# rll/rllab

Hardware: AMD Instinct MI355X
Metric: env steps/sec over full TRPO iterations (sample + process + update), 4096 envs per MI355X (higher is better)
Workload: dtype f32

## Files before the change

### include/rllab_amd.h

```cpp
#ifndef RLLAB_AMD_H
#define RLLAB_AMD_H

#include <stddef.h>
#include <stdint.h>

#ifdef __cplusplus
extern "C" {
#endif

enum rl_env_kind {
    RL_ENV_CARTPOLE = 0,
    RL_ENV_DOUBLE_PENDULUM = 1,
    RL_ENV_SWIMMER = 2,
    RL_ENV_HALF_CHEETAH = 3,
    RL_ENV_CARTPOLE_SWINGUP = 4,
    RL_ENV_WALKER2D = 5,
    RL_ENV_HOPPER = 6,
    RL_ENV_INVERTED_DOUBLE_PENDULUM = 7
};

enum rl_status {
    RL_OK = 0,
    RL_ERR_ARG = -1,
    RL_ERR_UNSUPPORTED = -2,
// ... 288 lines not shown
    float* actions;
    float* means;
    float* rewards;
    uint8_t* dones;
    float* first_path;
    const rl_env_cfg* cfg;
    const rl_launch_opts* opts;
} rl_population_gru_args;

int rl_rollout_population_gru(const rl_population_gru_args* args, void* stream);

int rl_gae(int T, int n, const float* rewards, const double* values, const uint8_t* dones,
           double gamma, double lambda, float* adv, float* ret, float* undiscounted, void* stream);

int rl_discount_cumsum(int T, int n, const float* x, const uint8_t* dones, double discount,
                       float* y, void* stream);


int rl_path_scan(int T, int n, int obs_dim, const uint8_t* dones, const float* obs, const double* coeffs,
                 int whole_paths, int32_t* tin, uint8_t* valid, double* values, void* stream);

size_t rl_process_workspace_bytes(int obs_dim);

int rl_sample_stats_cols(void);

int rl_sample_stats(size_t n_samples, const float* returns, const double* baselines,
                    const float* advantages, const float* undiscounted, const int32_t* tin,
                    const uint8_t* valid, double ret_shift, double und_shift, const float* progress,
                    int n_cols, void* workspace, size_t workspace_bytes, double* out, void* stream);

int rl_adv_finish(size_t n_samples, const float* adv_in, const uint8_t* valid, double mean, double denom,
                  double shift, float* adv_out, void* stream);

int rl_lfb_normal_eq(size_t n_samples, int obs_dim, const float* obs, const int32_t* tin,
                     const float* returns, const uint8_t* valid, void* workspace, size_t workspace_bytes,
                     double* out, int variant, void* stream);


size_t rl_reps_workspace_bytes(int T, int n);

int rl_reps_dual(int T, int n, int obs_dim, const float* obs, const float* rewards, const int32_t* tin,
                 const uint8_t* dones, const uint8_t* valid, double eta, const double* v_host, void* workspace,
                 size_t workspace_bytes, double* out, void* stream);

int rl_reps_weights(int T, int n, int obs_dim, const float* obs, const float* rewards, const int32_t* tin,
                    const uint8_t* dones, const uint8_t* valid, double eta, const double* v_host,
                    const double* dual_out, float* weights, void* stream);

typedef struct rl_policy_batch {
    int32_t n_samples;
    int32_t obs_dim, act_dim;
    int32_t hidden0, hidden1;
    int32_t hidden2;
    float inv_count;
    float log_min_std;
    const float* theta;
    const float* obs;
    const float* actions;
    const float* advantages;
    const float* old_means;
    const float* old_log_std;
    const float* weights;
    float* activations;
    float kl_penalty;
    int32_t activation;
    const rl_launch_opts* opts;
    int32_t layer_activations;
    int32_t reserved_pad;
    const int32_t* gate;
    float* obs_absmax;
} rl_policy_batch;

enum rl_activation { RL_ACT_TANH = 0, RL_ACT_RECTIFY = 1, RL_ACT_IDENTITY = 2 };

size_t rl_policy_workspace_bytes(int obs_dim, int act_dim, int hidden0, int hidden1, int hidden2);

size_t rl_policy_activation_bytes(int n_samples, int hidden0, int hidden1, int hidden2);

int rl_policy_loss_kl(const rl_policy_batch* batch, void* workspace, size_t workspace_bytes,
                      double* out4, void* stream);

int rl_policy_grad(const rl_policy_batch* batch, int vpg, void* workspace, size_t workspace_bytes,
                   double* grad_out, void* stream);

int rl_policy_grad_loss(const rl_policy_batch* batch, int vpg, void* workspace, size_t workspace_bytes,
                        double* grad_out, double* out4, void* stream);

int rl_policy_fvp(const rl_policy_batch* batch, const float* vec, void* workspace,
                  size_t workspace_bytes, double* fvp_out, void* stream);

int rl_policy_fvp_variant(const rl_policy_batch* batch);


int rl_mlp_forward(const rl_policy_batch* batch, const float* vec, float* out, float* dout, void* stream);
int rl_mlp_forward_ws(const rl_policy_batch* batch, const float* vec, void* workspace, size_t workspace_bytes, float* out,
                      float* dout, void* stream);

int rl_mlp_backward(const rl_policy_batch* batch, const float* cotangent, void* workspace, size_t workspace_bytes,
                    double* grad_out, void* stream);

size_t rl_gaussian_head_workspace_bytes(void);
int rl_gaussian_head(size_t n_samples, int act_dim, const float* mean, const float* log_std, const float* actions,
                     const float* advantages, const float* old_means, const float* old_log_stds,
// ... 45 lines not shown

int rl_categorical_softmax(size_t n_samples, int n_act, const float* logits, float* prob, void* stream);

size_t rl_categorical_head_workspace_bytes(void);
int rl_categorical_head(size_t n_samples, int n_act, const float* logits, const float* actions, const float* advantages,
                        const float* old_prob, const float* weights, float inv_count, int vpg, float kl_penalty,
                        float* g_logits, void* workspace, size_t workspace_bytes, double* out4, void* stream);

int rl_categorical_fisher(size_t n_samples, int n_act, const float* dlogits, const float* logits, const float* weights,
                          float inv_count, float* g_logits, void* stream);

int rl_cmaes_cov_update(int N, int ld, int mu, int mu_neg, double* C, double* Yneg, double* dC, const double* Ypos,
                        const double* wpos, const double* Vneg, const double* wneg, const double* pc, const double* scal,
                        void* stream);

int rl_cg_init(int n, const double* b, double* x, double* r, double* p, float* p32, double* scal,
               void* stream);
int rl_cg_step(int n, const double* fvp, double reg_coeff, double residual_tol, double* x, double* r,
               double* p, float* p32, double* scal, void* stream);

int rl_policy_fvp_cg_step(const rl_policy_batch* batch, void* workspace, size_t workspace_bytes, double reg_coeff,
                          double residual_tol, double* x, double* r, double* p, float* p32, double* scal,
                          double* fvp_scratch, unsigned int* ticket, void* stream);

int rl_trpo_step(int n, const double* x, const double* a, const double* b, double reg_coeff,
                 double max_constraint, double* step, double* out, void* stream);

int rl_line_search_point(int n, const float* prev, const double* step, double ratio, float* theta,
                         void* stream);

int rl_line_search_decide(int rows, const double* sums, const double* before, double inv_count, double max_constraint,
                          int candidate, double* state, int32_t* gate, int n, const float* prev, const double* step,
                          double next_ratio, float* theta, void* stream);

int rl_adam_step(int n, float* theta, const double* grad, double* m, double* v, double a_t, double beta1,
                 double beta2, double epsilon, void* stream);

size_t rl_peer_mailbox_bytes(int world, int max_n);
int rl_peer_alloc(size_t bytes, void** dev_ptr_out);
int rl_peer_free(void* dev_ptr);
int rl_peer_export(void* dev_ptr, void* handle_out64_host);
int rl_peer_open(const void* handle64_host, void** dev_ptr_out);
int rl_peer_close(void* dev_ptr);
int rl_peer_allreduce_sum(int n, double* data, int rank, int world, void* const* mailboxes_host, int max_n,
                          uint64_t seq, int* err_dev, int64_t spin_limit, void* stream);

int rl_debug_philox(uint32_t c0, uint32_t c1, uint32_t c2, uint32_t c3, uint32_t k0, uint32_t k1,
                    int count, uint32_t* out, void* stream);

#ifdef __cplusplus
}
#endif
#endif
```

### profiles/make_index.py

```python
#!/usr/bin/env python3
import fnmatch
import os
import subprocess

ROOT = os.path.dirname(os.path.dirname(os.path.abspath(__file__)))

RECIPES = [
    ("pmc_traffic.json", "HBM bytes + vector-instruction counters of the rollout kernels per workload, stamped with sha256(csrc/*); bench.py reads it",
     "profiles/run_profile.sh <tag> (traffic step: profiles/summarize.py traffic ...)"),
    ("gru_bptt_time.json", "loss + KL, gradient and Fisher-vector product of a GaussianGRUPolicy per call, and one whole TRPO update: the recurrent update kernels next to the float32 autograd closures, the sampler's batch for 4096 Cartpole envs, max_path_length 100 (105 rows x 4096 columns), 32 units",
     "python tools/exp/gru_bptt_time.py --out profiles/gru_bptt_time.json"),
    ("categorical_gru_bptt_time.json", "loss + KL, gradient and Fisher-vector product of a CategoricalGRUPolicy per call, and one whole TRPO update: the recurrent categorical update kernels next to the float32 autograd closures, the sampler's batch for 4096 GridWorld 4x4 envs, max_path_length 100, 32 units",
     "python tools/exp/categorical_gru_bptt_time.py --out profiles/categorical_gru_bptt_time.json"),
    ("*_bench_line.json", "the default bench line of that tree", "python bench.py"),
    ("*_bench_under_rocprof.log", "bench stdout under the kernel-trace pass", "profiles/run_profile.sh <tag>"),
    ("*_c5_kernel_stats.csv", "kernel stats of C5's per-GPU shard", "profiles/run_profile.sh <tag> cheetah1024_trpo_gae"),
    ("*_c5_pmc_*.csv", "PMC passes of C5's per-GPU shard (one counter group per pass)", "profiles/run_profile.sh <tag> cheetah1024_trpo_gae"),
    ("*_c2_*.csv", "kernel stats / PMC passes of C2 (Cartpole 4096 envs, VPG)", "profiles/run_profile.sh <tag> cartpole4096_vpg"),
    ("r06_csplit_*.csv", "SQ counter passes / kernel stats of csplit_fvp_kernel on (100, 50, 25) and (128, 128) at 2.048 M samples", "tools/exp/r06_call8.sh"),
    ("r06_c7_csplit_ab.txt", "cooperative product per library: round start / one instruction stream per wavefront (off) / compile-time shapes + k-slices", "tools/exp/r06_call7.sh"),
    ("r06_c9_csplit_ab.txt", "cooperative product per library: k-slices + compile-time shapes / round start / + late fetch", "tools/exp/r06_call9.sh"),
    ("r06_c10_csplit_ab.txt", "cooperative product: the library of the round's start, timed in the call that ran the parity tests and the wide bench lines on the final one", "tools/exp/r06_call10.sh"),
    ("r06_f16_split.txt", "device facts of the two-way f16 split: subnormal inputs honoured, accuracy of five product forms against float64 over ten magnitude regimes, the five-instruction split bit for bit, instruction rates", "tools/ubench/f16_split.hip (tools/exp/r06_call15.sh)"),
    ("r06_c14_half*.txt", "what a two-part / three-term product would buy: RL_ABL_HALF timing ablation of the bf16 split kernels (wrong results)", "tools/exp/r06_call14.sh"),
    ("r06_c16_splith_ab*.txt", "fvp() per library: bf16 three-way / f16 two-way / ablations and variants of policy_splith_kernels.hip", "tools/exp/r06_call16.sh"),
    ("r06_c18_splith_check.txt", "two-way f16 / three-way bf16 / f32 products against float64 over shapes, direction and observation scales, with timings", "tools/exp/fvp_splith_check.py (tools/exp/r06_call18.sh)"),
    ("r06_c17_bench_*.json", "headline and C5 bench lines, f16 two-way (default) and bf16 three-way (RLLAB_FVP_SPLIT=5) interleaved in one call", "tools/exp/r06_call17.sh"),
    ("r06_c20_splith_ab_wide.txt", "fvp() of (20, 6) on (32, 32), 512 k samples: bf16 three-way against f16 two-way at one wavefront per SIMD", "tools/exp/r06_call20.sh"),
    ("r06_splith_*.csv", "SQ counter passes / FETCH_SIZE / kernel stats of the bf16 and the f16 split products, (32, 32) at 2.048 M and (64, 64) at 512 k samples", "tools/exp/r06_call19.sh"),
    ("curves/r06_splith_*", "learning under the f16 two-way and the bf16 three-way split products, same seeds; 1500-iteration soak", "tools/exp/r06_splith_curves.sh"),
    ("fvp_lds_tr_ab_product.txt", "fvp() of the parent and the new library swapped in alternately, (13, 2) on (32, 32) at 2.048 M samples: the unit operands transposed through LDS, and two variants not kept",
     "tools/exp/fvp_split_ab.py's loop with FVP_AB_WARM=400 FVP_AB_N=300 FVP_AB_READINGS=9, the parent as build/exp/lib_parent.so"),
    ("fvp_lds_tr_ab_bench.txt", "headline bench lines of the parent and the new library, interleaved, and their --dump-outputs compared", "tools/exp/lib_ab.py 'python bench.py --gpus 1 --steps 20 --warmup 3'"),
    ("fvp_lds_tr_*_pmc_product.csv", "one SQ counter pass over ten f16 split products at 2.048 M samples, parent / new library", "rocprofv3 --kernel-trace --pmc SQ_VALU_MFMA_BUSY_CYCLES SQ_INSTS_VALU SQ_ACTIVE_INST_VALU SQ_INSTS_LDS SQ_LDS_BANK_CONFLICT SQ_WAIT_INST_ANY SQ_WAVES GRBM_GUI_ACTIVE -- python tools/exp/fvp_splith_pmc.py 32"),
    ("r06_c11_policy_time.txt", "wide loss / gradient / product passes with (.orig) and without (lib_before_wpf) the one-tile-ahead prefetch", "tools/exp/r06_call11.sh"),
    ("r06_wide_kernel_bench.txt", "loss / gradient / product passes of the wide nets at the final sources", "python tools/kernel_bench.py --configs ..."),
    ("*_split_kernel_stats.csv", "kernel stats of the three Fisher-vector-product kernels back to back", "tools/prof_split.sh"),
    ("*_split_pmc_*.csv", "PMC passes of the product kernels", "tools/prof_split.sh"),
    ("*_split64_*.csv", "kernel stats / PMC passes of the 64-unit split product", "tools/prof_split.sh 64"),
    ("*_wide*_pmc_*.csv", "PMC passes of the wide / deep kernels", "tools/prof_wide.sh"),
    ("*_wide*_stats.csv", "kernel stats of the wide / deep kernels", "tools/prof_wide.sh"),
    ("*_fvp_fixed_cost_stats.csv", "50 cached products back to back per batch size", "python tools/exp/fvp_fixed_cost.py under rocprofv3 --kernel-trace --stats"),
    ("*_step_kernel_roofline.jsonl", "rl_vecenv_step at 4 M envs, HIP-event timing", "python tools/step_kernel_roofline.py"),
    ("*_step_kernel_stats.csv", "the same under rocprofv3 --kernel-trace --stats", "profiles/run_profile.sh <tag>"),
    ("*_timeline.csv", "one iteration's dispatch timeline (start, duration, idle gap)", "profiles/run_profile.sh <tag> (summarize.py timeline)"),
    ("*_kernel_stats.csv", "rocprofv3 --kernel-trace --stats summary of `bench.py --steps 5 --warmup 2`", "profiles/run_profile.sh <tag>"),
    ("*_cheetah_pmc_*.csv", "PMC passes of the HalfCheetah shard", "profiles/run_profile.sh <tag> (cheetah leg)"),
    ("*_pmc_fetch_size.csv", "FETCH_SIZE pass (own run)", "profiles/run_profile.sh <tag>"),
    ("*_pmc_write_size.csv", "WRITE_SIZE pass (own run)", "profiles/run_profile.sh <tag>"),
    ("*_pmc_sq*.csv", "SQ_* counter passes (own runs)", "profiles/run_profile.sh <tag>"),
    ("*_bench_*.json", "side bench line: workload / size / switch in the file name", "python bench.py --workload ... | --n-envs ... | --hidden ... (tools/exp/r0N_final_bench.sh)"),
    ("*_resource_usage.txt", "-Rpass-analysis=kernel-resource-usage lines (registers, spills, LDS) of the named kernels", "tools/resource_usage.sh"),
    ("*_preflight*.json", "multi-GPU pre-flight record", "python tools/preflight_multigpu.py"),
    ("*_notes.md", "the round's measurements, experiments and dead ends in prose", "(written by hand from the files of that round)"),
    ("*_fallback_probe_*.txt", "which constructor options stay on the fused path, and the cost of an iteration (512 envs x 100 steps)",
     "python tools/exp/fallback_probe.py / tools/exp/fallback_probe_envs.py"),
    ("curves/r05_*", "tabular training logs of round 5's learning-curve runs", "tools/exp/r05_curves.sh, tools/exp/r05_call13.sh"),
    ("curves/*", "tabular training logs of the learning-curve runs", "tools/learning_curves.sh, tools/exp/r03_*curves*.sh"),
    ("run_profile.sh", "the profile recipe", "-"),
    ("summarize.py", "condenses rocprofv3 output directories into the CSVs kept here", "-"),
    ("make_index.py", "writes this index", "-"),
    ("INDEX.md", "this file", "python profiles/make_index.py"),
]
# ... 39 lines not shown
```

### rllab_amd/_lib.py

```python
import ctypes
import os

import torch

_HERE = os.path.dirname(os.path.abspath(__file__))
LIB_PATH = os.path.join(_HERE, "librllab_amd.so")

ENV_CARTPOLE = 0
ENV_DOUBLE_PENDULUM = 1
ENV_SWIMMER = 2
ENV_HALF_CHEETAH = 3
ENV_CARTPOLE_SWINGUP = 4
ENV_WALKER2D = 5
ENV_HOPPER = 6
ENV_INVERTED_DOUBLE_PENDULUM = 7

SYMBOLS = [
    "rl_last_error", "rl_abi_version", "rl_env_query", "rl_env_terminates", "rl_env_action_bounds", "rl_env_default_cfg", "rl_vecenv_com",
    "rl_vecenv_reset", "rl_vecenv_step", "rl_vecenv_step_graph", "rl_counter_add", "rl_vecenv_observe", "rl_rollout_gaussian_mlp", "rl_rollout_plan_query", "rl_rollout_lds_bytes", "rl_rollout_population", "rl_rollout_gaussian_gru",
    "rl_gru_workspace_bytes", "rl_gru_gaussian_eval", "rl_gru_gaussian_grad", "rl_gru_gaussian_fvp",
    "rl_gru_categorical_workspace_bytes", "rl_gru_categorical_eval", "rl_gru_categorical_grad", "rl_gru_categorical_fvp",
    "rl_rollout_population_gru", "rl_gae",
    "rl_discount_cumsum", "rl_debug_philox", "rl_policy_workspace_bytes", "rl_policy_activation_bytes", "rl_policy_loss_kl",
    "rl_policy_grad", "rl_policy_grad_loss", "rl_policy_fvp", "rl_policy_fvp_variant", "rl_policy_fvp_cg_step", "rl_cg_init", "rl_cg_step", "rl_trpo_step", "rl_line_search_point", "rl_line_search_decide", "rl_adam_step",
    "rl_path_scan", "rl_process_workspace_bytes", "rl_sample_stats_cols", "rl_sample_stats", "rl_adv_finish",
    "rl_lfb_normal_eq", "rl_reps_workspace_bytes", "rl_reps_dual", "rl_reps_weights",
    "rl_peer_mailbox_bytes", "rl_peer_alloc", "rl_peer_free", "rl_peer_export", "rl_peer_open", "rl_peer_close",
    "rl_peer_allreduce_sum",
    "rl_mlp_forward", "rl_mlp_forward_ws", "rl_mlp_backward", "rl_gaussian_head_workspace_bytes", "rl_gaussian_head", "rl_gaussian_fisher",
    "rl_rollout_gridworld", "rl_rollout_gridworld_gru", "rl_categorical_softmax", "rl_categorical_head_workspace_bytes", "rl_categorical_head",
    "rl_categorical_fisher", "rl_cmaes_cov_update",
]


class EnvCfg(ctypes.Structure):
    _fields_ = [
        ("ctrl_cost_coeff", ctypes.c_float), ("alive_coeff", ctypes.c_float), ("action_noise", ctypes.c_float),
        ("obs_noise", ctypes.c_float), ("frame_skip", ctypes.c_int32), ("flags", ctypes.c_int32),
        ("link_len", ctypes.c_float), ("reserved", ctypes.c_float), ("action_noise_z", ctypes.c_void_p), ("obs_noise_z", ctypes.c_void_p),
    ]


CFG_POLE_FOLLOWS_CART, CFG_FIXED_START, CFG_LIMIT_MUJOCO, CFG_CONTACT_MUJOCO = 1, 2, 4, 8


class RolloutArgs(ctypes.Structure):
    _fields_ = [
        ("kind", ctypes.c_int32), ("n_envs", ctypes.c_int32), ("horizon", ctypes.c_int32),
        ("max_path_length", ctypes.c_int32), ("normalize", ctypes.c_int32),
        ("reset_at_start", ctypes.c_int32), ("hidden0", ctypes.c_int32), ("hidden1", ctypes.c_int32),
        ("hidden2", ctypes.c_int32), ("env_offset", ctypes.c_int32), ("scale_reward", ctypes.c_float),
        ("log_min_std", ctypes.c_float), ("seed", ctypes.c_uint64), ("step_counter", ctypes.c_uint64),
        ("state", ctypes.c_void_p), ("ts", ctypes.c_void_p), ("theta", ctypes.c_void_p),
        ("eps", ctypes.c_void_p), ("reset_draws", ctypes.c_void_p), ("obs", ctypes.c_void_p),
        ("actions", ctypes.c_void_p), ("means", ctypes.c_void_p), ("rewards", ctypes.c_void_p),
        ("dones", ctypes.c_void_p), ("last_obs", ctypes.c_void_p), ("cfg", ctypes.POINTER(EnvCfg)),
        ("theta_std", ctypes.c_void_p), ("log_stds", ctypes.c_void_p), ("std_hidden0", ctypes.c_int32),
        ("std_hidden1", ctypes.c_int32), ("std_hidden2", ctypes.c_int32), ("layer_activations", ctypes.c_int32),
# ... 64 lines not shown
        ("reset_at_start", ctypes.c_int32), ("n_row", ctypes.c_int32), ("n_col", ctypes.c_int32),
        ("n_act", ctypes.c_int32), ("start_state", ctypes.c_int32), ("env_offset", ctypes.c_int32),
        ("reserved", ctypes.c_int32), ("seed", ctypes.c_uint64), ("step_counter", ctypes.c_uint64),
        ("cell", ctypes.c_void_p), ("prob", ctypes.c_void_p), ("u", ctypes.c_void_p), ("state", ctypes.c_void_p),
        ("ts", ctypes.c_void_p), ("obs", ctypes.c_void_p), ("actions", ctypes.c_void_p), ("prob_out", ctypes.c_void_p),
        ("rewards", ctypes.c_void_p), ("dones", ctypes.c_void_p),
    ]


class GridWorldGruArgs(ctypes.Structure):
    _fields_ = [
        ("n_envs", ctypes.c_int32), ("horizon", ctypes.c_int32), ("max_path_length", ctypes.c_int32),
        ("reset_at_start", ctypes.c_int32), ("n_row", ctypes.c_int32), ("n_col", ctypes.c_int32),
        ("n_act", ctypes.c_int32), ("start_state", ctypes.c_int32), ("env_offset", ctypes.c_int32),
        ("hidden", ctypes.c_int32), ("include_action", ctypes.c_int32), ("reserved", ctypes.c_int32),
        ("seed", ctypes.c_uint64), ("step_counter", ctypes.c_uint64),
        ("cell", ctypes.c_void_p), ("theta", ctypes.c_void_p), ("u", ctypes.c_void_p), ("state", ctypes.c_void_p),
        ("ts", ctypes.c_void_p), ("hidden_state", ctypes.c_void_p), ("prev_action", ctypes.c_void_p),
        ("obs", ctypes.c_void_p), ("actions", ctypes.c_void_p), ("prob_out", ctypes.c_void_p),
        ("rewards", ctypes.c_void_p), ("dones", ctypes.c_void_p),
    ]


class PolicyBatch(ctypes.Structure):
    _fields_ = [
        ("n_samples", ctypes.c_int32), ("obs_dim", ctypes.c_int32), ("act_dim", ctypes.c_int32),
        ("hidden0", ctypes.c_int32), ("hidden1", ctypes.c_int32), ("hidden2", ctypes.c_int32),
        ("inv_count", ctypes.c_float),
        ("log_min_std", ctypes.c_float), ("theta", ctypes.c_void_p), ("obs", ctypes.c_void_p),
        ("actions", ctypes.c_void_p), ("advantages", ctypes.c_void_p), ("old_means", ctypes.c_void_p),
        ("old_log_std", ctypes.c_void_p), ("weights", ctypes.c_void_p), ("activations", ctypes.c_void_p),
        ("kl_penalty", ctypes.c_float), ("activation", ctypes.c_int32), ("opts", ctypes.c_void_p),
        ("layer_activations", ctypes.c_int32), ("reserved_pad", ctypes.c_int32), ("gate", ctypes.c_void_p),
        ("obs_absmax", ctypes.c_void_p),
    ]


ACT_TANH, ACT_RECTIFY, ACT_IDENTITY = 0, 1, 2


def layer_activation_bits(codes):
    if all(c == ACT_TANH for c in codes):
        return 0
    return sum((int(c) + 1) << (2 * l) for l, c in enumerate(codes))


class LaunchOpts(ctypes.Structure):
    _fields_ = [
        ("rollout_epw", ctypes.c_int32), ("rollout_wpb", ctypes.c_int32), ("swimmer_lane_kernel", ctypes.c_int32),
        ("swimmer_coop", ctypes.c_int32), ("two_leg_lane_kernel", ctypes.c_int32), ("two_leg_wave_kernel", ctypes.c_int32),
        ("fvp_split", ctypes.c_int32), ("fvp_split_wps", ctypes.c_int32), ("lfb_valu", ctypes.c_int32),
        ("reserved", ctypes.c_int32 * 7),
    ]


class RunningNorm(ctypes.Structure):
    _fields_ = [
        ("obs_mean", ctypes.c_void_p), ("obs_var", ctypes.c_void_p), ("reward_mean", ctypes.c_void_p),
        ("reward_var", ctypes.c_void_p), ("obs_alpha", ctypes.c_double), ("reward_alpha", ctypes.c_double),
        ("normalize_obs", ctypes.c_int32), ("normalize_reward", ctypes.c_int32),
    ]


class RolloutPlan(ctypes.Structure):
    _fields_ = [
        ("kernel", ctypes.c_int32), ("envs_per_wavefront", ctypes.c_int32), ("wavefronts", ctypes.c_int32),
        ("wavefronts_per_workgroup", ctypes.c_int32), ("workgroups", ctypes.c_int32), ("lds_bytes", ctypes.c_int32),
# ... 73 lines not shown
                                         ctypes.POINTER(ctypes.c_size_t)]
    lib.rl_rollout_population.argtypes = [ctypes.POINTER(PopulationArgs), vp]
    lib.rl_rollout_gaussian_gru.argtypes = [ctypes.POINTER(GruRolloutArgs), vp]
    lib.rl_rollout_population_gru.argtypes = [ctypes.POINTER(PopulationGruArgs), vp]
    lib.rl_gru_workspace_bytes.restype = ctypes.c_size_t
    lib.rl_gru_workspace_bytes.argtypes = [i32, i32, i32, i32, i32, i32]
    lib.rl_gru_gaussian_eval.argtypes = [ctypes.POINTER(GruBatch), vp, vp]
    lib.rl_gru_gaussian_grad.argtypes = [ctypes.POINTER(GruBatch), vp, vp, vp]
    lib.rl_gru_gaussian_fvp.argtypes = [ctypes.POINTER(GruBatch), vp, vp, vp]
    lib.rl_gru_categorical_workspace_bytes.restype = ctypes.c_size_t
    lib.rl_gru_categorical_workspace_bytes.argtypes = [i32, i32, i32, i32, i32]
    lib.rl_gru_categorical_eval.argtypes = [ctypes.POINTER(GruCategoricalBatch), vp, vp]
    lib.rl_gru_categorical_grad.argtypes = [ctypes.POINTER(GruCategoricalBatch), vp, vp, vp]
    lib.rl_gru_categorical_fvp.argtypes = [ctypes.POINTER(GruCategoricalBatch), vp, vp, vp]
    lib.rl_gae.argtypes = [i32, i32, vp, vp, vp, f64, f64, vp, vp, vp, vp]
    lib.rl_discount_cumsum.argtypes = [i32, i32, vp, vp, f64, vp, vp]
    lib.rl_debug_philox.argtypes = [u32, u32, u32, u32, u32, u32, i32, vp, vp]
    pb = ctypes.POINTER(PolicyBatch)
    lib.rl_policy_workspace_bytes.restype = ctypes.c_size_t
    lib.rl_policy_workspace_bytes.argtypes = [i32, i32, i32, i32, i32]
    lib.rl_policy_activation_bytes.restype = ctypes.c_size_t
    lib.rl_policy_activation_bytes.argtypes = [i32, i32, i32, i32]
    lib.rl_policy_loss_kl.argtypes = [pb, vp, ctypes.c_size_t, vp, vp]
    lib.rl_policy_grad.argtypes = [pb, i32, vp, ctypes.c_size_t, vp, vp]
    lib.rl_policy_grad_loss.argtypes = [pb, i32, vp, ctypes.c_size_t, vp, vp, vp]
    lib.rl_policy_fvp.argtypes = [pb, vp, vp, ctypes.c_size_t, vp, vp]
    lib.rl_policy_fvp_variant.argtypes = [pb]
    lib.rl_policy_fvp_cg_step.argtypes = [pb, vp, ctypes.c_size_t, f64, f64, vp, vp, vp, vp, vp, vp, vp, vp]
    lib.rl_cg_init.argtypes = [i32, vp, vp, vp, vp, vp, vp, vp]
    lib.rl_cg_step.argtypes = [i32, vp, f64, f64, vp, vp, vp, vp, vp, vp]
    lib.rl_trpo_step.argtypes = [i32, vp, vp, vp, f64, f64, vp, vp, vp]
    lib.rl_line_search_point.argtypes = [i32, vp, vp, f64, vp, vp]
    lib.rl_line_search_decide.argtypes = [i32, vp, vp, f64, f64, i32, vp, vp, i32, vp, vp, f64, vp, vp]
    lib.rl_adam_step.argtypes = [i32, vp, vp, vp, vp, f64, f64, f64, f64, vp]
    sz = ctypes.c_size_t
    lib.rl_path_scan.argtypes = [i32, i32, i32, vp, vp, vp, i32, vp, vp, vp, vp]
    lib.rl_process_workspace_bytes.restype = sz
    lib.rl_process_workspace_bytes.argtypes = [i32]
    lib.rl_sample_stats_cols.restype = i32
    lib.rl_sample_stats.argtypes = [sz, vp, vp, vp, vp, vp, vp, f64, f64, vp, i32, vp, sz, vp, vp]
    lib.rl_adv_finish.argtypes = [sz, vp, vp, f64, f64, f64, vp, vp]
    lib.rl_lfb_normal_eq.argtypes = [sz, i32, vp, vp, vp, vp, vp, sz, vp, i32, vp]
    lib.rl_reps_workspace_bytes.restype = sz
    lib.rl_reps_workspace_bytes.argtypes = [i32, i32]
    lib.rl_reps_dual.argtypes = [i32, i32, i32, vp, vp, vp, vp, vp, f64, vp, vp, sz, vp, vp]
    lib.rl_reps_weights.argtypes = [i32, i32, i32, vp, vp, vp, vp, vp, f64, vp, vp, vp, vp]
    lib.rl_mlp_forward.argtypes = [pb, vp, vp, vp, vp]
    lib.rl_mlp_forward_ws.argtypes = [pb, vp, vp, sz, vp, vp, vp]
    lib.rl_mlp_backward.argtypes = [pb, vp, vp, sz, vp, vp]
    lib.rl_gaussian_head_workspace_bytes.restype = sz
    lib.rl_gaussian_head_workspace_bytes.argtypes = []
    lib.rl_gaussian_head.argtypes = [sz, i32, vp, vp, vp, vp, vp, vp, vp, f32, f32, i32, f32, vp, vp, vp, sz, vp, vp]
    lib.rl_gaussian_fisher.argtypes = [sz, i32, vp, vp, vp, vp, f32, f32, vp, vp, vp]
    lib.rl_rollout_gridworld.argtypes = [ctypes.POINTER(GridWorldArgs), vp]
    lib.rl_rollout_gridworld_gru.argtypes = [ctypes.POINTER(GridWorldGruArgs), vp]
    lib.rl_categorical_softmax.argtypes = [sz, i32, vp, vp, vp]
    lib.rl_categorical_head_workspace_bytes.restype = sz
    lib.rl_categorical_head_workspace_bytes.argtypes = []
    lib.rl_categorical_head.argtypes = [sz, i32, vp, vp, vp, vp, vp, f32, i32, f32, vp, vp, sz, vp, vp]
    lib.rl_categorical_fisher.argtypes = [sz, i32, vp, vp, vp, f32, vp, vp]
    lib.rl_cmaes_cov_update.argtypes = [i32, i32, i32, i32, vp, vp, vp, vp, vp, vp, vp, vp, vp, vp]
    vpp = ctypes.POINTER(ctypes.c_void_p)
    lib.rl_peer_mailbox_bytes.restype = sz
    lib.rl_peer_mailbox_bytes.argtypes = [i32, i32]
    lib.rl_peer_alloc.argtypes = [sz, vpp]
    lib.rl_peer_free.argtypes = [vp]
    lib.rl_peer_export.argtypes = [vp, vp]
    lib.rl_peer_open.argtypes = [vp, vpp]
    lib.rl_peer_close.argtypes = [vp]
    lib.rl_peer_allreduce_sum.argtypes = [i32, vp, i32, i32, vpp, i32, u64, vp, ctypes.c_int64, vp]
    for name in SYMBOLS:
        getattr(lib, name)
    return lib


# ... 81 lines not shown
```

### rllab_amd/algos/npo.py

```python
import os

import torch

import rllab_amd.misc.logger as logger
from rllab_amd.algos.batch_polopt import BatchPolopt
from rllab_amd.sampler import dist as D


def npo_inputs(policy, samples_data):
    traj = samples_data["_traj"]
    B = traj.B
    w = traj.valid.reshape(B).to(torch.float32)
    if getattr(traj, "count", None) is not None:
        cnt = torch.tensor(float(traj.count), dtype=torch.float64)
    else:
        cnt = D.all_reduce_sum_(w.to(torch.float64).sum())
    if getattr(traj, "categorical", False) and getattr(policy, "recurrent", False):
        return (traj.obs, traj.actions, traj.advantages, traj.means, (traj.tin == 0), traj.valid.to(torch.float32),
                (1.0 / cnt))
    if getattr(traj, "categorical", False):
        return (traj.obs.reshape(traj.obs_dim, B), traj.actions.reshape(traj.act_dim, B), traj.advantages.reshape(B),
                traj.means.reshape(traj.act_dim, B), w, (1.0 / cnt))
    if getattr(policy, "recurrent", False):
        if traj.log_std_planes is not None:
            raise NotImplementedError("a recurrent batch with per-sample log_std planes")
        return (traj.obs, traj.actions, traj.advantages, traj.means, traj.log_std.reshape(-1, 1, 1),
                (traj.tin == 0), traj.valid.to(torch.float32), (1.0 / cnt))
    old_ls = traj.log_std.reshape(-1, 1) if traj.log_std_planes is None \
        else traj.log_std_planes.reshape(traj.act_dim, B)
    return (traj.obs.reshape(traj.obs_dim, B), traj.actions.reshape(traj.act_dim, B),
            traj.advantages.reshape(B), traj.means.reshape(traj.act_dim, B), old_ls, w, (1.0 / cnt))


def log_update_path(policy, fused, why=None):
    if fused is not None:
        logger.log("update path: HIP kernels (%s)" % type(fused).__name__)
        return
    if why is None and hasattr(policy, "why_no_kernel_layout"):
        why = policy.why_no_kernel_layout()
    if why is None and getattr(policy, "recurrent", False) and getattr(policy, "bptt_kernels", False):
        why = "the recurrent kernels serve ConjugateGradientOptimizer (TRPO, TNPG)"
    logger.log("update path: torch autograd%s" % ("" if why is None else " -- " + why))


# ... 156 lines not shown
```

### rllab_amd/baselines/linear_feature_baseline.py

```python
import os

import numpy as np
import torch

from rllab_amd.baselines.base import Baseline


class LinearFeatureBaseline(Baseline):
    def __init__(self, env_spec, reg_coeff=1e-5):
        self._coeffs_value = None
        self._pending = None
        self._reg_coeff = reg_coeff

    @property
    def _coeffs(self):
        if self._pending is not None:
            read, F = self._pending
            self._pending = None
            host = read.get()
            self._coeffs_value = self._solve(host[:F * F].reshape(F, F), host[F * F:])
        return self._coeffs_value

    @_coeffs.setter
    def _coeffs(self, value):
        self._pending = None
        self._coeffs_value = value

    def __getstate__(self):
        d = dict(self.__dict__)
        d["_coeffs_value"] = self._coeffs
        d["_pending"] = None
        return d

    def __setstate__(self, d):
        d = dict(d)
        if "_coeffs" in d:
            d["_coeffs_value"] = d.pop("_coeffs")
        d.setdefault("_pending", None)
        self.__dict__.update(d)

    def get_param_values(self, **tags):
        return self._coeffs

    def set_param_values(self, val, **tags):
        self._coeffs = val

    def _features(self, path):
        o = np.clip(path["observations"], -10, 10)
        l = len(path["rewards"])
        al = np.arange(l).reshape(-1, 1) / 100.0
        return np.concatenate([o, o ** 2, al, al ** 2, al ** 3, np.ones((l, 1))], axis=1)

    def _solve(self, gram, rhs):
        reg_coeff = self._reg_coeff
        coeffs = None
        for _ in range(5):
            coeffs = np.linalg.lstsq(gram + reg_coeff * np.identity(gram.shape[0]), rhs, rcond=None)[0]
            if not np.any(np.isnan(coeffs)):
                break
            reg_coeff *= 10
        return coeffs

    def fit(self, paths):
        if hasattr(paths, "traj"):
            return self.fit_dense(paths.traj)
        featmat = np.concatenate([self._features(path) for path in paths])
        returns = np.concatenate([path["returns"] for path in paths])
        self._coeffs = self._solve(featmat.T.dot(featmat), featmat.T.dot(returns))

    def predict(self, path):
        if self._coeffs is None:
            return np.zeros(len(path["rewards"]))
        return self._features(path).dot(self._coeffs)

    def dense_coeffs(self):
        return self._coeffs

    @staticmethod
    def _features_dense(traj):
        o = traj.obs.reshape(traj.obs_dim, -1).to(torch.float64).clamp(-10, 10)
        al = (traj.time_in_path().reshape(1, -1).to(torch.float64)) / 100.0
        return torch.cat([o, o ** 2, al, al ** 2, al ** 3, torch.ones_like(al)], dim=0)

    def predict_dense(self, traj):
        if self._coeffs is None:
            return None
        if traj.obs_dim <= 21 and traj.device.type == "cuda":
            from rllab_amd.sampler.base import path_scan
            return path_scan(traj, True, self._coeffs)[2]
        w = torch.as_tensor(self._coeffs, dtype=torch.float64, device=traj.device)
        return (w @ self._features_dense(traj)).reshape(traj.T, traj.N)

    def fit_dense(self, traj, all_reduce=None):
        packed = self.normal_eq_dense(traj)
        if all_reduce is not None:
            all_reduce(packed)
        self.fit_from_packed(packed, 2 * traj.obs_dim + 4)

    def fit_from_packed(self, packed, F):
        from rllab_amd.misc.device_io import read_async
        self._coeffs_value = None
        self._pending = (read_async(packed), F)

    def normal_eq_dense(self, traj):
        F = 2 * traj.obs_dim + 4
        if traj.obs_dim <= 21 and traj.device.type == "cuda":
            from rllab_amd import _lib
            from rllab_amd.sampler.base import _workspace, path_scan
            tin = getattr(traj, "tin", None)
            if tin is None:
                tin = path_scan(traj, True, None, want_values=False)[0]
            valid = traj.valid if traj.valid is not None else torch.ones((traj.T, traj.N), dtype=torch.bool,
                                                                         device=traj.device)
            valid_u8 = valid.contiguous().view(torch.uint8) if valid.dtype == torch.bool else valid.to(torch.uint8).contiguous()
            ws = _workspace(traj.device, traj.obs_dim)
            packed = torch.empty((F + 1) * F, dtype=torch.float64, device=traj.device)
            _lib.check(_lib.lib.rl_lfb_normal_eq(traj.B, traj.obs_dim, _lib.ptr(traj.obs), _lib.ptr(tin),
                                                 _lib.ptr(traj.returns), _lib.ptr(valid_u8), _lib.ptr(ws),
                                                 ws.numel(), _lib.ptr(packed),
                                                 1 if os.environ.get("RLLAB_LFB_VALU") is not None else 0,
                                                 _lib.stream_ptr()),
                       "rl_lfb_normal_eq")
        else:
            phi = self._features_dense(traj)
            w = traj.valid.reshape(1, -1).to(torch.float64) if traj.valid is not None else None
            y = traj.returns.reshape(-1).to(torch.float64)
            phi_w = phi * w if w is not None else phi
            packed = torch.cat([(phi_w @ phi.t()).reshape(-1), phi_w @ y])
        return packed
```

### rllab_amd/csrc/cg_kernels.hip

```cpp
#include <hip/hip_runtime.h>
#include "../../include/rllab_amd.h"
#include "capi_util.h"
#include "cg_device.h"

namespace rl {

__global__ void __launch_bounds__(CG_THREADS) cg_init_kernel(int n, const double* __restrict__ b,
                                                             double* __restrict__ x, double* __restrict__ r,
                                                             double* __restrict__ p, float* __restrict__ p32,
                                                             double* __restrict__ scal) {
    __shared__ double scratch[CG_THREADS / 64];
    double acc = 0.0;
    for (int i = threadIdx.x; i < n; i += CG_THREADS) {
        const double bi = b[i];
        x[i] = 0.0; r[i] = bi; p[i] = bi; p32[i] = (float)bi;
        acc += bi * bi;
    }
    const double rdotr = block_sum(acc, scratch);
    if (threadIdx.x == 0) { scal[0] = rdotr; scal[1] = 1.0; scal[2] = 0.0; scal[3] = 0.0; }
}

__global__ void __launch_bounds__(CG_THREADS) cg_step_kernel(int n, const double* __restrict__ fp, double reg,
                                                             double tol, double* __restrict__ x,
                                                             double* __restrict__ r, double* __restrict__ p,
// ... 36 lines not shown
                                                               double delta, double* __restrict__ step,
                                                               double* __restrict__ out) {
    __shared__ double scratch[CG_THREADS / 64];
    double xv[CG_MAX_PER_THREAD];
    double acc = 0.0;
#pragma unroll
    for (int k = 0; k < CG_MAX_PER_THREAD; ++k) {
        const int i = threadIdx.x + k * CG_THREADS;
        if (i < n) {
            xv[k] = x[i];
            const double hx = (b ? a[i] - b[i] : a[i]) + reg * xv[k];
            acc += xv[k] * hx;
        }
    }
    const double xHx = block_sum(acc, scratch);
    double beta = sqrt(2.0 * delta * (1.0 / (xHx + 1e-8)));
    if (beta != beta) beta = 1.0;
#pragma unroll
    for (int k = 0; k < CG_MAX_PER_THREAD; ++k) {
        const int i = threadIdx.x + k * CG_THREADS;
        if (i < n) step[i] = beta * xv[k];
    }
    if (threadIdx.x == 0) { out[0] = xHx; out[1] = beta; }
}

__global__ void __launch_bounds__(256) line_search_point_kernel(int n, const float* __restrict__ prev,
                                                                const double* __restrict__ step, double ratio,
                                                                float* __restrict__ theta) {
    const int i = blockIdx.x * 256 + threadIdx.x;
    if (i < n) theta[i] = (float)((double)prev[i] - ratio * step[i]);
}

__global__ void __launch_bounds__(CG_THREADS) line_search_decide_kernel(
        int rows, const double* __restrict__ sums, const double* __restrict__ before, double inv_count, double delta,
        int candidate, double* __restrict__ state, int32_t* __restrict__ gate, int n, const float* __restrict__ prev,
        const double* __restrict__ step, double next_ratio, float* __restrict__ theta) {
    __shared__ int go_on;
    if (threadIdx.x == 0) {
        bool accepted = state[0] != 0.0;
        if (!accepted) {
            double s0 = 0.0, s1 = 0.0, s2 = 0.0, mx = -INFINITY, b0 = 0.0;
            for (int r = 0; r < rows; ++r) {
                s0 += sums[4 * r]; s1 += sums[4 * r + 1]; s2 += sums[4 * r + 2];
                mx = fmax(mx, sums[4 * r + 3]);
                b0 += before[4 * r];
            }
            double* rec = state + 2 + 4 * candidate;
            rec[0] = s0; rec[1] = s1; rec[2] = s2; rec[3] = mx;
            const double loss = -(s0 * inv_count), loss_before = -(b0 * inv_count), kl = s1 * inv_count;
            if (loss < loss_before && kl <= delta) {
                accepted = true;
                state[0] = 1.0;
                state[1] = (double)candidate;
                *gate = 1;
            }
        }
        go_on = accepted ? 0 : 1;
    }
    __syncthreads();
    if (go_on && next_ratio > 0.0)
        for (int i = threadIdx.x; i < n; i += CG_THREADS) theta[i] = (float)((double)prev[i] - next_ratio * step[i]);
}

__global__ void __launch_bounds__(256) adam_step_kernel(int n, float* __restrict__ theta, const double* __restrict__ g,
                                                        double* __restrict__ m, double* __restrict__ v, double a_t,
                                                        double b1, double b2, double eps) {
    const int i = blockIdx.x * 256 + threadIdx.x;
    if (i >= n) return;
    const double gi = g[i];
    const double mi = b1 * m[i] + (1.0 - b1) * gi;
    const double vi = b2 * v[i] + (1.0 - b2) * gi * gi;
    m[i] = mi;
    v[i] = vi;
// ... 11 lines not shown
                       a_t, beta1, beta2, epsilon);
    return check_launch("adam_step_kernel");
}

extern "C" int rl_trpo_step(int n, const double* x, const double* a, const double* b, double reg_coeff,
                            double max_constraint, double* step, double* out, void* stream) {
    if (n <= 0 || n > CG_MAX_N || !x || !a || !step || !out)
        return set_error(RL_ERR_ARG, "rl_trpo_step: bad argument (n = %d, max %d)", n, CG_MAX_N);
    if (n <= CG_THREADS * CG_MAX_PER_THREAD)
        hipLaunchKernelGGL(trpo_step_kernel, dim3(1), dim3(CG_THREADS), 0, (hipStream_t)stream, n, x, a, b, reg_coeff,
                           max_constraint, step, out);
    else
        hipLaunchKernelGGL(trpo_step_large_kernel, dim3(1), dim3(CG_THREADS), 0, (hipStream_t)stream, n, x, a, b,
                           reg_coeff, max_constraint, step, out);
    return check_launch("trpo_step_kernel");
}

extern "C" int rl_line_search_point(int n, const float* prev, const double* step, double ratio, float* theta,
                                    void* stream) {
    if (n <= 0 || !prev || !step || !theta) return set_error(RL_ERR_ARG, "rl_line_search_point: bad argument");
    hipLaunchKernelGGL(line_search_point_kernel, dim3((n + 255) / 256), dim3(256), 0, (hipStream_t)stream, n, prev,
                       step, ratio, theta);
    return check_launch("line_search_point_kernel");
}

extern "C" int rl_line_search_decide(int rows, const double* sums, const double* before, double inv_count,
                                     double max_constraint, int candidate, double* state, int32_t* gate, int n,
                                     const float* prev, const double* step, double next_ratio, float* theta,
                                     void* stream) {
    if (rows <= 0 || !sums || !before || !state || !gate || candidate < 0 ||
        (next_ratio > 0.0 && (n <= 0 || !prev || !step || !theta)))
        return set_error(RL_ERR_ARG, "rl_line_search_decide: bad argument");
    hipLaunchKernelGGL(line_search_decide_kernel, dim3(1), dim3(CG_THREADS), 0, (hipStream_t)stream, rows, sums, before,
                       inv_count, max_constraint, candidate, state, gate, n, prev, step, next_ratio, theta);
    return check_launch("line_search_decide_kernel");
}

extern "C" int rl_cg_init(int n, const double* b, double* x, double* r, double* p, float* p32, double* scal,
                          void* stream) {
    if (n <= 0 || n > CG_MAX_N || !b || !x || !r || !p || !p32 || !scal)
        return set_error(RL_ERR_ARG, "rl_cg_init: bad argument (n = %d, max %d)", n, CG_MAX_N);
    hipLaunchKernelGGL(cg_init_kernel, dim3(1), dim3(CG_THREADS), 0, (hipStream_t)stream, n, b, x, r, p, p32, scal);
    return check_launch("cg_init_kernel");
}

extern "C" int rl_cg_step(int n, const double* fvp, double reg_coeff, double residual_tol, double* x, double* r,
                          double* p, float* p32, double* scal, void* stream) {
    if (n <= 0 || n > CG_MAX_N || !fvp || !x || !r || !p || !p32 || !scal)
        return set_error(RL_ERR_ARG, "rl_cg_step: bad argument (n = %d, max %d)", n, CG_MAX_N);
    if (n <= CG_THREADS * CG_MAX_PER_THREAD)
        hipLaunchKernelGGL(cg_step_kernel, dim3(1), dim3(CG_THREADS), 0, (hipStream_t)stream, n, fvp, reg_coeff,
                           residual_tol, x, r, p, p32, scal);
    else
        hipLaunchKernelGGL(cg_step_large_kernel, dim3(1), dim3(CG_THREADS), 0, (hipStream_t)stream, n, fvp, reg_coeff,
                           residual_tol, x, r, p, p32, scal);
    return check_launch("cg_step_kernel");
}
```

### rllab_amd/csrc/policy_csplit_kernels.hip

```cpp
#include <hip/hip_runtime.h>
#include <cstdlib>
#include "../../include/rllab_amd.h"
#include "capi_util.h"
#include "policy_mfma.h"
#include "policy_wide.h"

namespace rl {

int launch_reduce_rows(const float* partial, int rows, int cols, double* out, hipStream_t st);
bool net_has_narrow_kernel(int obs_dim, int act_dim, int h0, int h1, int h2);

namespace cs {

typedef __attribute__((ext_vector_type(8))) __bf16 bf16x8;
typedef __attribute__((ext_vector_type(4))) __bf16 bf16x4;
typedef __attribute__((ext_vector_type(2))) __bf16 bf16x2;
typedef __attribute__((ext_vector_type(4))) short s16x4;
typedef __attribute__((ext_vector_type(2))) float f32x2;
typedef __attribute__((ext_vector_type(4))) float f32x4;
typedef __attribute__((address_space(3))) s16x4* lds_s16x4_ptr;

constexpr int CH = 1088;
constexpr int HSTR = 576;
constexpr int TILE_IMG = 6 * CH;
// ... 794 lines not shown
        if constexpr (L == 2) {
            CS_CASE(2, 0x44, 4) CS_CASE(2, 0x24, 2) CS_CASE(2, 0x14, 2) CS_CASE(2, 0x42, 2) CS_CASE(2, 0x41, 2)
        } else {
            CS_CASE(3, 0x244, 4) CS_CASE(3, 0x144, 4) CS_CASE(3, 0x224, 2) CS_CASE(3, 0x124, 2) CS_CASE(3, 0x114, 2)
        }
#undef CS_CASE
    }
    if (maxht == 2) return launch<L, 2, 2>(s, g, vec, ws, ws_bytes, out, st);
    return mt4 ? launch<L, 4, 4>(s, g, vec, ws, ws_bytes, out, st) : launch<L, 4, 2>(s, g, vec, ws, ws_bytes, out, st);
}

}

bool csplit_fvp_takes(const rl_policy_batch* g) {
    if (!g->activations || g->activation != RL_ACT_TANH || g->layer_activations != 0 || g->n_samples <= 0 ||
        g->n_samples % TS != 0)
        return false;
    const int req = g->opts ? g->opts->fvp_split : 0;
    if (req == 1) return false;
    cs::CsShape s;
    if (!cs::cs_shape(g, s)) return false;
    if (req == 2) return true;
    return s.HT[0] == 4 || s.HT[1] == 4 || s.HT[2] == 4;
}
size_t csplit_workspace_bytes_for(int obs_dim, int act_dim, int h0, int h1, int h2) {
    rl_policy_batch g = {};
    g.obs_dim = obs_dim; g.act_dim = act_dim; g.hidden0 = h0; g.hidden1 = h1; g.hidden2 = h2;
    cs::CsShape s;
    if (!cs::cs_shape(&g, s)) return 0;
    return cs::cs_workspace(s);
}
int csplit_fvp_dispatch(const rl_policy_batch* g, const float* vec, void* ws, size_t ws_bytes, double* out, hipStream_t st) {
    if (!csplit_fvp_takes(g)) return RL_SPLIT_NOT_TAKEN;
    cs::CsShape s;
    cs::cs_shape(g, s);
    return s.L == 2 ? cs::launch_class<2>(s, g, vec, ws, ws_bytes, out, st)
                    : cs::launch_class<3>(s, g, vec, ws, ws_bytes, out, st);
}

}
```

### rllab_amd/csrc/policy_kernels.hip

```cpp
#include <hip/hip_runtime.h>
#include "../../include/rllab_amd.h"
#include "capi_util.h"
#include "cg_device.h"
#include "policy_mfma.h"

namespace rl {


enum { MODE_LOSS = 0, MODE_GRAD = 1, MODE_FVP = 2, MODE_VPG = 3, MODE_OUT = 4, MODE_OUT_TAN = 5, MODE_BWD = 6 };
constexpr int LOSS_COLS = 4;

template <class N, int MODE, bool CACHE = false>
struct Smem {
    static constexpr bool GRADLIKE = (MODE == MODE_GRAD || MODE == MODE_FVP || MODE == MODE_VPG || MODE == MODE_BWD);
    static constexpr bool FVP = (MODE == MODE_FVP);
    static constexpr bool TAN = (MODE == MODE_FVP || MODE == MODE_OUT_TAN);
    static constexpr int ACT_FLOATS = 2 * N::H * TS;
    static constexpr int A0 = 0;
    static constexpr int A1 = A0 + N::FA0;
    static constexpr int A1T = A1 + N::FA1;
    static constexpr int DA0 = A1T + (GRADLIKE ? N::FA1 : 0);
    static constexpr int DA1 = DA0 + (TAN ? N::FA0 : 0);
    static constexpr int TAIL = DA1 + (TAN ? N::FA1 : 0);
    static constexpr int DTAIL = TAIL + N::TAILP;
    static constexpr int WAVE0 = DTAIL + (TAN ? N::TAILP : 0);
    static constexpr int WAVES = N::WAVES;
    static constexpr int ACTQ = WAVE0 + WAVES * N::WAVE_LDS;
    static constexpr int TOTAL = ACTQ + ((FVP && CACHE && N::ACT_LDS_PREFETCH) ? WAVES * ACT_FLOATS : 0);
    static constexpr int RED = 0;
    static_assert(TOTAL >= N::P, "LDS fold buffer must fit");
};

struct PolicyBatch {
    int B;
    const float* theta;
    const float* vec;
    float* acts;
    const float* obs;
    const float* act;
    const float* adv;
    const float* old_mean;
    const float* old_log_std;
    const float* weight;
    float inv_count;
    float log_min_std;
    float kl_penalty;
    const float* cot;
    float* out_mean;
    float* out_dmean;
    float* partial;
    double* partial_loss;
    const int* gate;
    unsigned* obs_absmax;
    int act0, act1;
};

template <bool RELU> __device__ __forceinline__ float act_fn(float z) { return RELU ? fmaxf(z, 0.0f) : ftanh(z); }
template <bool RELU> __device__ __forceinline__ float act_dz(float h) {
    return RELU ? (h > 0.0f ? 1.0f : 0.0f) : (1.0f - h * h);
}

#ifndef RL_POLICY_LOSS_WPS
#define RL_POLICY_LOSS_WPS 4
#endif
template <class N, int MODE>
constexpr int pass_wps() { return (MODE == MODE_LOSS && N::WPS < RL_POLICY_LOSS_WPS) ? RL_POLICY_LOSS_WPS : N::WPS; }

template <class N, int MODE, bool CACHE, bool RELU = false, bool ACTS = false>
__global__ void __launch_bounds__(N::WAVES * WV, (pass_wps<N, MODE>())) policy_pass_kernel(PolicyBatch a) {
    constexpr int WAVES = N::WAVES;
    static_assert(!CACHE || MODE == MODE_GRAD || MODE == MODE_FVP, "activation cache: grad writes, FVP reads");
    static_assert(!RELU || MODE == MODE_LOSS || MODE == MODE_VPG, "rectify nets: loss and log-likelihood gradient");
    using S = Smem<N, MODE, CACHE>;
    constexpr int DO = N::DO, DA = N::DA, H = N::H, HT = N::HT, KS0 = N::KS0, KS1 = N::KS1, P = N::P;
    constexpr bool GRADLIKE = S::GRADLIKE, FVP = S::FVP, TAN = S::TAN;
    constexpr bool OUTMODE = (MODE == MODE_OUT || MODE == MODE_OUT_TAN), BWD = (MODE == MODE_BWD);
    constexpr bool HEAD = (MODE == MODE_LOSS || MODE == MODE_GRAD || MODE == MODE_VPG);
    constexpr bool LOAD_ACTS = CACHE && FVP, STORE_ACTS = CACHE && !FVP;
    constexpr int TSTR = N::TSTR, XS = N::XS, GS = N::GS;
    constexpr int ACT_ROWS = 2 * HT * 4;

    extern __shared__ __attribute__((aligned(16))) float smem[];
    if (MODE == MODE_LOSS) {
        if (a.gate != nullptr && *a.gate != 0) return;
    }
    const int wave = threadIdx.x / WV, lane = threadIdx.x % WV;
    const int lj = lane & 31, lh = lane >> 5;
    const int c0 = RELU ? 1 : (ACTS ? a.act0 : 0), c1 = RELU ? 1 : (ACTS ? a.act1 : 0);
    float* const fa0 = smem + S::A0;
    float* const fa1 = smem + S::A1;
    float* const fa1t = smem + S::A1T;
    float* const fda0 = smem + S::DA0;
    float* const fda1 = smem + S::DA1;
    float* const tail = smem + S::TAIL;
    float* const dtail = smem + S::DTAIL;
    float* const tb = smem + S::WAVE0 + wave * N::WAVE_LDS;
    float* const tbx = tb + TS * TSTR;
    float* const tbg = tbx + TS * XS;

    stage_fragments<N, WAVES * WV>(a.theta, fa0, fa1, GRADLIKE ? fa1t : nullptr);
    if (TAN) stage_fragments<N, WAVES * WV>(a.vec, fda0, fda1, nullptr);
    for (int k = threadIdx.x; k < N::TAIL; k += WAVES * WV) {
        tail[k] = a.theta[N::B1 + k];
        if (TAN) dtail[k] = a.vec[N::B1 + k];
    }
    for (int k = lane; k < N::WAVE_LDS; k += WV) tb[k] = 0.0f;
    __syncthreads();
    constexpr int T_B1 = 0, T_W2 = N::W2 - N::B1, T_B2 = N::B2 - N::B1, T_LS = N::LSTD - N::B1;

    float lstd[DA], inv_std[DA], var_[DA];
    bool floored[DA];
#pragma unroll
    for (int k = 0; k < DA; ++k) {
        const float raw = tail[T_LS + k];
        floored[k] = raw < a.log_min_std;
// ... 167 lines not shown
            const float advb = a.adv[bi];
            float zz_new = 0.0f, zz_old = 0.0f, sls_new = 0.0f, sls_old = 0.0f, kl = 0.0f;
            float znew[DA], dmv[DA], numv[DA];
#pragma unroll
            for (int k = 0; k < DA; ++k) {
                const float ak = a.act[(size_t)k * B + bi];
                const float mo = a.old_mean[(size_t)k * B + bi];
                const float lo = a.old_log_std[k];
                const float so = __expf(lo);
                znew[k] = (ak - mean[k]) * inv_std[k];
                const float zo = (ak - mo) / so;
                zz_new = __builtin_fmaf(znew[k], znew[k], zz_new);
                zz_old = __builtin_fmaf(zo, zo, zz_old);
                sls_new += lstd[k];
                sls_old += lo;
                const float dm = mo - mean[k];
                const float num = dm * dm + so * so - var_[k];
                const float den = 2.0f * var_[k] + 1e-8f;
                kl += num / den + lstd[k] - lo;
                dmv[k] = dm;
                numv[k] = num;
            }
            const float logp_new = -sls_new - 0.5f * zz_new;
            const float dlog = logp_new - (-sls_old - 0.5f * zz_old);
            const float lr = __expf(dlog);
            const float w1 = (lh == 0) ? wgt : 0.0f;
            if (MODE == MODE_LOSS || ((MODE == MODE_GRAD || MODE == MODE_VPG) && a.partial_loss != nullptr)) {
                acc_loss += (double)(w1 * lr * advb);
                acc_kl += (double)(w1 * kl);
                acc_vpg += (double)(w1 * (logp_new - 0.5f * (float)DA * 1.8378770664093453f) * advb);
                if (w1 > 0.0f) max_kl = fmaxf(max_kl, kl);
            }
            if (MODE != MODE_LOSS) {
                const float c = -wgt * advb * (MODE == MODE_GRAD ? lr : 1.0f) * a.inv_count;
                const float c1 = (lh == 0) ? c : 0.0f;
#pragma unroll
                for (int k = 0; k < DA; ++k) {
                    gmu[k] = c * znew[k] * inv_std[k];
                    if (!floored[k]) gls[k] += c1 * (znew[k] * znew[k] - 1.0f);
                }
                if (a.kl_penalty != 0.0f) {
                    const float p = a.kl_penalty * wgt * a.inv_count;
                    const float p1 = (lh == 0) ? p : 0.0f;
#pragma unroll
                    for (int k = 0; k < DA; ++k) {
                        const float den = 2.0f * var_[k] + 1e-8f;
                        const float dkl_mu = -2.0f * dmv[k] / den;
                        const float dkl_ls = 1.0f - (2.0f * var_[k] * den + 4.0f * var_[k] * numv[k]) / (den * den);
                        gmu[k] = __builtin_fmaf(p, dkl_mu, gmu[k]);
                        if (!floored[k]) gls[k] += p1 * dkl_ls;
                    }
                }
            }
        }
        float dmu_[DA];
        if constexpr (TAN) {
            f32x16 dh0[HT], dh1[HT];
#pragma unroll
            for (int t = 0; t < HT; ++t) {
                f32x16 acc;
#pragma unroll
                for (int r = 0; r < 16; ++r) acc[r] = 0.0f;
#pragma unroll
                for (int m = 0; m < KS0; ++m) acc = mfma(fda0[(t * KS0 + m) * WV + lane], xb[m], acc);
                act_bwd_frag(dh0[t], acc, h0[t], c0);
            }
#pragma unroll
            for (int t = 0; t < HT; ++t) {
                f32x16 acc;
#pragma unroll
                for (int r = 0; r < 16; ++r) acc[r] = dtail[T_B1 + 32 * t + frag_unit(r, 0) + 4 * lh];
#pragma unroll
                for (int m = 0; m < KS1; ++m) {
                    acc = mfma(fda1[(t * KS1 + m) * WV + lane], h0[m / 16][m % 16], acc);
                    acc = mfma(fa1[(t * KS1 + m) * WV + lane], dh0[m / 16][m % 16], acc);
                }
                act_bwd_frag(dh1[t], acc, h1[t], c1);
            }
            const float c = wgt * a.inv_count;
#pragma unroll
            for (int k = 0; k < DA; ++k) {
                float pd = 0.0f;
#pragma unroll
                for (int t = 0; t < HT; ++t)
#pragma unroll
                    for (int r = 0; r < 16; ++r) {
                        const int u = (32 * t + frag_unit(r, 0) + 4 * lh) * DA + k;
                        pd = __builtin_fmaf(h1[t][r], dtail[T_W2 + u], pd);
                        pd = __builtin_fmaf(dh1[t][r], tail[T_W2 + u], pd);
                    }
                const float dmu = dtail[T_B2 + k] + half_sum(pd);
                dmu_[k] = dmu;
                if constexpr (FVP) gmu[k] = c * dmu * (2.0f / (2.0f * var_[k] + 1e-8f));
            }
            if (FVP && lh == 0) wsum += c;
        }
        if constexpr (OUTMODE) {
            if (live && lh == 0) {
#pragma unroll
                for (int k = 0; k < DA; ++k) {
                    a.out_mean[(size_t)k * B + b] = mean[k];
                    if constexpr (MODE == MODE_OUT_TAN) a.out_dmean[(size_t)k * B + b] = dmu_[k];
                }
            }
        }
        if constexpr (BWD) {
#pragma unroll
            for (int k = 0; k < DA; ++k) gmu[k] = live ? a.cot[(size_t)k * B + bi] : 0.0f;
        }

        if (GRADLIKE) {
            f32x16 gz1[HT], gz0[HT];
// ... 319 lines not shown
int launch_reduce_loss(const double* partial, int rows, double* out, hipStream_t st) {
    hipLaunchKernelGGL(reduce_loss_kernel, dim3(1), dim3(LOSS_COLS * WV), 0, st, partial, rows, out);
    return check_launch("reduce_loss_kernel");
}
int wide_dispatch(int mode, const rl_policy_batch* g, const float* vec, void* ws, size_t ws_bytes, double* out,
                  hipStream_t st, double* loss_out, const float* cot = nullptr, float* out_mean = nullptr,
                  float* out_dmean = nullptr);
struct WideShape;
int split_fvp_dispatch(const rl_policy_batch* g, const float* vec, void* ws, size_t ws_bytes, double* out, hipStream_t st);
int splith_fvp_dispatch(const rl_policy_batch* g, const float* vec, void* ws, size_t ws_bytes, double* out, hipStream_t st);
int csplit_fvp_dispatch(const rl_policy_batch* g, const float* vec, void* ws, size_t ws_bytes, double* out, hipStream_t st);
size_t csplit_workspace_bytes_for(int obs_dim, int act_dim, int h0, int h1, int h2);
size_t wide_workspace_bytes_for(int obs_dim, int act_dim, int h0, int h1, int h2);

struct PlaneArgs {
    const float* cot = nullptr;
    float* out_mean = nullptr;
    float* out_dmean = nullptr;
};

template <class N, int MODE, bool CACHE = false, bool RELU = false, bool ACTS = false>
static int launch_pass(const rl_policy_batch* g, const float* vec, void* workspace, size_t workspace_bytes,
                       double* out, hipStream_t st, double* loss_out = nullptr, const CgArgs* cg = nullptr,
                       const PlaneArgs* planes = nullptr) {
    using S = Smem<N, MODE, CACHE>;
    PolicyBatch a;
    a.cot = planes ? planes->cot : nullptr;
    a.out_mean = planes ? planes->out_mean : nullptr;
    a.out_dmean = planes ? planes->out_dmean : nullptr;
    a.acts = g->activations;
    a.kl_penalty = g->kl_penalty;
    a.B = g->n_samples; a.theta = g->theta; a.vec = vec; a.obs = g->obs; a.act = g->actions; a.adv = g->advantages;
    a.old_mean = g->old_means; a.old_log_std = g->old_log_std; a.weight = g->weights;
    a.inv_count = g->inv_count; a.log_min_std = g->log_min_std;
    a.gate = (MODE == MODE_LOSS) ? g->gate : nullptr;
    a.obs_absmax = nullptr;
    if (MODE == MODE_GRAD && CACHE && g->activations && g->obs_absmax) {
        a.obs_absmax = reinterpret_cast<unsigned*>(g->obs_absmax);
        hipError_t e = hipMemsetAsync(g->obs_absmax, 0, sizeof(float), st);
        if (e != hipSuccess) return set_error(RL_ERR_HIP, "hipMemsetAsync(obs_absmax): %s", hipGetErrorString(e));
    }
    a.act0 = layer_act(g->activation, g->layer_activations, 0);
    a.act1 = layer_act(g->activation, g->layer_activations, 1);
    const int n_tiles = (a.B + TS - 1) / TS;
    const size_t lds = (size_t)S::TOTAL * sizeof(float);
    if (lds > 160 * 1024) return set_error(RL_ERR_UNSUPPORTED, "policy pass needs %zu B of LDS", lds);
    constexpr int WAVES = N::WAVES;
    int blocks_per_cu = (int)((160 * 1024) / lds);
    if (blocks_per_cu > pass_wps<N, MODE>() * 4 / WAVES) blocks_per_cu = pass_wps<N, MODE>() * 4 / WAVES;
    int grid = 256 * blocks_per_cu;
    const int need = (n_tiles + WAVES - 1) / WAVES;
    if (grid > need) grid = need;
    if (grid > MAX_GRID) grid = MAX_GRID;
    const bool with_loss = (MODE == MODE_GRAD || MODE == MODE_VPG) && loss_out != nullptr;
    const size_t row_bytes = (((size_t)grid * N::P * sizeof(float)) + 15) & ~(size_t)15;
    constexpr bool OUTMODE = (MODE == MODE_OUT || MODE == MODE_OUT_TAN);
    const size_t need_bytes = OUTMODE ? 0 : (MODE == MODE_LOSS)
        ? (size_t)grid * LOSS_COLS * sizeof(double)
        : row_bytes + (with_loss ? (size_t)grid * LOSS_COLS * sizeof(double) : 0);
    if (workspace_bytes < need_bytes)
        return set_error(RL_ERR_ARG, "policy pass workspace too small: %zu < %zu bytes", workspace_bytes,
                         need_bytes);
    a.partial = (float*)workspace;
    a.partial_loss = (MODE == MODE_LOSS) ? (double*)workspace
                                         : (with_loss ? (double*)((char*)workspace + row_bytes) : nullptr);
    auto kern = policy_pass_kernel<N, MODE, CACHE, RELU, ACTS>;
    static bool attr_set = false;
// ... 69 lines not shown
#define NARROWCASE(DO, DA, H) if (d == DO && k == DA && h0 == H && h1 == H) return true;
    RL_NARROW_NETS(NARROWCASE)
#undef NARROWCASE
    return false;
}

static int dispatch_net(int mode, const rl_policy_batch* g, const float* vec, void* ws, size_t ws_bytes,
                        double* out, hipStream_t st, double* loss_out = nullptr, const CgArgs* cg = nullptr,
                        const PlaneArgs* pl = nullptr) {
    const int d = g->obs_dim, k = g->act_dim, h0 = g->hidden0, h1 = g->hidden1;
    const int a0 = layer_act(g->activation, g->layer_activations, 0), a1 = layer_act(g->activation, g->layer_activations, 1),
              a2 = g->hidden2 > 0 ? layer_act(g->activation, g->layer_activations, 2) : RL_ACT_TANH;
    if (a0 < 0 || a0 > RL_ACT_IDENTITY || a1 < 0 || a1 > RL_ACT_IDENTITY || a2 < 0 || a2 > RL_ACT_IDENTITY)
        return set_error(RL_ERR_ARG, "unknown activation (%d, layers 0x%x)", g->activation, g->layer_activations);
    const bool all_tanh = a0 == RL_ACT_TANH && a1 == RL_ACT_TANH && a2 == RL_ACT_TANH;
    if (mode >= MODE_OUT) {
        if (a0 == RL_ACT_RECTIFY || a1 == RL_ACT_RECTIFY || a2 == RL_ACT_RECTIFY)
            return set_error(RL_ERR_UNSUPPORTED, "rl_mlp_forward / rl_mlp_backward: tanh (and identity) layers");
#define PLANECASE(DO, DA, H) \
        if (all_tanh && g->hidden2 == 0 && d == DO && k == DA && h0 == H && h1 == H) \
            return dispatch_planes<Net<DO, DA, H>>(mode, g, vec, ws, ws_bytes, out, st, pl);
        PLANECASE(4, 1, 32) PLANECASE(6, 1, 32) PLANECASE(11, 1, 32) PLANECASE(13, 2, 32) PLANECASE(20, 3, 32)
        PLANECASE(20, 6, 32) PLANECASE(21, 6, 32)
        PLANECASE(4, 1, 64) PLANECASE(6, 1, 64) PLANECASE(11, 1, 64) PLANECASE(13, 2, 64) PLANECASE(20, 3, 64)
        PLANECASE(20, 6, 64) PLANECASE(21, 6, 64)
#undef PLANECASE
        if (ws == nullptr)
            return set_error(RL_ERR_ARG, "rl_mlp_forward: obs_dim=%d act_dim=%d hidden=(%d,%d,%d) runs on the cooperative "
                             "kernels, which need a workspace: call rl_mlp_forward_ws", d, k, h0, h1, g->hidden2);
        return wide_dispatch(mode, g, vec, ws, ws_bytes, out, st, nullptr, pl ? pl->cot : nullptr,
                             pl ? pl->out_mean : nullptr, pl ? pl->out_dmean : nullptr);
    }
    if (g->hidden2 < 0) return set_error(RL_ERR_ARG, "rl_policy_batch.hidden2 = %d", g->hidden2);
    if (g->hidden2 > 0) {
        if (cg) return set_error(RL_ERR_UNSUPPORTED, "rl_policy_fvp_cg_step: two-layer 32 / 64-unit nets only");
        if (!all_tanh)
            return set_error(RL_ERR_UNSUPPORTED, "three hidden layers: tanh layers only (the cooperative kernels)");
        if (mode == MODE_FVP) {
            const int rc = csplit_fvp_dispatch(g, vec, ws, ws_bytes, out, st);
            if (rc != RL_SPLIT_NOT_TAKEN) return rc;
        }
        return wide_dispatch(mode, g, vec, ws, ws_bytes, out, st, loss_out);
    }
    if (g->activation == RL_ACT_RECTIFY && g->layer_activations == 0 && k == 1 && h0 == 32 && h1 == 32 &&
        (mode == MODE_LOSS || mode == MODE_VPG)) {
#define RELUCASE(DO) \
        if (d == DO && k == 1 && h0 == 32 && h1 == 32) return dispatch_relu<Net<DO, 1, 32>>(mode, g, ws, ws_bytes, out, st, loss_out);
        RELUCASE(4) RELUCASE(6) RELUCASE(11) RELUCASE(13) RELUCASE(20) RELUCASE(21)
#undef RELUCASE
    }
    if (g->kl_penalty != 0.0f && mode != MODE_VPG && mode != MODE_GRAD)
        return set_error(RL_ERR_ARG, "rl_policy_batch.kl_penalty applies to the gradient passes only");
    if (mode == MODE_FVP && cg == nullptr && all_tanh) {
        int rc = splith_fvp_dispatch(g, vec, ws, ws_bytes, out, st);
        if (rc != RL_SPLIT_NOT_TAKEN) return rc;
        rc = split_fvp_dispatch(g, vec, ws, ws_bytes, out, st);
        if (rc != RL_SPLIT_NOT_TAKEN) return rc;
        rc = csplit_fvp_dispatch(g, vec, ws, ws_bytes, out, st);
        if (rc != RL_SPLIT_NOT_TAKEN) return rc;
    }
#define NETCASE(DO, DA, H) \
    if (d == DO && k == DA && h0 == H && h1 == H) \
        return all_tanh ? dispatch_mode<Net<DO, DA, H>, false>(mode, g, vec, ws, ws_bytes, out, st, loss_out, cg) \
                        : dispatch_mode<Net<DO, DA, H>, true>(mode, g, vec, ws, ws_bytes, out, st, loss_out, cg);
    RL_NARROW_NETS(NETCASE)
#undef NETCASE
// ... 128 lines not shown
```

### rllab_amd/csrc/policy_mfma.h

```cpp
#pragma once
#include <hip/hip_runtime.h>

namespace rl {

constexpr int WV = 64;
constexpr int RL_SPLIT_NOT_TAKEN = 1 << 20;
constexpr int TS = 32;

using f32x16 = __attribute__((ext_vector_type(16))) float;

__device__ __forceinline__ float ftanh(float x) {
    const float e = __builtin_amdgcn_exp2f(x * 2.8853900817779268f);
    return __builtin_fmaf(-2.0f, __builtin_amdgcn_rcpf(e + 1.0f), 1.0f);
}

__device__ __forceinline__ void act_frag(f32x16& h, const f32x16& z, int code) {
    if (code == 0) {
#pragma unroll
        for (int r = 0; r < 16; ++r) h[r] = ftanh(z[r]);
    } else if (code == 1) {
#pragma unroll
        for (int r = 0; r < 16; ++r) h[r] = fmaxf(z[r], 0.0f);
    } else {
        h = z;
    }
}
__device__ __forceinline__ void act_bwd_frag(f32x16& out, const f32x16& v, const f32x16& h, int code) {
    if (code == 0) {
#pragma unroll
        for (int r = 0; r < 16; ++r) out[r] = v[r] * (1.0f - h[r] * h[r]);
    } else if (code == 1) {
#pragma unroll
        for (int r = 0; r < 16; ++r) out[r] = h[r] > 0.0f ? v[r] : 0.0f;
    } else {
        out = v;
    }
}
__device__ __forceinline__ float act_one(float z, int code) { return code == 0 ? ftanh(z) : code == 1 ? fmaxf(z, 0.0f) : z; }
__host__ __device__ inline int layer_act(int activation, int layer_activations, int l) {
    const int f = (layer_activations >> (2 * l)) & 3;
    return (layer_activations == 0 || f == 0) ? activation : f - 1;
}

__device__ __forceinline__ f32x16 mfma(float a, float b, f32x16 c) {
    return __builtin_amdgcn_mfma_f32_32x32x2f32(a, b, c, 0, 0, 0);
}
// ... 83 lines not shown
```

### rllab_amd/csrc/policy_split16_kernels.hip

```cpp
#include <hip/hip_runtime.h>
#include <cstdlib>
#include "../../include/rllab_amd.h"
#include "capi_util.h"
#include "policy_mfma.h"

namespace rl {

int launch_reduce_rows(const float* partial, int rows, int cols, double* out, hipStream_t st);

namespace split16 {

typedef __attribute__((ext_vector_type(8))) __bf16 bf16x8;
typedef __attribute__((ext_vector_type(2))) __bf16 bf16x2;
typedef __attribute__((ext_vector_type(2))) float f32x2;
typedef __attribute__((ext_vector_type(4))) float f32x4;
typedef __attribute__((ext_vector_type(4))) unsigned u32x4;
typedef __attribute__((address_space(3))) void* lptr_t;

constexpr int H = 32;
constexpr int T16 = 16;

#ifndef RL_SPLIT16_DOT2
#define RL_SPLIT16_DOT2 0
#endif
// ... 527 lines not shown
    int grid = (n_tiles + WAVES - 1) / WAVES;
    if (grid > 256) grid = 256;
    const size_t need = (size_t)grid * N::P * sizeof(float);
    if (ws_bytes < need) return set_error(RL_ERR_ARG, "policy pass workspace too small: %zu < %zu bytes", ws_bytes, need);
    a.partial = (float*)ws;
    auto kern = fvp_split16_kernel<DO, DA, WPS>;
    static bool attr_set = false;
    if (!attr_set) {
        hipError_t e = hipFuncSetAttribute(reinterpret_cast<const void*>(kern), hipFuncAttributeMaxDynamicSharedMemorySize,
                                           S::LDS_TOTAL);
        if (e != hipSuccess) return set_error(RL_ERR_HIP, "hipFuncSetAttribute: %s", hipGetErrorString(e));
        attr_set = true;
    }
    hipLaunchKernelGGL(kern, dim3(grid), dim3(WAVES * WV), S::LDS_TOTAL, st, a);
    int rc = check_launch("fvp_split16_kernel");
    if (rc) return rc;
    return launch_reduce_rows(a.partial, grid, N::P, out, st);
}

}

#define SPLIT16_SHAPES(X) X(4, 1) X(6, 1) X(11, 1) X(13, 2) X(13, 1)
bool split16_fvp_takes(const rl_policy_batch* g) {
    if (!g->activations || g->hidden2 != 0 || g->hidden0 != 32 || g->hidden1 != 32 || g->activation != RL_ACT_TANH ||
        g->layer_activations != 0 || g->n_samples <= 0 || g->n_samples % TS != 0)
        return false;
#define SPLITCASE(DO, DA) if (g->obs_dim == DO && g->act_dim == DA) return true;
    SPLIT16_SHAPES(SPLITCASE)
#undef SPLITCASE
    return false;
}
int split16_fvp_dispatch(const rl_policy_batch* g, const float* vec, void* ws, size_t ws_bytes, double* out, hipStream_t st) {
    if (!split16_fvp_takes(g)) return RL_SPLIT_NOT_TAKEN;
    const bool three = !(g->opts && g->opts->fvp_split_wps == 4);
#define SPLITCASE(DO, DA) if (g->obs_dim == DO && g->act_dim == DA) \
        return three ? split16::launch<DO, DA, 3>(g, vec, ws, ws_bytes, out, st) : split16::launch<DO, DA, 4>(g, vec, ws, ws_bytes, out, st);
    SPLIT16_SHAPES(SPLITCASE)
#undef SPLITCASE
    return RL_SPLIT_NOT_TAKEN;
}

}
```

### rllab_amd/csrc/policy_split_kernels.hip

```cpp
#include <hip/hip_runtime.h>
#include <cstdlib>
#include "../../include/rllab_amd.h"
#include "capi_util.h"
#include "policy_mfma.h"

namespace rl {

int launch_reduce_rows(const float* partial, int rows, int cols, double* out, hipStream_t st);

namespace split {

typedef __attribute__((ext_vector_type(8))) __bf16 bf16x8;
typedef __attribute__((ext_vector_type(2))) __bf16 bf16x2;
typedef __attribute__((ext_vector_type(2))) float f32x2;
typedef __attribute__((ext_vector_type(4))) float f32x4;
typedef __attribute__((address_space(1))) const void* gptr_t;
typedef __attribute__((address_space(3))) void* lptr_t;

constexpr int H = 32;
constexpr int LAND_BYTES = 2 * H * TS * 4;
constexpr int ops_count(int kb0) { return kb0 + 6; }
constexpr int ops_bytes(int kb0) { return ops_count(kb0) * 3 * WV * 16; }

struct Args {
    int B;
    const float* theta;
    const float* vec;
    const float* acts;
    const float* obs;
    const float* weight;
    float inv_count;
    float log_min_std;
    float* partial;
};

struct Parts { bf16x8 p[3]; };

#ifndef RL_ABL_MFMA
#define RL_ABL_MFMA 0
#endif
#ifndef RL_ABL_SPLIT
#define RL_ABL_SPLIT 0
#endif
#ifndef RL_ABL_FETCH
#define RL_ABL_FETCH 0
#endif
#ifndef RL_ABL_OPS
#define RL_ABL_OPS 0
#endif
#ifndef RL_ABL_HALF
#define RL_ABL_HALF 0
#endif
__device__ __forceinline__ f32x16 mfma16(bf16x8 a, bf16x8 b, f32x16 c) {
#if RL_ABL_MFMA
    asm volatile("" : "+v"(c) : "v"(a), "v"(b));
    return c;
#else
    return __builtin_amdgcn_mfma_f32_32x32x16_bf16(a, b, c, 0, 0, 0);
#endif
}
__device__ __forceinline__ f32x16 mm6(const Parts& A, const Parts& B, f32x16 c) {
#if !RL_ABL_HALF
    c = mfma16(A.p[1], B.p[1], c);
    c = mfma16(A.p[0], B.p[2], c);
// ... 139 lines not shown
__device__ __forceinline__ void set_pair(f32x16& v, int j, f32x2 p) { v[2 * j] = p[0]; v[2 * j + 1] = p[1]; }
__device__ __forceinline__ void times_dtanh(const f32x16& acc, const f32x16& h, f32x16& out) {
#if RL_SPLIT_PK
#pragma unroll
    for (int j = 0; j < 8; ++j) {
        const f32x2 hh = pair_of(h, j);
        const f32x2 d = __builtin_elementwise_fma(-hh, hh, f32x2{1.0f, 1.0f});
        set_pair(out, j, pair_of(acc, j) * d);
    }
#else
#pragma unroll
    for (int r = 0; r < 16; ++r) out[r] = acc[r] * (1.0f - h[r] * h[r]);
#endif
}

template <int DO, int DA, int WPS>
__global__ void __launch_bounds__(4 * WPS * WV, 1) fvp_split_kernel(Args a) {
    using N = Net<DO, DA, H>;
    constexpr int P = N::P;
    constexpr int WAVES = 4 * WPS;
    constexpr int KB0 = (DO + 1 + 15) / 16;
    constexpr int N_OPS = ops_count(KB0), OPS_BYTES = ops_bytes(KB0);
    constexpr bool INV_LDS = (WPS == 2);
    constexpr bool TAIL_LDS = INV_LDS || DA > 2;
    constexpr int TAILV = 16 * DA * 2 + 16;
    constexpr int SPILL_BYTES = INV_LDS ? 2 * 3 * WV * 16 : 0;
    constexpr int XPIECES = (DO + 1 + 7) / 8;
    constexpr int XLAND_BYTES = RL_SPLIT_ASM_DMA ? XPIECES * WV * 16 : 0;
    constexpr int WAVE_BYTES = LAND_BYTES + SPILL_BYTES + XLAND_BYTES;
    constexpr int LDS_TOTAL = WAVES * WAVE_BYTES + (INV_LDS ? OPS_BYTES : 0) + (TAIL_LDS ? 2 * TAILV * 4 : 0);
    static_assert(DO + 1 <= 32, "two k-blocks of inputs + the bias slot");
    static_assert(LDS_TOTAL >= WAVES * P * 4 && LDS_TOTAL <= 160 * 1024, "LDS budget; the fold rows alias the landing zones");
    extern __shared__ __attribute__((aligned(16))) char smem[];
    const int wave = threadIdx.x / WV, lane = threadIdx.x % WV;
    const int lj = lane & 31, lh = lane >> 5;
    char* const land = smem + wave * WAVE_BYTES;
    char* const spill = land + LAND_BYTES;
    char* const xland = spill + SPILL_BYTES;
    char* const ops = smem + WAVES * WAVE_BYTES;
    float* const tailv = reinterpret_cast<float*>(ops + (INV_LDS ? OPS_BYTES : 0));

    const int B = a.B;
    const int n_tiles = B / TS;
    const int wave_global = blockIdx.x * WAVES + wave;
    const int waves_total = gridDim.x * WAVES;

#if RL_SPLIT_ASM_DMA
    const unsigned xland_lds = __builtin_amdgcn_readfirstlane((unsigned)(size_t)(lptr_t)xland);
    auto fetch = [&](int tile, float (&)[KB0][8], float&) {
#pragma unroll
        for (int p = 0; p < XPIECES; ++p) {
            const int d = 8 * p + (lane >> 3);
            const float* g = (d < DO ? a.obs + (size_t)d * B : a.weight) + tile * TS + 4 * (lane & 7);
            asm volatile("s_mov_b32 m0, %1\n\tglobal_load_lds_dwordx4 %0, off" :: "v"(g), "s"(xland_lds + p * (WV * 16)) : "memory");
        }
    };
    auto take_x = [&](float (&xq)[KB0][8], float& wq) {
        const float* xl = reinterpret_cast<const float*>(xland) + lj;
#pragma unroll
        for (int kb = 0; kb < KB0; ++kb)
#pragma unroll
            for (int j = 0; j < 8; ++j) {
                const int d = 16 * kb + 8 * lh + j;
                const float v = xl[32 * (d < DO ? d : DO)];
                xq[kb][j] = d < DO ? v : (d == DO ? 1.0f : 0.0f);
            }
// ... 239 lines not shown
                }
                opcur = nxtp;
                __builtin_amdgcn_sched_barrier(0);
            }
        } else
#elif RL_SPLIT_OPS_AHEAD
        if constexpr (INV_LDS) acc = chain_ahead(KB0, 2, H0s, acc, opcur, KB0 + 2);
        else
#endif
#pragma unroll
        for (int kb = 0; kb < 2; ++kb) acc = mm6(op(KB0 + kb), H0s[kb], acc);
        if constexpr (INV_LDS) {
#pragma unroll
            for (int kb = 0; kb < 2; ++kb)
#pragma unroll
                for (int p = 0; p < 3; ++p) *reinterpret_cast<bf16x8*>(spill + ((kb * 3 + p) * WV + lane) * 16) = H0s[kb].p[p];
        }
        stage();
        {
            Parts D0s[2];
#if RL_SPLIT_OPS_AHEAD && RL_SPLIT_FILL
            if constexpr (INV_LDS) { D0s[0] = D0s_f[0]; D0s[1] = D0s_f[1]; }
            else
#endif
            split_frag(dh0, D0s);
#if RL_SPLIT_OPS_AHEAD
            if constexpr (INV_LDS) acc = chain_ahead(KB0 + 2, 2, D0s, acc, opcur, -1);
            else
#endif
#pragma unroll
            for (int kb = 0; kb < 2; ++kb) acc = mm6(op(KB0 + 2 + kb), D0s[kb], acc);
        }
        stage();
        const float c = wgt * a.inv_count;
        f32x16 dz1;
        float gmu[DA];
        f32x16 gz1;
#if RL_SPLIT_PK
#pragma unroll
        for (int j = 0; j < 8; ++j) {
            const f32x2 hh = pair_of(h1, j);
            const f32x2 d = __builtin_elementwise_fma(-hh, hh, f32x2{1.0f, 1.0f});
            set_pair(dz1, j, d);
            set_pair(acc, j, pair_of(acc, j) * d);
        }
#if RL_SPLIT_BULK_ROWS
        auto rows_of = [&](int which, int k, f32x4 (&out_)[4]) {
#pragma unroll
            for (int q = 0; q < 4; ++q) {
                if constexpr (TAIL_LDS) out_[q] = *reinterpret_cast<const f32x4*>(tv + (which * DA + k) * 16 + 4 * q);
                else
#pragma unroll
                    for (int e = 0; e < 4; ++e) out_[q][e] = which ? R_dW2[4 * q + e][k] : R_W2[4 * q + e][k];
            }
        };
#pragma unroll
        for (int k = 0; k < DA; ++k) {
            f32x4 wq[4], dq[4];
            rows_of(0, k, wq);
            rows_of(1, k, dq);
            f32x2 pa[2], pb[2];
            pa[0] = pa[1] = pb[0] = pb[1] = f32x2{0.0f, 0.0f};
#pragma unroll
            for (int j = 0; j < 8; ++j) {
                const int q = j >> 1, e = 2 * (j & 1);
                pa[j & 1] = __builtin_elementwise_fma(pair_of(h1, j), f32x2{dq[q][e], dq[q][e + 1]}, pa[j & 1]);
                pb[j & 1] = __builtin_elementwise_fma(pair_of(acc, j), f32x2{wq[q][e], wq[q][e + 1]}, pb[j & 1]);
// ... 191 lines not shown
            const float cc = floored[k] ? 0.0f : 4.0f * vv * (2.0f * vv - e) / ((2.0f * vv + e) * (2.0f * vv + e));
            myrow[N::LSTD + k] = cc * vc[N::LSTD + k] * ws;
        }
    }
    __syncthreads();
    float* row = a.partial + (size_t)blockIdx.x * P;
    for (int k = threadIdx.x; k < P; k += WAVES * WV) {
        float t = 0.0f;
#pragma unroll
        for (int w = 0; w < WAVES; ++w) t += reinterpret_cast<const float*>(smem)[w * P + k];
        row[k] = t;
    }
}

template <int DO, int DA>
__global__ void __launch_bounds__(4 * WV, 1) fvp_split64_kernel(Args a) {
    constexpr int HT = 2, HH = 64;
    using N = Net<DO, DA, HH>;
    constexpr int P = N::P;
    constexpr int WAVES = 4;
    constexpr int KB0 = (DO + 1 + 15) / 16;
    constexpr int KBH = 2 * HT;
    constexpr int O_DW0 = 0, O_DW1 = O_DW0 + HT * KB0, O_W1T = O_DW1 + HT * KBH, O_W1 = O_W1T + HT * KBH,
                  N_OPS = O_W1 + HT * KBH;
    constexpr int OPS_BYTES = N_OPS * 3 * WV * 16;
    constexpr int TAILV = HT * 16 * DA * 2 + HT * 16;
    constexpr int LAND64 = 2 * HH * TS * 4;
    constexpr int GMU_BYTES = TS * 8 * 4;
    constexpr int WAVE_BYTES = LAND64 + GMU_BYTES;
    constexpr int LDS_TOTAL = WAVES * WAVE_BYTES + OPS_BYTES + 2 * TAILV * 4;
    static_assert(DO + 1 <= 32 && DA <= 8, "two k-blocks of inputs + the bias slot; at most eight actions");
    static_assert(LDS_TOTAL >= WAVES * P * 4 && LDS_TOTAL <= 160 * 1024, "LDS budget; the fold rows alias everything");
    extern __shared__ __attribute__((aligned(16))) char smem[];
    const int wave = threadIdx.x / WV, lane = threadIdx.x % WV;
    const int lj = lane & 31, lh = lane >> 5;
    char* const land = smem + wave * WAVE_BYTES;
    float* const gmub = reinterpret_cast<float*>(land + LAND64);
    char* const ops = smem + WAVES * WAVE_BYTES;
    float* const tailv = reinterpret_cast<float*>(ops + OPS_BYTES);

    const int B = a.B;
    const int n_tiles = B / TS;
    const int wave_global = blockIdx.x * WAVES + wave;
    const int waves_total = gridDim.x * WAVES;

    auto fetch = [&](int tile, float (&xq)[KB0][8], float& wq) {
        const int b = tile * TS + lj;
        wq = a.weight[b];
#pragma unroll
        for (int kb = 0; kb < KB0; ++kb)
#pragma unroll
            for (int j = 0; j < 8; ++j) {
                const int d = 16 * kb + 8 * lh + j;
                const float v = a.obs[(size_t)(d < DO ? d : DO - 1) * B + b];
                xq[kb][j] = d < DO ? v : (d == DO ? 1.0f : 0.0f);
            }
    };
    auto fetch_acts = [&](int tile) {
        const float* src = a.acts + ((size_t)tile * (4 * 2 * HT) * WV + lane) * 4;
#pragma unroll
        for (int q = 0; q < 4 * 2 * HT; ++q)
            __builtin_amdgcn_global_load_lds((gptr_t)(src + q * WV * 4), (lptr_t)(land + q * WV * 16), 16, 0, 0);
    };
    float xb[KB0][8], xb_next[KB0][8];
    float wgt = 0.0f, wgt_next = 0.0f;
    if (wave_global < n_tiles) {
// ... 130 lines not shown
        f32x16 acc[HT], dh0[HT];
#pragma unroll
        for (int t = 0; t < HT; ++t)
#pragma unroll
            for (int r = 0; r < 16; ++r) acc[t][r] = 0.0f;
        chains(O_DW0, Xs, acc);
#pragma unroll
        for (int t = 0; t < HT; ++t) times_dtanh(acc[t], h0[t], dh0[t]);
        stage();
        {
            f32x4 bq[HT][4];
#pragma unroll
            for (int t = 0; t < HT; ++t)
#pragma unroll
                for (int q = 0; q < 4; ++q) bq[t][q] = *reinterpret_cast<const f32x4*>(tv + 2 * DA * HT * 16 + t * 16 + 4 * q);
#pragma unroll
            for (int t = 0; t < HT; ++t)
#pragma unroll
                for (int r = 0; r < 16; ++r) acc[t][r] = bq[t][r >> 2][r & 3];
        }
        chains(O_DW1, H0s, acc);
        stage();
        {
            Parts D0s[KBH];
#pragma unroll
            for (int t = 0; t < HT; ++t) {
                Parts tmp[2];
                split_frag(dh0[t], tmp);
                D0s[2 * t] = tmp[0]; D0s[2 * t + 1] = tmp[1];
            }
            chains(O_W1T, D0s, acc);
        }
        stage();
        const float c = wgt * a.inv_count;
        f32x16 dz1[HT], gz1[HT];
        float gmu[DA];
#pragma unroll
        for (int t = 0; t < HT; ++t)
#pragma unroll
            for (int j = 0; j < 8; ++j) {
                const f32x2 hh = pair_of(h1[t], j);
                const f32x2 d = __builtin_elementwise_fma(-hh, hh, f32x2{1.0f, 1.0f});
                set_pair(dz1[t], j, d);
                set_pair(acc[t], j, pair_of(acc[t], j) * d);
            }
#ifndef RL_ABL_THIN
#define RL_ABL_THIN 0
#endif
#if RL_ABL_THIN
#pragma unroll
        for (int k = 0; k < DA; ++k) gmu[k] = c * db2[k];
#pragma unroll
        for (int t = 0; t < HT; ++t) gz1[t] = acc[t];
        asm volatile("s_waitcnt lgkmcnt(0)" ::: "memory");
        fetch_acts(nxt);
#else
        auto rows_of = [&](int which, int k, f32x4 (&out_)[HT][4]) {
#pragma unroll
            for (int t = 0; t < HT; ++t)
#pragma unroll
                for (int q = 0; q < 4; ++q)
                    out_[t][q] = *reinterpret_cast<const f32x4*>(tv + ((which * DA + k) * HT + t) * 16 + 4 * q);
        };
#pragma unroll
        for (int k = 0; k < DA; ++k) {
            f32x4 wq[HT][4], dq[HT][4];
            rows_of(0, k, wq);
// ... 149 lines not shown
#pragma unroll
            for (int r = 0; r < 16; ++r) myrow[N::B1 + 32 * t + frag_unit(r, lh)] = b1s[t][r];
    }
#pragma unroll
    for (int k = 0; k < DA; ++k) myrow[N::W2 + lane * DA + k] = gW2u[k];
    if (lane == 0) {
#pragma unroll
        for (int k = 0; k < DA; ++k) {
            myrow[N::B2 + k] = b2s[k];
            const float vv = var_[k], e = 1e-8f;
            const float cc = floored[k] ? 0.0f : 4.0f * vv * (2.0f * vv - e) / ((2.0f * vv + e) * (2.0f * vv + e));
            myrow[N::LSTD + k] = cc * vc[N::LSTD + k] * ws;
        }
    }
    __syncthreads();
    float* row = a.partial + (size_t)blockIdx.x * P;
    for (int k = threadIdx.x; k < P; k += WAVES * WV) {
        float t = 0.0f;
#pragma unroll
        for (int w = 0; w < WAVES; ++w) t += reinterpret_cast<const float*>(smem)[w * P + k];
        row[k] = t;
    }
}

template <int DO, int DA>
static int launch64(const rl_policy_batch* g, const float* vec, void* ws, size_t ws_bytes, double* out, hipStream_t st) {
    using N = Net<DO, DA, 64>;
    constexpr int HT = 2, WAVES = 4;
    constexpr int KB0 = (DO + 1 + 15) / 16;
    constexpr int N_OPS = HT * KB0 + 3 * HT * 2 * HT;
    constexpr int LDS_BYTES = WAVES * (2 * 64 * TS * 4 + TS * 8 * 4) + N_OPS * 3 * WV * 16 + 2 * (HT * 16 * DA * 2 + HT * 16) * 4;
    Args a;
    a.B = g->n_samples; a.theta = g->theta; a.vec = vec; a.acts = g->activations; a.obs = g->obs; a.weight = g->weights;
    a.inv_count = g->inv_count; a.log_min_std = g->log_min_std;
    const int n_tiles = a.B / TS;
    int grid = (n_tiles + WAVES - 1) / WAVES;
    if (grid > 256) grid = 256;
    const size_t need = (size_t)grid * N::P * sizeof(float);
    if (ws_bytes < need) return set_error(RL_ERR_ARG, "policy pass workspace too small: %zu < %zu bytes", ws_bytes, need);
    a.partial = (float*)ws;
    auto kern = fvp_split64_kernel<DO, DA>;
    static bool attr_set = false;
    if (!attr_set) {
        hipError_t e = hipFuncSetAttribute(reinterpret_cast<const void*>(kern), hipFuncAttributeMaxDynamicSharedMemorySize,
                                           LDS_BYTES);
        if (e != hipSuccess) return set_error(RL_ERR_HIP, "hipFuncSetAttribute: %s", hipGetErrorString(e));
        attr_set = true;
    }
    hipLaunchKernelGGL(kern, dim3(grid), dim3(WAVES * WV), LDS_BYTES, st, a);
    int rc = check_launch("fvp_split64_kernel");
    if (rc) return rc;
    return launch_reduce_rows(a.partial, grid, N::P, out, st);
}

template <int DO, int DA, int WPS>
static int launch(const rl_policy_batch* g, const float* vec, void* ws, size_t ws_bytes, double* out, hipStream_t st) {
    using N = Net<DO, DA, H>;
    constexpr int WAVES = 4 * WPS;
    constexpr int KB0 = (DO + 1 + 15) / 16;
    constexpr int LDS_BYTES = WAVES * (LAND_BYTES + (WPS == 2 ? 2 * 3 * WV * 16 : 0) + (RL_SPLIT_ASM_DMA ? ((DO + 1 + 7) / 8) * WV * 16 : 0)) +
                              (WPS == 2 ? ops_bytes(KB0) : 0) +
                              ((WPS == 2 || DA > 2) ? 2 * (16 * DA * 2 + 16) * 4 : 0);
    Args a;
    a.B = g->n_samples; a.theta = g->theta; a.vec = vec; a.acts = g->activations; a.obs = g->obs; a.weight = g->weights;
    a.inv_count = g->inv_count; a.log_min_std = g->log_min_std;
    const int n_tiles = a.B / TS;
    int grid = (n_tiles + WAVES - 1) / WAVES;
    if (grid > 256) grid = 256;
    const size_t need = (size_t)grid * N::P * sizeof(float);
    if (ws_bytes < need) return set_error(RL_ERR_ARG, "policy pass workspace too small: %zu < %zu bytes", ws_bytes, need);
    a.partial = (float*)ws;
    auto kern = fvp_split_kernel<DO, DA, WPS>;
    static bool attr_set = false;
    if (!attr_set) {
        hipError_t e = hipFuncSetAttribute(reinterpret_cast<const void*>(kern), hipFuncAttributeMaxDynamicSharedMemorySize,
                                           LDS_BYTES);
        if (e != hipSuccess) return set_error(RL_ERR_HIP, "hipFuncSetAttribute: %s", hipGetErrorString(e));
        attr_set = true;
    }
    hipLaunchKernelGGL(kern, dim3(grid), dim3(WAVES * WV), LDS_BYTES, st, a);
    int rc = check_launch("fvp_split_kernel");
    if (rc) return rc;
    return launch_reduce_rows(a.partial, grid, N::P, out, st);
}

}

#define SPLIT_SHAPES(X) X(4, 1) X(6, 1) X(11, 1) X(13, 2) X(13, 1) X(20, 3) X(20, 6) X(21, 6)
#define SPLIT64_SHAPES(X) X(4, 1) X(6, 1) X(11, 1) X(13, 2) X(20, 3) X(20, 6) X(21, 6)
bool split_fvp_takes(const rl_policy_batch* g) {
    if (!g->activations || g->hidden2 != 0 || g->hidden0 != g->hidden1 || (g->hidden0 != 32 && g->hidden0 != 64) ||
        g->activation != RL_ACT_TANH || g->layer_activations != 0 || g->n_samples <= 0 || g->n_samples % TS != 0)
        return false;
    const int req = g->opts ? g->opts->fvp_split : 0;
    if (req == 1) return false;
    if (g->hidden0 == 64) {
        if (req == 2) return false;
#define SPLITCASE(DO, DA) if (g->obs_dim == DO && g->act_dim == DA) return true;
// ... 43 lines not shown
```

### rllab_amd/csrc/policy_splith_kernels.hip

```cpp
#include <hip/hip_runtime.h>
#include <cstdlib>
#include "../../include/rllab_amd.h"
#include "capi_util.h"
#include "policy_mfma.h"
#include "lds_tr_image.h"

namespace rl {

int launch_reduce_rows(const float* partial, int rows, int cols, double* out, hipStream_t st);

namespace splith {

typedef _Float16 f16;
typedef __attribute__((ext_vector_type(8))) _Float16 f16x8;
typedef __attribute__((ext_vector_type(4))) _Float16 f16x4;
typedef __attribute__((ext_vector_type(2))) _Float16 f16x2;
typedef __attribute__((ext_vector_type(2))) float f32x2;
typedef __attribute__((ext_vector_type(4))) float f32x4;
typedef __attribute__((address_space(1))) const void* gptr_t;
typedef __attribute__((address_space(3))) void* lptr_t;

struct Args {
    int B;
    const float* theta;
    const float* vec;
    const float* acts;
    const float* obs;
    const float* weight;
    const float* xmax;
    float inv_count;
    float log_min_std;
    float* partial;
};

struct PB { f16x8 hi, lo; };
struct PA { f16x8 hi, lo, hs; };

#ifndef RL_ABL_FETCH
#define RL_ABL_FETCH 0
#endif
#ifndef RL_ABL_MFMA
#define RL_ABL_MFMA 0
#endif
#ifndef RL_ABL_SPLIT
#define RL_ABL_SPLIT 0
#endif
#ifndef RL_ABL_TRANSPOSE
#define RL_ABL_TRANSPOSE 0
#endif

__device__ __forceinline__ f32x16 mf(f16x8 a, f16x8 b, f32x16 c) {
#if RL_ABL_MFMA
    asm volatile("" : "+v"(c) : "v"(a), "v"(b));
    return c;
#else
    return __builtin_amdgcn_mfma_f32_32x32x16_f16(a, b, c, 0, 0, 0);
#endif
}
__device__ __forceinline__ f32x16 mm_ab(const PA& A, const PB& b, f32x16 c) {
    c = mf(A.hs, b.lo, c);
    c = mf(A.lo, b.hi, c);
    c = mf(A.hi, b.hi, c);
    return c;
// ... 254 lines not shown
        m[i] = v;
    }
}
__host__ __device__ constexpr int ceil_log2(int n) { return n <= 1 ? 0 : n <= 2 ? 1 : n <= 4 ? 2 : 3; }

constexpr int H = 32;
constexpr int LAND_BYTES = 2 * H * TS * 4;
constexpr int ops_count(int kb0) { return kb0 + 6; }
constexpr int ops_bytes(int kb0) { return ops_count(kb0) * 3 * WV * 16; }
#ifndef RL_SPLITH_TWO_ACC
#define RL_SPLITH_TWO_ACC 0
#endif
#ifndef RL_SPLITH_TWO_ACC_W0
#define RL_SPLITH_TWO_ACC_W0 0
#endif
constexpr float XT_SCALE = 256.0f;

template <int DO, int DA, int WPS>
__global__ void __launch_bounds__(4 * WPS * WV, 1) fvp_splith_kernel(Args a) {
    using N = Net<DO, DA, H>;
    constexpr int P = N::P;
    constexpr int WAVES = 4 * WPS;
    constexpr int KB0 = (DO + 1 + 15) / 16;
    constexpr int N_OPS = ops_count(KB0), OPS_BYTES = ops_bytes(KB0);
    constexpr int TAILV = 16 * DA * 2 + 16;
    constexpr int SPILL_BYTES = 2 * lds_tr::TR_PART_BYTES;
    constexpr int XPIECES = (DO + 1 + 7) / 8;
    constexpr int XLAND_BYTES = XPIECES * WV * 16;
    constexpr int WAVE_BYTES = LAND_BYTES + SPILL_BYTES + XLAND_BYTES;
    constexpr int LDS_TOTAL = WAVES * WAVE_BYTES + OPS_BYTES + 2 * TAILV * 4 + WAVES * 5 * 4;
    static_assert(DO + 1 <= 32 && (DA <= 2 || WPS == 1), "two k-blocks of inputs + the bias slot; thin heads at two per SIMD");
    static_assert(LDS_TOTAL >= WAVES * P * 4 && LDS_TOTAL <= 160 * 1024, "LDS budget; the fold rows alias the landing zones");
    extern __shared__ __attribute__((aligned(16))) char smem[];
    const int wave = threadIdx.x / WV, lane = threadIdx.x % WV;
    const int lj = lane & 31, lh = lane >> 5;
    char* const land = smem + wave * WAVE_BYTES;
    char* const spill = land + LAND_BYTES;
    char* const xland = spill + SPILL_BYTES;
    char* const tr_w = spill + lds_tr::tr_store_lane(lane);
    const char* const tr_r = spill + lds_tr::tr_read_lane(lane);
    char* const ops = smem + WAVES * WAVE_BYTES;
    float* const tailv = reinterpret_cast<float*>(ops + OPS_BYTES);
    float* const red = tailv + 2 * TAILV;

    const int B = a.B;
    const int n_tiles = B / TS;
    const int wave_global = blockIdx.x * WAVES + wave;
    const int waves_total = gridDim.x * WAVES;

    const unsigned xland_lds = __builtin_amdgcn_readfirstlane((unsigned)(size_t)(lptr_t)xland);
    auto fetch = [&](int tile) {
#pragma unroll
        for (int p = 0; p < XPIECES; ++p) {
            const int d = 8 * p + (lane >> 3);
            const float* g = (d < DO ? a.obs + (size_t)d * B : a.weight) + tile * TS + 4 * (lane & 7);
            asm volatile("s_mov_b32 m0, %1\n\tglobal_load_lds_dwordx4 %0, off" :: "v"(g), "s"(xland_lds + p * (WV * 16)) : "memory");
        }
    };
    const unsigned land_lds = __builtin_amdgcn_readfirstlane((unsigned)(size_t)(lptr_t)land);
    auto fetch_acts = [&](int tile) {
        const float* src = a.acts + ((size_t)tile * 8 * WV + lane) * 4;
        asm volatile("s_mov_b32 m0, %2\n\t"
                     "global_load_lds_dwordx4 %0, off\n\t"
                     "global_load_lds_dwordx4 %0, off offset:1024\n\t"
                     "global_load_lds_dwordx4 %0, off offset:2048\n\t"
                     "global_load_lds_dwordx4 %0, off offset:3072\n\t"
                     "s_mov_b32 m0, %3\n\t"
                     "global_load_lds_dwordx4 %1, off\n\t"
                     "global_load_lds_dwordx4 %1, off offset:1024\n\t"
                     "global_load_lds_dwordx4 %1, off offset:2048\n\t"
                     "global_load_lds_dwordx4 %1, off offset:3072"
                     :: "v"(src), "v"(src + 4 * WV * 4), "s"(land_lds), "s"(land_lds + 4096u) : "memory");
    };
    if (wave_global < n_tiles) {
        fetch(wave_global);
        fetch_acts(wave_global);
    }
    asm volatile("" ::: "memory");

    const float* __restrict__ th = a.theta;
    const float* __restrict__ vc = a.vec;
    float db2[DA], fkS[DA], var_[DA];
    bool floored[DA];
    float fkmax = 0.0f;
#pragma unroll
    for (int k = 0; k < DA; ++k) {
        const float raw = th[N::LSTD + k];
        floored[k] = raw < a.log_min_std;
        const float ls = fmaxf(raw, a.log_min_std);
        var_[k] = __expf(2.0f * ls);
        fkS[k] = 2.0f / (2.0f * var_[k] + 1e-8f) * a.inv_count;
        fkmax = fmaxf(fkmax, fkS[k]);
    }
    float mx[5];
    block_maxima<N, WAVES * WV>(th, vc, red, mx);
    const Scales S = make_scales<5, ceil_log2(DA)>(*a.xmax, mx[0], mx[1], mx[2], mx[3], mx[4], fkmax);
#pragma unroll
    for (int k = 0; k < DA; ++k) {
        fkS[k] *= S.eg2;
        db2[k] = vc[N::B2 + k] * S.s1;
    }

    for (int o = wave; o < N_OPS; o += WAVES) {
        float t[8];
#pragma unroll
        for (int j = 0; j < 8; ++j) {
            if (o < KB0) {
                const int d = 16 * o + 8 * lh + j;
                t[j] = d < DO ? vc[N::W0 + d * H + lj] * S.sv0 : (d == DO ? vc[N::B0 + lj] * S.sv0b : 0.0f);
            } else {
                const int q = o - KB0, kb = q & 1, u = frag_unit(8 * kb + j, lh);
                t[j] = q < 2 ? vc[N::W1 + u * H + lj] * S.s1
                     : q < 4 ? th[N::W1 + u * H + lj] * S.sw1
                             : th[N::W1 + lj * H + u] * S.sw1;
            }
        }
        const PA im = image8(t);
        *reinterpret_cast<f16x8*>(ops + ((o * 3 + 0) * WV + lane) * 16) = im.hi;
        *reinterpret_cast<f16x8*>(ops + ((o * 3 + 1) * WV + lane) * 16) = im.lo;
        *reinterpret_cast<f16x8*>(ops + ((o * 3 + 2) * WV + lane) * 16) = im.hs;
    }
    for (int e = threadIdx.x; e < 2 * 16; e += WAVES * WV) {
        const int hh = e / 16, r = e % 16, u = frag_unit(r, hh);
        float* tv = tailv + hh * TAILV;
// ... 106 lines not shown
        }
        stage();
        f32x16 dz1, gz1;
        float gmu[DA];
#pragma unroll
        for (int j = 0; j < 8; ++j) {
            const f32x2 hh = pair_of(h1, j);
            const f32x2 d = __builtin_elementwise_fma(-hh, hh, f32x2{1.0f, 1.0f});
            set_pair(dz1, j, d);
            set_pair(acc, j, pair_of(acc, j) * d);
        }
        auto rows_of = [&](int which, int k, f32x4 (&out_)[4]) {
#pragma unroll
            for (int q = 0; q < 4; ++q) out_[q] = *reinterpret_cast<const f32x4*>(tv + (which * DA + k) * 16 + 4 * q);
        };
#pragma unroll
        for (int k = 0; k < DA; ++k) {
            f32x4 wq[4], dq[4];
            rows_of(0, k, wq);
            rows_of(1, k, dq);
            f32x2 pa[2], pb[2];
            pa[0] = pa[1] = pb[0] = pb[1] = f32x2{0.0f, 0.0f};
#pragma unroll
            for (int j = 0; j < 8; ++j) {
                const int q = j >> 1, e = 2 * (j & 1);
                pa[j & 1] = __builtin_elementwise_fma(pair_of(h1, j), f32x2{dq[q][e], dq[q][e + 1]}, pa[j & 1]);
                pb[j & 1] = __builtin_elementwise_fma(pair_of(acc, j), f32x2{wq[q][e], wq[q][e + 1]}, pb[j & 1]);
            }
            const f32x2 pd = (pa[0] + pb[0]) + (pa[1] + pb[1]);
            const float dmu = db2[k] + half_sum_swap(pd[0] + pd[1]);
            gmu[k] = wgt * (dmu * fkS[k]);
        }
        if (lh == 0) {
            wsum += wgt * a.inv_count;
#pragma unroll
            for (int k = 0; k < DA; ++k) gb2[k] += gmu[k];
        }
        stage();
        {
            f32x2 g[8];
#pragma unroll
            for (int j = 0; j < 8; ++j) g[j] = f32x2{0.0f, 0.0f};
#pragma unroll
            for (int k = 0; k < DA; ++k) {
                f32x4 wq[4];
                rows_of(0, k, wq);
                const f32x2 gk = {gmu[k], gmu[k]};
#pragma unroll
                for (int j = 0; j < 8; ++j) {
                    const int q = j >> 1, e = 2 * (j & 1);
                    g[j] = __builtin_elementwise_fma(f32x2{wq[q][e], wq[q][e + 1]}, gk, g[j]);
                    const f32x2 w2 = __builtin_elementwise_fma(pair_of(h1, j), gk, f32x2{gW2l[2 * j][k], gW2l[2 * j + 1][k]});
                    gW2l[2 * j][k] = w2[0]; gW2l[2 * j + 1][k] = w2[1];
                }
            }
#pragma unroll
            for (int j = 0; j < 8; ++j) {
                const f32x2 gz = g[j] * pair_of(dz1, j);
                set_pair(gz1, j, gz);
                const f32x2 b1n = f32x2{gb1l[2 * j], gb1l[2 * j + 1]} + gz;
                gb1l[2 * j] = b1n[0]; gb1l[2 * j + 1] = b1n[1];
            }
        }
        stage();
        opcur = op(KB0 + 4);
        __builtin_amdgcn_sched_barrier(0);
        PB G1s[2], H0t[2], G1t[2];
// ... 87 lines not shown
            const float cc = floored[k] ? 0.0f : 4.0f * vv * (2.0f * vv - e) / ((2.0f * vv + e) * (2.0f * vv + e));
            myrow[N::LSTD + k] = cc * vc[N::LSTD + k] * ws;
        }
    }
    __syncthreads();
    float* row = a.partial + (size_t)blockIdx.x * P;
    for (int k = threadIdx.x; k < P; k += WAVES * WV) {
        float t = 0.0f;
#pragma unroll
        for (int w = 0; w < WAVES; ++w) t += reinterpret_cast<const float*>(smem)[w * P + k];
        row[k] = t;
    }
}

template <int DO, int DA>
__global__ void __launch_bounds__(4 * WV, 1) fvp_splith64_kernel(Args a) {
    constexpr int HT = 2, HH = 64;
    using N = Net<DO, DA, HH>;
    constexpr int P = N::P;
    constexpr int WAVES = 4;
    constexpr int KB0 = (DO + 1 + 15) / 16;
    constexpr int KBH = 2 * HT;
    constexpr int O_DW0 = 0, O_DW1 = O_DW0 + HT * KB0, O_W1T = O_DW1 + HT * KBH, O_W1 = O_W1T + HT * KBH,
                  N_OPS = O_W1 + HT * KBH;
    constexpr int OPS_BYTES = N_OPS * 3 * WV * 16;
    constexpr int TAILV = HT * 16 * DA * 2 + HT * 16;
    constexpr int LAND64 = 2 * HH * TS * 4;
    constexpr int GMU_BYTES = TS * 8 * 4;
    constexpr int WAVE_BYTES = LAND64 + GMU_BYTES;
    constexpr int LDS_TOTAL = WAVES * WAVE_BYTES + OPS_BYTES + 2 * TAILV * 4 + WAVES * 5 * 4;
    static_assert(DO + 1 <= 32 && DA <= 8, "two k-blocks of inputs + the bias slot; at most eight actions");
    static_assert(LDS_TOTAL >= WAVES * P * 4 && LDS_TOTAL <= 160 * 1024, "LDS budget; the fold rows alias everything");
    extern __shared__ __attribute__((aligned(16))) char smem[];
    const int wave = threadIdx.x / WV, lane = threadIdx.x % WV;
    const int lj = lane & 31, lh = lane >> 5;
    char* const land = smem + wave * WAVE_BYTES;
    float* const gmub = reinterpret_cast<float*>(land + LAND64);
    char* const ops = smem + WAVES * WAVE_BYTES;
    float* const tailv = reinterpret_cast<float*>(ops + OPS_BYTES);
    float* const red = tailv + 2 * TAILV;

    const int B = a.B;
    const int n_tiles = B / TS;
    const int wave_global = blockIdx.x * WAVES + wave;
    const int waves_total = gridDim.x * WAVES;

    auto fetch = [&](int tile, float (&xq)[KB0][8], float& wq) {
        const int b = tile * TS + lj;
        wq = a.weight[b];
#pragma unroll
        for (int kb = 0; kb < KB0; ++kb)
#pragma unroll
            for (int j = 0; j < 8; ++j) {
                const int d = 16 * kb + 8 * lh + j;
                xq[kb][j] = a.obs[(size_t)(d < DO ? d : DO - 1) * B + b];
            }
    };
    auto fetch_acts = [&](int tile) {
        const float* src = a.acts + ((size_t)tile * (4 * 2 * HT) * WV + lane) * 4;
#pragma unroll
        for (int q = 0; q < 4 * 2 * HT; ++q)
            __builtin_amdgcn_global_load_lds((gptr_t)(src + q * WV * 4), (lptr_t)(land + q * WV * 16), 16, 0, 0);
    };
    float xb[KB0][8], xb_next[KB0][8];
    float wgt = 0.0f, wgt_next = 0.0f;
    if (wave_global < n_tiles) {
        fetch(wave_global, xb_next, wgt_next);
        fetch_acts(wave_global);
    }
    asm volatile("" ::: "memory");

    const float* __restrict__ th = a.theta;
    const float* __restrict__ vc = a.vec;
    float db2[DA], fkS[DA], var_[DA];
    bool floored[DA];
    float fkmax = 0.0f;
#pragma unroll
    for (int k = 0; k < DA; ++k) {
        const float raw = th[N::LSTD + k];
        floored[k] = raw < a.log_min_std;
        const float ls = fmaxf(raw, a.log_min_std);
        var_[k] = __expf(2.0f * ls);
        fkS[k] = 2.0f / (2.0f * var_[k] + 1e-8f) * a.inv_count;
        fkmax = fmaxf(fkmax, fkS[k]);
    }
    float mx[5];
    block_maxima<N, WAVES * WV>(th, vc, red, mx);
    const Scales S = make_scales<6, ceil_log2(DA)>(*a.xmax, mx[0], mx[1], mx[2], mx[3], mx[4], fkmax);
#pragma unroll
    for (int k = 0; k < DA; ++k) {
        fkS[k] *= S.eg2;
        db2[k] = vc[N::B2 + k] * S.s1;
    }

    for (int o = wave; o < N_OPS; o += WAVES) {
        float tv8[8];
#pragma unroll
        for (int j = 0; j < 8; ++j) {
            if (o < O_DW1) {
                const int t = o / KB0, kb0 = o % KB0, i = 32 * t + lj, d = 16 * kb0 + 8 * lh + j;
                tv8[j] = d < DO ? vc[N::W0 + d * HH + i] * S.sv0 : (d == DO ? vc[N::B0 + i] * S.sv0b : 0.0f);
            } else {
                const int q = o - O_DW1, fam = q / (HT * KBH), r_ = q % (HT * KBH), t = r_ / KBH, kbg = r_ % KBH;
                const int i = 32 * t + lj, u = 32 * (kbg >> 1) + frag_unit(8 * (kbg & 1) + j, lh);
                tv8[j] = fam == 0 ? vc[N::W1 + u * HH + i] * S.s1
                       : fam == 1 ? th[N::W1 + u * HH + i] * S.sw1
                                  : th[N::W1 + i * HH + u] * S.sw1;
            }
        }
        const PA im = image8(tv8);
        *reinterpret_cast<f16x8*>(ops + ((o * 3 + 0) * WV + lane) * 16) = im.hi;
        *reinterpret_cast<f16x8*>(ops + ((o * 3 + 1) * WV + lane) * 16) = im.lo;
        *reinterpret_cast<f16x8*>(ops + ((o * 3 + 2) * WV + lane) * 16) = im.hs;
    }
    for (int e = threadIdx.x; e < 2 * HT * 16; e += WAVES * WV) {
        const int hh = e / (HT * 16), t = (e / 16) % HT, r = e % 16, u = 32 * t + frag_unit(r, hh);
// ... 126 lines not shown
                const f32x2 hh = pair_of(h1[t], j);
                const f32x2 d = __builtin_elementwise_fma(-hh, hh, f32x2{1.0f, 1.0f});
                set_pair(dz1[t], j, d);
                set_pair(acc[t], j, pair_of(acc[t], j) * d);
            }
        auto rows_of = [&](int which, int k, f32x4 (&out_)[HT][4]) {
#pragma unroll
            for (int t = 0; t < HT; ++t)
#pragma unroll
                for (int q = 0; q < 4; ++q)
                    out_[t][q] = *reinterpret_cast<const f32x4*>(tv + ((which * DA + k) * HT + t) * 16 + 4 * q);
        };
#pragma unroll
        for (int k = 0; k < DA; ++k) {
            f32x4 wq[HT][4], dq[HT][4];
            rows_of(0, k, wq);
            rows_of(1, k, dq);
            f32x2 pa[HT], pb[HT];
#pragma unroll
            for (int t = 0; t < HT; ++t) pa[t] = pb[t] = f32x2{0.0f, 0.0f};
#pragma unroll
            for (int j = 0; j < 8; ++j)
#pragma unroll
                for (int t = 0; t < HT; ++t) {
                    const int q = j >> 1, e = 2 * (j & 1);
                    pa[t] = __builtin_elementwise_fma(pair_of(h1[t], j), f32x2{dq[t][q][e], dq[t][q][e + 1]}, pa[t]);
                    pb[t] = __builtin_elementwise_fma(pair_of(acc[t], j), f32x2{wq[t][q][e], wq[t][q][e + 1]}, pb[t]);
                }
            const f32x2 pd = (pa[0] + pb[0]) + (pa[1] + pb[1]);
            const float dmu = db2[k] + half_sum_swap(pd[0] + pd[1]);
            gmu[k] = wgt * (dmu * fkS[k]);
        }
        if (lh == 0) {
            wsum += wgt * a.inv_count;
#pragma unroll
            for (int k = 0; k < DA; ++k) { gb2[k] += gmu[k]; gmub[lj * 8 + k] = gmu[k]; }
        }
        {
            f32x2 g[HT][8];
#pragma unroll
            for (int t = 0; t < HT; ++t)
#pragma unroll
                for (int j = 0; j < 8; ++j) g[t][j] = f32x2{0.0f, 0.0f};
#pragma unroll
            for (int k = 0; k < DA; ++k) {
                f32x4 wq[HT][4];
                rows_of(0, k, wq);
                const f32x2 gk = {gmu[k], gmu[k]};
#pragma unroll
                for (int t = 0; t < HT; ++t)
#pragma unroll
                    for (int j = 0; j < 8; ++j) {
                        const int q = j >> 1, e = 2 * (j & 1);
                        g[t][j] = __builtin_elementwise_fma(f32x2{wq[t][q][e], wq[t][q][e + 1]}, gk, g[t][j]);
                    }
            }
#pragma unroll
            for (int t = 0; t < HT; ++t)
#pragma unroll
                for (int j = 0; j < 8; ++j) {
                    const f32x2 gz = g[t][j] * pair_of(dz1[t], j);
                    set_pair(gz1[t], j, gz);
                    const f32x2 b1n = f32x2{gb1l[t][2 * j], gb1l[t][2 * j + 1]} + gz;
                    gb1l[t][2 * j] = b1n[0]; gb1l[t][2 * j + 1] = b1n[1];
                }
        }
        wave_sync();
// ... 95 lines not shown
            if (d < DO) myrow[N::W0 + d * HH + 32 * t + lj] = gW0[t][r] * S.u0;
            else if (d == DO) myrow[N::B0 + 32 * t + lj] = gW0[t][r] * S.u0b;
        }
    if (lj == 0) {
#pragma unroll
        for (int t = 0; t < HT; ++t)
#pragma unroll
            for (int r = 0; r < 16; ++r) myrow[N::B1 + 32 * t + frag_unit(r, lh)] = b1s[t][r] * S.u1;
    }
#pragma unroll
    for (int k = 0; k < DA; ++k) myrow[N::W2 + lane * DA + k] = gW2u[k] * S.u1;
    if (lane == 0) {
#pragma unroll
        for (int k = 0; k < DA; ++k) {
            myrow[N::B2 + k] = b2s[k] * S.u1;
            const float vv = var_[k], e = 1e-8f;
            const float cc = floored[k] ? 0.0f : 4.0f * vv * (2.0f * vv - e) / ((2.0f * vv + e) * (2.0f * vv + e));
            myrow[N::LSTD + k] = cc * vc[N::LSTD + k] * ws;
        }
    }
    __syncthreads();
    float* row = a.partial + (size_t)blockIdx.x * P;
    for (int k = threadIdx.x; k < P; k += WAVES * WV) {
        float t = 0.0f;
#pragma unroll
        for (int w = 0; w < WAVES; ++w) t += reinterpret_cast<const float*>(smem)[w * P + k];
        row[k] = t;
    }
}

static Args make_args(const rl_policy_batch* g, const float* vec) {
    Args a;
    a.B = g->n_samples; a.theta = g->theta; a.vec = vec; a.acts = g->activations; a.obs = g->obs; a.weight = g->weights;
    a.xmax = g->obs_absmax; a.inv_count = g->inv_count; a.log_min_std = g->log_min_std; a.partial = nullptr;
    return a;
}

template <int DO, int DA>
static int launch32(const rl_policy_batch* g, const float* vec, void* ws, size_t ws_bytes, double* out, hipStream_t st) {
    using N = Net<DO, DA, H>;
    constexpr int WPS = DA <= 2 ? 2 : 1;
    constexpr int WAVES = 4 * WPS;
    constexpr int KB0 = (DO + 1 + 15) / 16;
    constexpr int LDS_BYTES = WAVES * (LAND_BYTES + 2 * 2 * WV * 16 + ((DO + 1 + 7) / 8) * WV * 16) + ops_bytes(KB0) +
                              2 * (16 * DA * 2 + 16) * 4 + WAVES * 5 * 4;
    Args a = make_args(g, vec);
    const int n_tiles = a.B / TS;
    int grid = (n_tiles + WAVES - 1) / WAVES;
    if (grid > 256) grid = 256;
    const size_t need = (size_t)grid * N::P * sizeof(float);
    if (ws_bytes < need) return set_error(RL_ERR_ARG, "policy pass workspace too small: %zu < %zu bytes", ws_bytes, need);
    a.partial = (float*)ws;
    auto kern = fvp_splith_kernel<DO, DA, WPS>;
    static bool attr_set = false;
    if (!attr_set) {
        hipError_t e = hipFuncSetAttribute(reinterpret_cast<const void*>(kern), hipFuncAttributeMaxDynamicSharedMemorySize,
                                           LDS_BYTES);
        if (e != hipSuccess) return set_error(RL_ERR_HIP, "hipFuncSetAttribute: %s", hipGetErrorString(e));
        attr_set = true;
    }
    hipLaunchKernelGGL(kern, dim3(grid), dim3(WAVES * WV), LDS_BYTES, st, a);
    int rc = check_launch("fvp_splith_kernel");
    if (rc) return rc;
    return launch_reduce_rows(a.partial, grid, N::P, out, st);
}

template <int DO, int DA>
// ... 60 lines not shown
```

### rllab_amd/csrc/process_kernels.hip

```cpp
#include <hip/hip_runtime.h>
#include <stdlib.h>
#include "../../include/rllab_amd.h"
#include "capi_util.h"

namespace rl {

constexpr int PS_EW = 32;
constexpr int PS_KB = 32;
constexpr int MAX_DO = 21;

template <class F>
__device__ __forceinline__ void lfb_features(int Do, const float* __restrict__ obs, size_t plane, size_t off,
                                             int tin, F&& emit) {
    for (int d = 0; d < Do; ++d) {
        double o = (double)obs[(size_t)d * plane + off];
        o = fmin(fmax(o, -10.0), 10.0);
        emit(d, o);
        emit(Do + d, o * o);
    }
    const double al = (double)tin / 100.0;
    emit(2 * Do, al);
    emit(2 * Do + 1, al * al);
    emit(2 * Do + 2, al * al * al);
    emit(2 * Do + 3, 1.0);
// ... 221 lines not shown
    if (threadIdx.x < ST_NCOLS) {
        const int c = threadIdx.x;
        double v = sm[0][c];
        for (int w = 1; w < ST_BLOCK / 64; ++w)
            v = (c < ST_NSUM) ? v + sm[w][c] : (stat_is_max(c) ? fmax(v, sm[w][c]) : fmin(v, sm[w][c]));
        partial[(size_t)blockIdx.x * ST_NCOLS + c] = v;
    }
}

__global__ void __launch_bounds__(64) stats_reduce_kernel(const double* __restrict__ partial, int rows,
                                                          double* __restrict__ out) {
    const int c = blockIdx.x, lane = threadIdx.x;
    const bool is_sum = c < ST_NSUM, is_max = stat_is_max(c);
    double v = is_sum ? 0.0 : (is_max ? -INFINITY : INFINITY);
    for (int r = lane; r < rows; r += 64) {
        const double w = partial[(size_t)r * ST_NCOLS + c];
        v = is_sum ? v + w : (is_max ? fmax(v, w) : fmin(v, w));
    }
#pragma unroll
    for (int o = 32; o > 0; o >>= 1) {
        const double w = __shfl_xor(v, o, 64);
        v = is_sum ? v + w : (is_max ? fmax(v, w) : fmin(v, w));
    }
    if (lane == 0) out[c] = v;
}

__global__ void __launch_bounds__(256)
adv_finish_kernel(size_t B, const float* __restrict__ adv_in, const uint8_t* __restrict__ valid, double mean,
                  double denom, double shift, float* __restrict__ adv_out) {
    const size_t b = (size_t)blockIdx.x * 256 + threadIdx.x;
    if (b >= B) return;
    const double a = ((double)adv_in[b] - mean) / denom + shift;
    adv_out[b] = valid[b] ? (float)a : 0.0f;
}

constexpr int NE_TILE = 64;
constexpr int NE_WAVES = 4;

template <int FB>
__global__ void __launch_bounds__(NE_WAVES * 64)
lfb_normal_eq_kernel(size_t B, int Do, const float* __restrict__ obs, const int32_t* __restrict__ tin,
                     const float* __restrict__ ret, const uint8_t* __restrict__ valid,
                     double* __restrict__ partial) {
    constexpr int FE = 8 * FB;
    constexpr int STR = FE + 2;
    extern __shared__ __attribute__((aligned(16))) double sm[];
    const int wave = threadIdx.x >> 6, lane = threadIdx.x & 63;
    double* tile = sm + (size_t)wave * NE_TILE * STR;
    const int bi = lane >> 3, bj = lane & 7;
    const int F = 2 * Do + 4;
    double acc[FB][FB];
#pragma unroll
    for (int r = 0; r < FB; ++r)
#pragma unroll
        for (int c = 0; c < FB; ++c) acc[r][c] = 0.0;
    const size_t n_tiles = (B + NE_TILE - 1) / NE_TILE;
    for (size_t tl = (size_t)blockIdx.x * NE_WAVES + wave; tl < n_tiles; tl += (size_t)gridDim.x * NE_WAVES) {
        const size_t b = tl * NE_TILE + lane;
        const bool use = (b < B) && valid[b];
        double* row = tile + (size_t)lane * STR;
        if (use) {
            lfb_features(Do, obs, B, b, tin[b], [&](int f, double v) { row[f] = v; });
            row[F] = (double)ret[b];
            for (int f = F + 1; f < FE; ++f) row[f] = 0.0;
        } else {
            for (int f = 0; f < FE; ++f) row[f] = 0.0;
// ... 190 lines not shown
extern "C" size_t rl_process_workspace_bytes(int obs_dim) {
    const int FE = (2 * obs_dim + 5 <= 32) ? 32 : 64;
    const size_t a = (size_t)1024 * ST_NCOLS * sizeof(double);
    const size_t b = (size_t)512 * FE * FE * sizeof(double);
    return a > b ? a : b;
}

extern "C" int rl_sample_stats(size_t n_samples, const float* returns, const double* baselines,
                               const float* advantages, const float* undiscounted, const int32_t* tin,
                               const uint8_t* valid, double ret_shift, double und_shift, const float* progress,
                               int n_cols, void* workspace, size_t workspace_bytes, double* out, void* stream) {
    if (n_samples == 0 || !returns || !advantages || !undiscounted || !tin || !valid || !workspace || !out ||
        (progress && n_cols <= 0))
        return set_error(RL_ERR_ARG, "rl_sample_stats: bad argument");
    int grid = (int)((n_samples + ST_BLOCK * 8 - 1) / (ST_BLOCK * 8));
    if (grid > 1024) grid = 1024;
    if (grid < 1) grid = 1;
    if (workspace_bytes < (size_t)grid * ST_NCOLS * sizeof(double))
        return set_error(RL_ERR_ARG, "rl_sample_stats: workspace too small");
    hipLaunchKernelGGL(sample_stats_kernel, dim3(grid), dim3(ST_BLOCK), 0, (hipStream_t)stream, n_samples, returns,
                       baselines, advantages, undiscounted, tin, valid, ret_shift, und_shift, progress, n_cols,
                       (double*)workspace);
    hipLaunchKernelGGL(stats_reduce_kernel, dim3(ST_NCOLS), dim3(64), 0, (hipStream_t)stream,
                       (const double*)workspace, grid, out);
    return check_launch("sample_stats_kernel");
}

extern "C" int rl_adv_finish(size_t n_samples, const float* adv_in, const uint8_t* valid, double mean,
                             double denom, double shift, float* adv_out, void* stream) {
    if (n_samples == 0 || !adv_in || !valid || !adv_out) return set_error(RL_ERR_ARG, "rl_adv_finish: bad argument");
    hipLaunchKernelGGL(adv_finish_kernel, dim3((unsigned)((n_samples + 255) / 256)), dim3(256), 0,
                       (hipStream_t)stream, n_samples, adv_in, valid, mean, denom, shift, adv_out);
    return check_launch("adv_finish_kernel");
}

extern "C" int rl_lfb_normal_eq(size_t n_samples, int obs_dim, const float* obs, const int32_t* tin,
                                const float* returns, const uint8_t* valid, void* workspace,
                                size_t workspace_bytes, double* out, int variant, void* stream) {
    if (n_samples == 0 || obs_dim <= 0 || obs_dim > MAX_DO || !obs || !tin || !returns || !valid || !workspace || !out)
        return set_error(RL_ERR_ARG, "rl_lfb_normal_eq: bad argument (obs_dim <= %d)", MAX_DO);
    const int F = 2 * obs_dim + 4;
    const int FE = (F + 1 <= 32) ? 32 : 64;
    const size_t n_tiles = (n_samples + NE_TILE - 1) / NE_TILE;
    int grid = (int)((n_tiles + NE_WAVES - 1) / NE_WAVES);
    if (grid > 512) grid = 512;
    if (workspace_bytes < (size_t)grid * FE * FE * sizeof(double))
        return set_error(RL_ERR_ARG, "rl_lfb_normal_eq: workspace too small");
    const size_t lds = (size_t)NE_WAVES * NE_TILE * (FE + 2) * sizeof(double);
    hipError_t e = hipSuccess;
    const bool valu = variant == 1;
    if (FE == 32 && !valu) {
        static bool set = false;
        if (!set) { e = hipFuncSetAttribute(reinterpret_cast<const void*>(lfb_normal_eq_mfma_kernel<32>), hipFuncAttributeMaxDynamicSharedMemorySize, (int)lds); set = true; }
        hipLaunchKernelGGL(lfb_normal_eq_mfma_kernel<32>, dim3(grid), dim3(NE_WAVES * 64), lds, (hipStream_t)stream, n_samples,
                           obs_dim, obs, tin, returns, valid, (double*)workspace);
    } else if (!valu) {
        static bool set = false;
        if (!set) { e = hipFuncSetAttribute(reinterpret_cast<const void*>(lfb_normal_eq_mfma_kernel<64>), hipFuncAttributeMaxDynamicSharedMemorySize, (int)lds); set = true; }
        hipLaunchKernelGGL(lfb_normal_eq_mfma_kernel<64>, dim3(grid), dim3(NE_WAVES * 64), lds, (hipStream_t)stream, n_samples,
                           obs_dim, obs, tin, returns, valid, (double*)workspace);
    } else if (FE == 32) {
        static bool set32 = false;
        if (!set32) { e = hipFuncSetAttribute(reinterpret_cast<const void*>(lfb_normal_eq_kernel<4>), hipFuncAttributeMaxDynamicSharedMemorySize, (int)lds); set32 = true; }
        hipLaunchKernelGGL(lfb_normal_eq_kernel<4>, dim3(grid), dim3(NE_WAVES * 64), lds, (hipStream_t)stream, n_samples,
                           obs_dim, obs, tin, returns, valid, (double*)workspace);
    } else {
// ... 11 lines not shown
```

### rllab_amd/policies/fused_ops.py

```python
import ctypes
import math
import os

import torch

from rllab_amd import _lib
from rllab_amd.core.serializable import Serializable
from rllab_amd.misc.device_io import read_async
from rllab_amd.sampler import dist as D


class FusedGaussianMLPOps(object):
    device_line_search = True

    def __init__(self, policy):
        self.policy = policy
        self.layout = policy.kernel_layout()
        assert self.layout is not None
        self.dims = (policy.obs_dim, policy.action_dim) + self.layout.hidden3
        self.n_kernel = self.layout.P_pad
        self.wide_kernels = self.layout.wide or (policy.obs_dim, policy.action_dim) not in self.NARROW_PAIRS
        self._ws = None
        self._loss_cache = None
        self._bound = {}
# ... 7 lines not shown

    @_epoch.setter
    def _epoch(self, value):
        self.policy._raw_writes = value

    NARROW_PAIRS = ((4, 1), (6, 1), (11, 1), (13, 2), (20, 3), (20, 6), (21, 6))

    @staticmethod
    def supported(policy):
        layout = policy.kernel_layout() if hasattr(policy, "kernel_layout") else None
        return layout is not None

    def accepts(self, inputs):
        return inputs[4].numel() == self.dims[1] and inputs[0].is_cuda

    def _workspace(self, device):
        if self._ws is None or self._ws.device != device:
            n = _lib.lib.rl_policy_workspace_bytes(*self.dims)
            self._ws = torch.empty(n, dtype=torch.uint8, device=device)
        return self._ws

    def _batch(self, inputs):
        self.layout.theta()
        key = tuple(id(t) for t in inputs)
        hit = self._bound.get(key)
        if hit is not None:
            return hit
        obs, act, adv, old_mean, old_log_std, w, inv_count = inputs
        theta = self.layout.theta()
        keep = [t.contiguous() for t in (obs, act, adv, old_mean, old_log_std.reshape(-1).float(), w, theta)]
        obs, act, adv, old_mean, old_ls, w, theta = keep
        assert theta.data_ptr() == self.layout.theta().data_ptr()
        pol = self.policy
        inv = float(inv_count)
        b = _lib.PolicyBatch(
            n_samples=obs.shape[-1], obs_dim=self.dims[0], act_dim=self.dims[1], hidden0=self.dims[2],
            hidden1=self.dims[3], hidden2=self.dims[4], inv_count=inv,
            log_min_std=math.log(pol.min_std) if pol.min_std is not None else -1e30,
            theta=theta.data_ptr(), obs=obs.data_ptr(), actions=act.data_ptr(), advantages=adv.data_ptr(),
            old_means=old_mean.data_ptr(), old_log_std=old_ls.data_ptr(), weights=w.data_ptr(),
            layer_activations=self.layout.layer_activations,
            opts=_lib.launch_opts())
        if len(self._bound) >= 2:
            self._bound.clear()
        self._bound[key] = (b, keep + list(inputs), inv)
        return self._bound[key]

    def release(self):
        self._bound.clear()
        self._loss_cache = None
        self._acts = None
        self._acts_tag = None

    def _loss_record(self, tag, out, inv, rows=None):
        if rows is None:
            rows = D.all_gather_rows(out)
        c = dict(tag=tag, out=out, rows=rows, inv=inv, dev=None, read=read_async(rows), host=None)
        self._loss_cache = c
        return c

    def _loss_eval(self, inputs):
        tag = self._eval_point(inputs)
        c = self._loss_cache
        if c is not None and c["tag"] == tag:
            return c
        b, keep, inv = self._batch(inputs)
        ws = self._workspace(keep[0].device)
        out = torch.empty(4, dtype=torch.float64, device=keep[0].device)
        _lib.check(_lib.lib.rl_policy_loss_kl(ctypes.byref(b), _lib.ptr(ws), ws.numel(), _lib.ptr(out),
                                              _lib.stream_ptr()), "rl_policy_loss_kl")
        return self._loss_record(tag, out, inv)

    @staticmethod
    def _resolve(c):
        if c["host"] is None:
            h = c["read"].get().reshape(-1, 4)
            sums = h[:, :3].sum(axis=0) * c["inv"]
            c["host"] = (float(sums[0]), float(sums[1]), float(sums[2]), float(h[:, 3].max()))
        return c["host"]

    def loss_stats(self, inputs):
        c = self._loss_eval(inputs)
        if c["dev"] is None:
            c["dev"] = torch.as_tensor(self._resolve(c), dtype=torch.float64, device=c["out"].device)
        return c["dev"]

    def loss_stats_host(self, inputs):
        return self._resolve(self._loss_eval(inputs))

    def loss_and_kl(self, inputs):
        s = self.loss_stats_host(inputs)
        return -s[0], s[1]

    def loss_stats_deferred(self, inputs):
        c = self._loss_eval(inputs)
        return lambda: self._resolve(c)

    def loss_and_kl_deferred(self, inputs):
        c = self._loss_eval(inputs)

        def get():
            s = self._resolve(c)
            return -s[0], s[1]
        get.record = c
        return get

    def _eval_point(self, inputs):
        return (tuple(id(t) for t in inputs), self.policy.flat_params._version, self._epoch)

    def loss_grad(self, inputs, vpg=False, keep_activations=False, with_loss=False):
# ... 36 lines not shown
            b.activations = None
            b.obs_absmax = None
        return self._mask_frozen(self.layout.unpack(D.update_sum_(out)))

    @property
    def masks_frozen(self):
        return self._frozen_index() is not None

    def _frozen_index(self):
        if not hasattr(self, "_frozen_idx"):
            pol = self.policy
            tr = pol._flat_index(trainable=True)
            if tr is None:
                self._frozen_idx = None
            else:
                keep = torch.ones(pol.flat_params.numel(), dtype=torch.bool, device=pol.flat_params.device)
                keep[tr] = False
                self._frozen_idx = torch.nonzero(keep).reshape(-1)
        return self._frozen_idx

    def _mask_frozen(self, g):
        idx = self._frozen_index()
        if idx is not None:
            g.index_fill_(0, idx, 0.0)
        return g

    def value_and_grad(self, inputs, penalty=0.0, vpg=False):
        assert not (vpg and penalty), "the log-likelihood objective has no KL penalty"
        b, keep, inv = self._batch(inputs)
        dev = keep[0].device
        ws = self._workspace(dev)
        grad = torch.empty(self.n_kernel, dtype=torch.float64, device=dev)
        out4 = torch.empty(4, dtype=torch.float64, device=dev)
        self._acts_tag = None
        b.activations = None
        b.kl_penalty = float(penalty)
        try:
            _lib.check(_lib.lib.rl_policy_grad_loss(ctypes.byref(b), int(bool(vpg)), _lib.ptr(ws), ws.numel(),
                                                    _lib.ptr(grad), _lib.ptr(out4), _lib.stream_ptr()),
                       "rl_policy_grad_loss")
        finally:
            b.kl_penalty = 0.0
        packed = torch.cat([out4[:3], self.layout.unpack(grad)])
        D.all_reduce_sum_(packed)
        idx = self.policy._flat_index(trainable=True)
        host = packed.cpu().numpy()
        g = host[3:] if idx is None else host[3:][idx.cpu().numpy()]
        if vpg:
            return float(-host[2] * inv), g.copy()
        return float((-host[0] + penalty * host[1]) * inv), g.copy()

    def loglik_loss(self, inputs):
        return -self.loss_stats_host(inputs)[2]

    def _fvp_into(self, b, ws, vec32, out, inputs=None):
        cached = inputs is not None and self._acts_tag is not None and self._acts_tag == self._eval_point(inputs)
        b.activations = self._acts.data_ptr() if cached else None
        b.obs_absmax = self._absmax.data_ptr() if cached and self._absmax is not None else None
        b.opts = _lib.launch_opts()
        try:
            _lib.check(_lib.lib.rl_policy_fvp(ctypes.byref(b), _lib.ptr(vec32), _lib.ptr(ws), ws.numel(),
                                              _lib.ptr(out), _lib.stream_ptr()), "rl_policy_fvp")
        finally:
            b.activations = None
            b.obs_absmax = None
        out = D.update_sum_(out)
# ... 93 lines not shown
        theta = self.policy.flat_params
        assert prev32.dtype == torch.float32 and step.dtype == torch.float64 and theta.is_contiguous()
        _lib.check(_lib.lib.rl_line_search_point(theta.numel(), _lib.ptr(prev32), _lib.ptr(step), float(ratio),
                                                 _lib.ptr(theta.detach()), _lib.stream_ptr()),
                   "rl_line_search_point")
        self._epoch += 1

    def line_search_device(self, inputs, prev32, step, ratios, max_constraint, before_record):
        b, keep, inv = self._batch(inputs)
        dev = keep[0].device
        ws = self._workspace(dev)
        K = len(ratios)
        theta = self.policy.flat_params.detach()
        assert prev32.dtype == torch.float32 and step.dtype == torch.float64 and theta.is_contiguous() and K >= 1
        buf = getattr(self, "_ls_buf", None)
        if buf is None or buf.numel() != 3 + 4 * K or buf.device != dev:
            buf = self._ls_buf = torch.empty(3 + 4 * K, dtype=torch.float64, device=dev)
        buf.zero_()
        state, gate = buf[:2 + 4 * K], buf[2 + 4 * K:].view(torch.int32)
        outs = torch.empty((K, 4), dtype=torch.float64, device=dev)
        n, st = theta.numel(), _lib.stream_ptr()
        brows = before_record["rows"]
        _lib.check(_lib.lib.rl_line_search_point(n, _lib.ptr(prev32), _lib.ptr(step), float(ratios[0]), _lib.ptr(theta),
                                                 st), "rl_line_search_point")
        self._epoch += 1
        b.gate = gate.data_ptr()
        try:
            for k in range(K):
                self.layout.theta()
                _lib.check(_lib.lib.rl_policy_loss_kl(ctypes.byref(b), _lib.ptr(ws), ws.numel(), _lib.ptr(outs[k]),
                                                      st), "rl_policy_loss_kl")
                rows = D.all_gather_rows(outs[k])
                nxt = float(ratios[k + 1]) if k + 1 < K else 0.0
                _lib.check(_lib.lib.rl_line_search_decide(
                    rows.shape[0], _lib.ptr(rows), _lib.ptr(brows), inv, float(max_constraint), k, _lib.ptr(state),
                    _lib.ptr(gate), n, _lib.ptr(prev32), _lib.ptr(step), nxt, _lib.ptr(theta), st),
                    "rl_line_search_decide")
                self._epoch += 1
        finally:
            b.gate = None
        return dict(read=read_async(state), K=K, inv=inv, state=state, world=brows.shape[0])

    def line_search_resolve(self, rec, inputs):
        h = rec["read"].get()
        K, inv = rec["K"], rec["inv"]
        accepted = int(h[1]) if h[0] != 0.0 else None
        n_eval = K if accepted is None else accepted + 1
        sums = h[2:2 + 4 * K].reshape(K, 4)
        evals = [(-(sums[k, 0] * inv), sums[k, 1] * inv) for k in range(n_eval)]
        last = n_eval - 1
        host = (float(sums[last, 0] * inv), float(sums[last, 1] * inv), float(sums[last, 2] * inv), float(sums[last, 3]))
        rows = torch.zeros((rec["world"], 4), dtype=torch.float64, device=rec["state"].device)
        rows[0].copy_(rec["state"][2 + 4 * last:6 + 4 * last])
        self._loss_cache = dict(tag=self._eval_point(inputs), out=rows[0], rows=rows, inv=inv, dev=None, read=None,
                                host=host)
        return accepted, [(float(l), float(c)) for l, c in evals]

    def hvp_approach(self):
        return FusedFisherHvp(self)


class FusedFisherHvp(Serializable):

    def __init__(self, ops=None):
        self.ops = ops
        self.target = None
        self.reg_coeff = None

    def update_opt(self, f, target, inputs, reg_coeff):
        self.target, self.reg_coeff = target, reg_coeff

    def build_eval(self, inputs, trainable_index=None):
        ops, reg = self.ops, self.reg_coeff
        n = self.target.flat_params.numel()

        def eval(x):
            if trainable_index is None:
                full = x
# ... 9 lines not shown
```

### rllab_amd/sampler/base.py

```python
import numpy as np
import torch

import rllab_amd.misc.logger as logger
from rllab_amd import _lib
from rllab_amd.misc import special
from rllab_amd.misc.device_io import read_async, upload_async
from rllab_amd.sampler import dist as D
from rllab_amd.sampler.trajectories import PathList, Trajectories


class Sampler(object):
    def start_worker(self):
        raise NotImplementedError

    def obtain_samples(self, itr):
        raise NotImplementedError

    def process_samples(self, itr, paths):
        raise NotImplementedError

    def shutdown_worker(self):
        raise NotImplementedError


# ... 8 lines not shown

        def rows(planes):
            x = planes.reshape(planes.shape[0], -1).t()
            return x if sel is None else x[sel]

        def vec(plane):
            x = plane.reshape(-1)
            return x if sel is None else x[sel]
        if key == "observations":
            val = rows(tr.obs)
        elif key == "actions":
            val = rows(tr.actions)
        elif key == "rewards":
            val = vec(tr.rewards)
        elif key == "returns":
            val = vec(tr.returns)
        elif key == "advantages":
            val = vec(tr.advantages)
        elif key == "agent_infos" and getattr(tr, "categorical", False):
            val = dict(prob=rows(tr.means))
        elif key == "agent_infos":
            mean = rows(tr.means)
            val = dict(mean=mean, log_std=rows(tr.log_std_planes) if tr.log_std_planes is not None
                       else tr.log_std.unsqueeze(0).expand_as(mean))
        else:
            val = dict()
        self[key] = val
        return val


_WS = {}


def _workspace(device, obs_dim):
    key = (device, obs_dim)
    if key not in _WS:
        n = _lib.lib.rl_process_workspace_bytes(int(obs_dim))
        _WS[key] = torch.empty(n, dtype=torch.uint8, device=device)
    return _WS[key]


(_COUNT, _RET, _RET2, _BASE, _BASE2, _RES, _RES2, _ADV, _ADV2, _NPATH, _UND, _UND2, _DISC, _PROG, _PROG2,
 _ADVMIN, _UNDMAX, _UNDMIN, _PROGMAX, _PROGMIN) = range(20)
_N_SUM = 15


def path_scan(traj, whole_paths, coeffs=None, want_values=True):
    dev = traj.device
    T, N = traj.T, traj.N
    tin = torch.empty((T, N), dtype=torch.int32, device=dev)
    valid = torch.empty((T, N), dtype=torch.uint8, device=dev)
    values = torch.empty((T, N), dtype=torch.float64, device=dev) if (want_values and coeffs is not None) else None
    cf = None
    if coeffs is not None:
        if torch.is_tensor(coeffs) and coeffs.device == dev:
            cf = coeffs.to(torch.float64).contiguous()
        else:
            cf = upload_async(np.asarray(coeffs, dtype=np.float64), torch.float64, dev)
        assert cf.numel() == 2 * traj.obs_dim + 4
    obs_dim = traj.obs_dim if (cf is not None or traj.obs_dim <= 21) else 0
    _lib.check(_lib.lib.rl_path_scan(T, N, obs_dim, _lib.ptr(traj.dones), _lib.ptr(traj.obs) if obs_dim else None, _lib.ptr(cf),
                                     int(bool(whole_paths)), _lib.ptr(tin), _lib.ptr(valid), _lib.ptr(values),
                                     _lib.stream_ptr()), "rl_path_scan")
    return tin, valid.view(torch.bool), values


def merge_stats(st):
    if not D.is_distributed():
        return st
    return torch.as_tensor(fold_stats(D.all_gather_rows(st).cpu().numpy()), device=st.device)


def fold_stats(rows):
    rows = np.asarray(rows, dtype=np.float64).reshape(-1, 20)
    out = rows[:, :].sum(axis=0)
    for c in (_ADVMIN, _UNDMIN, _PROGMIN):
        out[c] = rows[:, c].min()
    for c in (_UNDMAX, _PROGMAX):
        out[c] = rows[:, c].max()
    return out


_SHIFT = dict(ret=0.0, und=0.0)


def process_dense(algo, itr, traj, log=True):
    dev = traj.device
    T, N = traj.T, traj.N
    B = T * N
    gamma, lam = float(algo.discount), float(algo.gae_lambda)
    baseline = algo.baseline
    dense_lfb = hasattr(baseline, "dense_coeffs") and traj.obs_dim <= 21
    preset_valid = traj.valid
    tin, valid, base = path_scan(traj, algo.whole_paths, baseline.dense_coeffs() if dense_lfb else None)
    if preset_valid is not None:
        valid = preset_valid
    traj.valid, traj.tin = valid, tin
    if not dense_lfb:
        if hasattr(baseline, "predict_dense"):
            base = baseline.predict_dense(traj)
        else:
            base = _predict_by_path(baseline, traj)
    adv = torch.empty((T, N), dtype=torch.float32, device=dev)
    ret = torch.empty((T, N), dtype=torch.float32, device=dev)
    und = torch.empty((T, N), dtype=torch.float32, device=dev)
    base_c = base.contiguous() if base is not None else None
    _lib.check(_lib.lib.rl_gae(T, N, _lib.ptr(traj.rewards), _lib.ptr(base_c), _lib.ptr(traj.dones),
                               gamma, lam, _lib.ptr(adv), _lib.ptr(ret), _lib.ptr(und), _lib.stream_ptr()), "rl_gae")
    traj.returns = ret
    traj.baselines = base

    valid_u8 = valid.contiguous().view(torch.uint8)
    ws = _workspace(dev, traj.obs_dim)
    st = torch.empty(20, dtype=torch.float64, device=dev)
    inner = getattr(algo, "env", None)
    while hasattr(inner, "wrapped_env"):
        inner = inner.wrapped_env
    prog_idx = getattr(inner, "progress_obs_index", None)
    prog = traj.obs[prog_idx % traj.obs_dim] if prog_idx is not None else None
    _lib.check(_lib.lib.rl_sample_stats(B, _lib.ptr(ret), _lib.ptr(base_c), _lib.ptr(adv), _lib.ptr(und),
                                        _lib.ptr(tin), _lib.ptr(valid_u8), _SHIFT["ret"], _SHIFT["und"],
                                        _lib.ptr(prog), N, _lib.ptr(ws), ws.numel(), _lib.ptr(st),
                                        _lib.stream_ptr()), "rl_sample_stats")
    dense_fit = hasattr(baseline, "fit_dense")
    pdist = algo.policy.distribution
    categorical = getattr(traj, "categorical", False)
    if categorical and D.is_distributed():
        raise NotImplementedError("a categorical batch is processed in one process on one GPU (not sharded over ranks)")
    if categorical and type(baseline).__name__ == "GaussianMLPBaseline":
        raise NotImplementedError("GaussianMLPBaseline on a categorical batch: its fused regressor is built for the "
                                  "continuous envs' observations; use LinearFeatureBaseline or ZeroBaseline")
    if dense_fit and log:
        logger.log("fitting baseline...")
    if dense_fit and D.is_distributed() and hasattr(baseline, "normal_eq_dense"):
        packed = baseline.normal_eq_dense(traj)
        rows = D.all_gather_rows(torch.cat([st, packed]))
        stats_read = read_async(rows[:, :st.numel()].contiguous())
        baseline.fit_from_packed(rows[:, st.numel():].sum(dim=0), 2 * traj.obs_dim + 4)
        dense_fit_done = True
    elif categorical:
        ent_sum = (pdist.entropy_sym(dict(prob=traj.means.to(torch.float64)), axis=0) * valid.to(torch.float64)).sum()
        stats_read = read_async(torch.cat([st, ent_sum.reshape(1)]).reshape(1, -1))
        dense_fit_done = False
    else:
        stats_read = read_async(D.all_gather_rows(st))
        dense_fit_done = False
    ls_read = read_async(traj.log_std) if (traj.log_std is not None and traj.log_std_planes is None) else None
    if dense_fit and not dense_fit_done:
        baseline.fit_dense(traj, all_reduce=D.all_reduce_sum_ if D.is_distributed() else None)
    if categorical:
        host = stats_read.get().reshape(-1)
        s, ent_sum_host = fold_stats(host[:20]), float(host[20])
    else:
        s = fold_stats(stats_read.get())
    traj.log_std_host = ls_read.get().astype(np.float64) if ls_read is not None else None
    cnt, n_paths = s[_COUNT], s[_NPATH]
    traj.count = float(cnt)

    def moments(i_sum, i_sq, n):
        m = s[i_sum] / n
        return m, max(s[i_sq] / n - m * m, 0.0)
    m_ret, var_y = moments(_RET, _RET2, cnt)
    _, var_pred = moments(_BASE, _BASE2, cnt)
    _, var_res = moments(_RES, _RES2, cnt)
    if np.isclose(var_y, 0):
        ev = 0 if var_pred > 0 else 1
    else:
        ev = 1 - var_res / (var_y + 1e-8)

    mean_a, denom, shift = 0.0, 1.0, 0.0
    if algo.center_adv:
        mean_a, var_a = moments(_ADV, _ADV2, cnt)
        denom = float(np.sqrt(var_a)) + 1e-8
    if algo.positive_adv:
        shift = -((s[_ADVMIN] - mean_a) / denom) + 1e-8
    adv_out = torch.empty((T, N), dtype=torch.float32, device=dev)
    _lib.check(_lib.lib.rl_adv_finish(B, _lib.ptr(adv), _lib.ptr(valid_u8), float(mean_a), float(denom),
                                      float(shift), _lib.ptr(adv_out), _lib.stream_ptr()), "rl_adv_finish")
    traj.advantages = adv_out
    paths = PathList(traj)
    samples_data = SamplesData(_traj=traj, paths=paths)
    if hasattr(algo, "prefetch_update") and traj.obs.is_cuda and getattr(algo, "_update_follows", False):
        algo.prefetch_update(samples_data)

    if prog is not None and n_paths > 0:
        m_prog, var_prog = moments(_PROG, _PROG2, n_paths)
        traj.progress_stats = (float(m_prog), float(s[_PROGMAX]), float(s[_PROGMIN]), float(np.sqrt(var_prog)))
    m_und_s, var_und = moments(_UND, _UND2, n_paths) if n_paths > 0 else (np.nan, np.nan)
    mean_und = m_und_s + _SHIFT["und"]
    _SHIFT["ret"], _SHIFT["und"] = float(m_ret + _SHIFT["ret"]), (float(mean_und) if n_paths > 0 else 0.0)

    if categorical:
        ent = ent_sum_host / cnt
    elif traj.log_std_planes is not None and hasattr(pdist, "entropy_sym"):
        e = pdist.entropy_sym(dict(log_std=traj.log_std_planes.to(torch.float64)), axis=0)
        (es,) = D.sums((e * valid.to(torch.float64)).sum())
        ent = float(es) / cnt
    elif traj.log_std_host is not None and hasattr(pdist, "entropy"):
        ent = float(np.asarray(pdist.entropy(dict(log_std=traj.log_std_host[None, :]))).reshape(-1)[0])
    elif traj.log_std is not None and hasattr(pdist, "entropy_sym"):
        ent = float(pdist.entropy_sym(dict(log_std=traj.log_std.to(torch.float64)), axis=0))
    else:
        ent = float("nan")

    if not dense_fit:
        if log:
            logger.log("fitting baseline...")
        if hasattr(baseline, 'fit_with_samples'):
            baseline.fit_with_samples(paths, samples_data)
        else:
            baseline.fit(paths)
    if log:
        logger.log("fitted")
        logger.record_tabular('Iteration', itr)
        logger.record_tabular('AverageDiscountedReturn', float(s[_DISC] / n_paths) if n_paths > 0 else np.nan)
        logger.record_tabular('AverageReturn', float(mean_und))
# ... 71 lines not shown
```

### rllab_amd/sampler/trajectories.py

```python
import numpy as np
import torch


class Trajectories(object):
    def __init__(self, obs, actions, means, log_std, rewards, dones, max_path_length, log_std_planes=None,
                 categorical=False, prev_action_info=False):
        self.obs, self.actions, self.means = obs, actions, means
        self.categorical = bool(categorical)
        self.prev_action_info = bool(prev_action_info)
        self.log_std, self.rewards, self.dones = log_std, rewards, dones
        self.log_std_planes = log_std_planes
        self.max_path_length = max_path_length
        self.T, self.N = rewards.shape
        self.obs_dim, self.act_dim = obs.shape[0], actions.shape[0]
        self._seg = None
        self.valid = None
        self.advantages = None
        self.returns = None
        self.baselines = None
        self.tin = None
        self.progress_stats = None
        self.count = None
        self.log_std_host = None

    @property
    def device(self):
        return self.rewards.device

    _PLANES = ("obs", "actions", "means", "log_std_planes")
    _ROWS = ("rewards", "dones")

    @classmethod
    def concat(cls, chunks):
        if len(chunks) == 1:
            return chunks[0]
        first = chunks[0]
        cat = lambda name, dim: (None if getattr(first, name) is None
                                 else torch.cat([getattr(c, name) for c in chunks], dim=dim))
        return cls(cat("obs", 1), cat("actions", 1), cat("means", 1), first.log_std, cat("rewards", 0), cat("dones", 0),
                   first.max_path_length, log_std_planes=cat("log_std_planes", 1), categorical=first.categorical,
                   prev_action_info=first.prev_action_info)

    def first_steps(self, steps):
        if steps >= self.T:
            return self
        cut3 = lambda x: None if x is None else x[:, :steps, :].contiguous()
        return Trajectories(cut3(self.obs), cut3(self.actions), cut3(self.means), self.log_std,
                            self.rewards[:steps].contiguous(), self.dones[:steps].contiguous(), self.max_path_length,
                            log_std_planes=cut3(self.log_std_planes), categorical=self.categorical,
                            prev_action_info=self.prev_action_info)

    @property
    def B(self):
        return self.T * self.N

    def segments(self):
# ... 92 lines not shown
```

### rllab_amd/sampler/vectorized_sampler.py

```python
import math
import os
import time

import torch

import rllab_amd.misc.logger as logger
from rllab_amd import _lib
from rllab_amd.sampler import dist as D
from rllab_amd.sampler.base import BaseSampler
from rllab_amd.sampler.trajectories import PathList, Trajectories


class VectorizedSampler(BaseSampler):
    def __init__(self, algo, n_envs=None, seed=None, use_graph=True):
        super(VectorizedSampler, self).__init__(algo)
        self.n_envs = n_envs
        self.seed = seed
        self.use_graph = use_graph
        self.vec_env = None
        self.last_sample_time = None
        self.last_num_samples = None

    def start_worker(self):
        algo = self.algo
# ... 23 lines not shown
        if not self._takes_fused_rollout(policy):
            raise NotImplementedError("recurrent policy without a sampling path: this executor has no recurrent rollout")

    def sampling_path(self, policy):
        ve = self.vec_env
        if self._takes_fused_rollout(policy):
            return "fused rollout kernel (one launch per batch of %d envs)" % ve.n, None
        if ve is None:
            return "none (no executor yet)", None
        if not getattr(ve, "graphable", True) and ve.position_ids is not None:
            why = "Box2DEnv(position_only=True) under NormalizedEnv(normalize_obs / normalize_reward): the running " \
                  "estimates are over the kept rows, the fused rollout's over the full observation"
        elif not getattr(ve, "graphable", True):
            why = "NormalizedEnv(normalize_obs / normalize_reward): the running estimates ride in the fused rollout of the " \
                  "(32, 32) / (64, 64) policies only (and not together with obs_noise)"
        else:
            layout = policy.kernel_layout() if hasattr(policy, "kernel_layout") else None
            dual = policy.rollout_networks() if hasattr(policy, "rollout_networks") else None
            if layout is not None or dual is not None:
                why = "the policy's weight fragments do not fit the 160 KB LDS of a CU next to this env's observation tile"
            elif getattr(policy, "state_dependent_std", False):
                why = "the policy's two networks have no rollout kernel (each: two or three tanh layers of at most 128 units)"
            elif hasattr(policy, "why_no_kernel_layout"):
                why = policy.why_no_kernel_layout()
            else:
                why = "%s is not a GaussianMLPPolicy" % type(policy).__name__
        graph = self.use_graph and getattr(ve, "graphable", True) and not os.environ.get("RLLAB_NO_GRAPH") \
            and hasattr(policy, "recorded_log_std")
        name = "per-transition loop (%s), one policy evaluation + one env-step launch per step" % (
            "hipGraph replay" if graph else "eager")
        return name, why

    def shutdown_worker(self):
        if self.vec_env is not None:
            self.vec_env.terminate()

    def __getstate__(self):
        d = dict(self.__dict__)
        d["vec_env"] = None
        d.pop("_step_graph", None)
        d.pop("_prefetched", None)
        d.pop("_carry_obs", None)
        d.pop("_launch_start", None)
        return d

    def _takes_fused_rollout(self, policy):
        ve = self.vec_env
        if ve is None:
            return False
        if hasattr(ve, "takes_rollout_of"):
            return ve.takes_rollout_of(policy)
        return (hasattr(policy, "kernel_layout") and policy.kernel_layout() is not None) or \
            (hasattr(policy, "rollout_networks") and policy.rollout_networks() is not None)

    def prefetch(self, itr):
        policy = self.algo.policy
        pre = getattr(self, "_prefetched", None)
        if pre is not None and pre[0] == itr and hasattr(policy, "param_version") and pre[1] == policy.param_version():
            return
        self._drop_prefetched()
        if not hasattr(policy, "param_version") or not self._takes_fused_rollout(policy):
            return
        if getattr(self.vec_env, "stateful_rollouts", False):
            return
        counter = self.vec_env.step_counter
        first = self._rollout_chunk(policy, self.algo.max_path_length, True)
        self._prefetched = (itr, policy.param_version(), first, counter)

    def _drop_prefetched(self):
        pre = getattr(self, "_prefetched", None)
        self._prefetched = None
        if pre is not None and self.vec_env is not None:
            self.vec_env.step_counter = pre[3]

    def obtain_samples(self, itr):
        algo = self.algo
        policy = algo.policy
        pre = getattr(self, "_prefetched", None)
        first = None
        if pre is not None:
            if pre[0] == itr and pre[1] is not None and pre[1] == policy.param_version():
                first = pre[2]
                self._prefetched = None
            else:
                self._drop_prefetched()
        t_start = time.time()
        if first is None:
            first = self._launch(policy, algo.max_path_length, True)
        traj = self._meet_batch_size(policy, first)
        self.last_num_samples = traj.B
        self.last_sample_time = time.time() - t_start
        return PathList(traj)

    def _rollout_chunk(self, policy, steps, first):
        graphable = getattr(self.vec_env, "graphable", True)
        if self._takes_fused_rollout(policy):
            return self.vec_env.rollout(policy, steps, reset_at_start=first)
        if self.use_graph and graphable and not os.environ.get("RLLAB_NO_GRAPH") and hasattr(policy, "recorded_log_std"):
            try:
                return self._stepwise_rollout_graph(policy, steps, first)
            except RuntimeError as err:
                logger.log("hipGraph capture of the per-transition loop failed (%s); using the eager loop"
                           % str(err).split("\n")[0])
                self.use_graph = False
                self._step_graph = None
                torch.cuda.synchronize()
        return self._stepwise_rollout(policy, steps, first)

    MAX_STALLED_CHUNKS = 8

    def _launch(self, policy, steps, first):
        v = self.vec_env
        self._launch_start = None
        if getattr(v, "stateful_rollouts", False):
            self._launch_start = (v.snapshot(), getattr(self, "_carry_obs", None), bool(first))
        return self._rollout_chunk(policy, steps, first)

    def _commit_first_steps(self, policy, chunk, steps):
        start = getattr(self, "_launch_start", None)
        if start is None:
            return
        v = self.vec_env
        snap, carry, first = start
        v.restore(snap)
        self._carry_obs = carry
# ... 202 lines not shown
```

Measured before the change: 274.4 million.

## Compute batch scalars on device and defer baseline fit to a side stream

Advantage normalisation scalars (mean, denom, shift, 1/count) are now computed by a device kernel and consumed through device pointers by the policy, line-search and advantage-finish kernels. This removes the host round-trip on the sample stats before the update can be prefetched. The linear feature baseline fit is deferred and launched on a side stream after the next rollout is enqueued, so it overlaps sampling. The cost is more code paths, extra synchronisation with events, and a fallback guard that excludes distributed, categorical, recurrent and some split-FVP configurations.

Measured after the change: 275.7 million, median of 6. About the same (+0.4%).

```diff
diff --git a/include/rllab_amd.h b/include/rllab_amd.h
--- a/include/rllab_amd.h
+++ b/include/rllab_amd.h
@@ -344,6 +344,18 @@
 int rl_adv_finish(size_t n_samples, const float* adv_in, const uint8_t* valid, double mean, double denom,
                   double shift, float* adv_out, void* stream);
 
+typedef struct rl_batch_scalars_t {
+    double mean, denom, shift;
+    double inv_count;
+    float inv_count_f32;
+    float reserved_pad;
+} rl_batch_scalars_t;
+
+int rl_batch_scalars(const double* stats20, int center_adv, int positive_adv, rl_batch_scalars_t* out, void* stream);
+
+int rl_adv_finish_dev(size_t n_samples, const float* adv_in, const uint8_t* valid, const rl_batch_scalars_t* scalars,
+                      float* adv_out, float* weight_out, void* stream);
+
 int rl_lfb_normal_eq(size_t n_samples, int obs_dim, const float* obs, const int32_t* tin,
                      const float* returns, const uint8_t* valid, void* workspace, size_t workspace_bytes,
                      double* out, int variant, void* stream);
@@ -381,6 +393,7 @@
     int32_t reserved_pad;
     const int32_t* gate;
     float* obs_absmax;
+    const float* inv_count_dev;
 } rl_policy_batch;
 
 enum rl_activation { RL_ACT_TANH = 0, RL_ACT_RECTIFY = 1, RL_ACT_IDENTITY = 2 };
@@ -492,6 +505,9 @@
 int rl_line_search_decide(int rows, const double* sums, const double* before, double inv_count, double max_constraint,
                           int candidate, double* state, int32_t* gate, int n, const float* prev, const double* step,
                           double next_ratio, float* theta, void* stream);
+int rl_line_search_decide_dev(int rows, const double* sums, const double* before, const double* inv_count_dev,
+                              double max_constraint, int candidate, double* state, int32_t* gate, int n, const float* prev,
+                              const double* step, double next_ratio, float* theta, void* stream);
 
 int rl_adam_step(int n, float* theta, const double* grad, double* m, double* v, double a_t, double beta1,
                  double beta2, double epsilon, void* stream);
diff --git a/profiles/make_index.py b/profiles/make_index.py
--- a/profiles/make_index.py
+++ b/profiles/make_index.py
@@ -29,6 +29,9 @@
     ("r06_c20_splith_ab_wide.txt", "fvp() of (20, 6) on (32, 32), 512 k samples: bf16 three-way against f16 two-way at one wavefront per SIMD", "tools/exp/r06_call20.sh"),
     ("r06_splith_*.csv", "SQ counter passes / FETCH_SIZE / kernel stats of the bf16 and the f16 split products, (32, 32) at 2.048 M and (64, 64) at 512 k samples", "tools/exp/r06_call19.sh"),
     ("curves/r06_splith_*", "learning under the f16 two-way and the bf16 three-way split products, same seeds; 1500-iteration soak", "tools/exp/r06_splith_curves.sh"),
+    ("process_device_scalars_ab_bench.jsonl", "headline bench lines of the parent tree, this tree, this tree with RLLAB_PROCESS_HOST_STATS=1 and with RLLAB_FIT_SIDE_STREAM=0, interleaved five times in one call",
+     "python bench.py --gpus 1 --steps 20 --warmup 3 per line (ms_per_step, phase_ms and roofline.avg_launch_ms kept)"),
+    ("process_device_scalars_c5_*.csv", "kernel stats / PMC passes of C5's per-GPU shard", "profiles/run_profile.sh process_device_scalars cheetah1024_trpo_gae process_device_scalars_c5"),
     ("fvp_lds_tr_ab_product.txt", "fvp() of the parent and the new library swapped in alternately, (13, 2) on (32, 32) at 2.048 M samples: the unit operands transposed through LDS, and two variants not kept",
      "tools/exp/fvp_split_ab.py's loop with FVP_AB_WARM=400 FVP_AB_N=300 FVP_AB_READINGS=9, the parent as build/exp/lib_parent.so"),
     ("fvp_lds_tr_ab_bench.txt", "headline bench lines of the parent and the new library, interleaved, and their --dump-outputs compared", "tools/exp/lib_ab.py 'python bench.py --gpus 1 --steps 20 --warmup 3'"),
diff --git a/rllab_amd/_lib.py b/rllab_amd/_lib.py
--- a/rllab_amd/_lib.py
+++ b/rllab_amd/_lib.py
@@ -22,8 +22,9 @@
     "rl_gru_categorical_workspace_bytes", "rl_gru_categorical_eval", "rl_gru_categorical_grad", "rl_gru_categorical_fvp",
     "rl_rollout_population_gru", "rl_gae",
     "rl_discount_cumsum", "rl_debug_philox", "rl_policy_workspace_bytes", "rl_policy_activation_bytes", "rl_policy_loss_kl",
-    "rl_policy_grad", "rl_policy_grad_loss", "rl_policy_fvp", "rl_policy_fvp_variant", "rl_policy_fvp_cg_step", "rl_cg_init", "rl_cg_step", "rl_trpo_step", "rl_line_search_point", "rl_line_search_decide", "rl_adam_step",
+    "rl_policy_grad", "rl_policy_grad_loss", "rl_policy_fvp", "rl_policy_fvp_variant", "rl_policy_fvp_cg_step", "rl_cg_init", "rl_cg_step", "rl_trpo_step", "rl_line_search_point", "rl_line_search_decide", "rl_line_search_decide_dev", "rl_adam_step",
     "rl_path_scan", "rl_process_workspace_bytes", "rl_sample_stats_cols", "rl_sample_stats", "rl_adv_finish",
+    "rl_batch_scalars", "rl_adv_finish_dev",
     "rl_lfb_normal_eq", "rl_reps_workspace_bytes", "rl_reps_dual", "rl_reps_weights",
     "rl_peer_mailbox_bytes", "rl_peer_alloc", "rl_peer_free", "rl_peer_export", "rl_peer_open", "rl_peer_close",
     "rl_peer_allreduce_sum",
@@ -154,7 +155,14 @@
         ("old_log_std", ctypes.c_void_p), ("weights", ctypes.c_void_p), ("activations", ctypes.c_void_p),
         ("kl_penalty", ctypes.c_float), ("activation", ctypes.c_int32), ("opts", ctypes.c_void_p),
         ("layer_activations", ctypes.c_int32), ("reserved_pad", ctypes.c_int32), ("gate", ctypes.c_void_p),
-        ("obs_absmax", ctypes.c_void_p),
+        ("obs_absmax", ctypes.c_void_p), ("inv_count_dev", ctypes.c_void_p),
+    ]
+
+
+class BatchScalars(ctypes.Structure):
+    _fields_ = [
+        ("mean", ctypes.c_double), ("denom", ctypes.c_double), ("shift", ctypes.c_double), ("inv_count", ctypes.c_double),
+        ("inv_count_f32", ctypes.c_float), ("reserved_pad", ctypes.c_float),
     ]
 
 
@@ -294,7 +302,8 @@
     lib.rl_trpo_step.argtypes = [i32, vp, vp, vp, f64, f64, vp, vp, vp]
     lib.rl_line_search_point.argtypes = [i32, vp, vp, f64, vp, vp]
     lib.rl_line_search_decide.argtypes = [i32, vp, vp, f64, f64, i32, vp, vp, i32, vp, vp, f64, vp, vp]
-    lib.rl_adam_step.argtypes = [i32, vp, vp, vp, vp, f64, f64, f64, f64, vp]
+    lib.rl_line_search_decide_dev.argtypes = [i32, vp, vp, vp, f64, i32, vp, vp, i32, vp, vp, f64, vp, vp]
+    lib.rl_adam_step.argtypes =[i32, vp, vp, vp, vp, f64, f64, f64, f64, vp]
     sz = ctypes.c_size_t
     lib.rl_path_scan.argtypes = [i32, i32, i32, vp, vp, vp, i32, vp, vp, vp, vp]
     lib.rl_process_workspace_bytes.restype = sz
@@ -302,7 +311,9 @@
     lib.rl_sample_stats_cols.restype = i32
     lib.rl_sample_stats.argtypes = [sz, vp, vp, vp, vp, vp, vp, f64, f64, vp, i32, vp, sz, vp, vp]
     lib.rl_adv_finish.argtypes = [sz, vp, vp, f64, f64, f64, vp, vp]
-    lib.rl_lfb_normal_eq.argtypes = [sz, i32, vp, vp, vp, vp, vp, sz, vp, i32, vp]
+    lib.rl_batch_scalars.argtypes = [vp, i32, i32, vp, vp]
+    lib.rl_adv_finish_dev.argtypes = [sz, vp, vp, vp, vp, vp, vp]
+    lib.rl_lfb_normal_eq.argtypes =[sz, i32, vp, vp, vp, vp, vp, sz, vp, i32, vp]
     lib.rl_reps_workspace_bytes.restype = sz
     lib.rl_reps_workspace_bytes.argtypes = [i32, i32]
     lib.rl_reps_dual.argtypes = [i32, i32, i32, vp, vp, vp, vp, vp, f64, vp, vp, sz, vp, vp]
diff --git a/rllab_amd/algos/npo.py b/rllab_amd/algos/npo.py
--- a/rllab_amd/algos/npo.py
+++ b/rllab_amd/algos/npo.py
@@ -10,6 +10,10 @@
 def npo_inputs(policy, samples_data):
     traj = samples_data["_traj"]
     B = traj.B
+    scal = getattr(traj, "batch_scalars", None)
+    if scal is not None:
+        return (traj.obs.reshape(traj.obs_dim, B), traj.actions.reshape(traj.act_dim, B), traj.advantages.reshape(B),
+                traj.means.reshape(traj.act_dim, B), traj.log_std.reshape(-1, 1), traj.weights, scal)
     w = traj.valid.reshape(B).to(torch.float32)
     if getattr(traj, "count", None) is not None:
         cnt = torch.tensor(float(traj.count), dtype=torch.float64)
diff --git a/rllab_amd/baselines/linear_feature_baseline.py b/rllab_amd/baselines/linear_feature_baseline.py
--- a/rllab_amd/baselines/linear_feature_baseline.py
+++ b/rllab_amd/baselines/linear_feature_baseline.py
@@ -10,26 +10,64 @@
     def __init__(self, env_spec, reg_coeff=1e-5):
         self._coeffs_value = None
         self._pending = None
+        self._deferred = None
+        self._in_flight = []
+        self.dense_fits_launched = 0
         self._reg_coeff = reg_coeff
+
+    def defer_fit_dense(self, traj):
+        self._coeffs_value = None
+        self._pending = None
+        self._deferred = traj
+
+    def has_deferred_fit(self):
+        return self.__dict__.get("_deferred") is not None
+
+    _SIDE = {}
+
+    def launch_deferred_fit(self, after=None):
+        traj, self._deferred = self.__dict__.get("_deferred"), None
+        if traj is None:
+            return
+        self._in_flight = [(e, t) for e, t in self._in_flight if not e.query()]
+        if after is None:
+            self.fit_dense(traj)
+            return
+        dev = traj.device
+        side = self._SIDE.get(dev)
+        if side is None:
+            side = self._SIDE[dev] = torch.cuda.Stream(device=dev)
+        side.wait_event(after)
+        with torch.cuda.stream(side):
+            self.fit_dense(traj, side=True)
+            done = torch.cuda.Event()
+            done.record()
+        self._in_flight.append((done, traj))
 
     @property
     def _coeffs(self):
+        if self.__dict__.get("_deferred") is not None:
+            self.launch_deferred_fit()
         if self._pending is not None:
             read, F = self._pending
             self._pending = None
             host = read.get()
+            self._in_flight = [(e, t) for e, t in self.__dict__.get("_in_flight", []) if not e.query()]
             self._coeffs_value = self._solve(host[:F * F].reshape(F, F), host[F * F:])
         return self._coeffs_value
 
     @_coeffs.setter
     def _coeffs(self, value):
         self._pending = None
+        self._deferred = None
         self._coeffs_value = value
 
     def __getstate__(self):
         d = dict(self.__dict__)
         d["_coeffs_value"] = self._coeffs
         d["_pending"] = None
+        d["_deferred"] = None
+        d["_in_flight"] = []
         return d
 
     def __setstate__(self, d):
@@ -37,6 +75,9 @@
         if "_coeffs" in d:
             d["_coeffs_value"] = d.pop("_coeffs")
         d.setdefault("_pending", None)
+        d.setdefault("_deferred", None)
+        d.setdefault("_in_flight", [])
+        d.setdefault("dense_fits_launched", 0)
         self.__dict__.update(d)
 
     def get_param_values(self, **tags):
@@ -91,8 +132,9 @@
         w = torch.as_tensor(self._coeffs, dtype=torch.float64, device=traj.device)
         return (w @ self._features_dense(traj)).reshape(traj.T, traj.N)
 
-    def fit_dense(self, traj, all_reduce=None):
-        packed = self.normal_eq_dense(traj)
+    def fit_dense(self, traj, all_reduce=None, side=False):
+        self._deferred = None
+        packed = self.normal_eq_dense(traj, side=side)
         if all_reduce is not None:
             all_reduce(packed)
         self.fit_from_packed(packed, 2 * traj.obs_dim + 4)
@@ -102,7 +144,7 @@
         self._coeffs_value = None
         self._pending = (read_async(packed), F)
 
-    def normal_eq_dense(self, traj):
+    def normal_eq_dense(self, traj, side=False):
         F = 2 * traj.obs_dim + 4
         if traj.obs_dim <= 21 and traj.device.type == "cuda":
             from rllab_amd import _lib
@@ -113,8 +155,9 @@
             valid = traj.valid if traj.valid is not None else torch.ones((traj.T, traj.N), dtype=torch.bool,
                                                                          device=traj.device)
             valid_u8 = valid.contiguous().view(torch.uint8) if valid.dtype == torch.bool else valid.to(torch.uint8).contiguous()
-            ws = _workspace(traj.device, traj.obs_dim)
+            ws = _workspace(traj.device, traj.obs_dim, "side" if side else None)
             packed = torch.empty((F + 1) * F, dtype=torch.float64, device=traj.device)
+            self.dense_fits_launched = self.__dict__.get("dense_fits_launched", 0) + 1
             _lib.check(_lib.lib.rl_lfb_normal_eq(traj.B, traj.obs_dim, _lib.ptr(traj.obs), _lib.ptr(tin),
                                                  _lib.ptr(traj.returns), _lib.ptr(valid_u8), _lib.ptr(ws),
                                                  ws.numel(), _lib.ptr(packed),
diff --git a/rllab_amd/csrc/cg_kernels.hip b/rllab_amd/csrc/cg_kernels.hip
--- a/rllab_amd/csrc/cg_kernels.hip
+++ b/rllab_amd/csrc/cg_kernels.hip
@@ -92,13 +92,15 @@
 }
 
 __global__ void __launch_bounds__(CG_THREADS) line_search_decide_kernel(
-        int rows, const double* __restrict__ sums, const double* __restrict__ before, double inv_count, double delta,
+        int rows, const double* __restrict__ sums, const double* __restrict__ before, double inv_count,
+        const double* __restrict__ inv_count_dev, double delta,
         int candidate, double* __restrict__ state, int32_t* __restrict__ gate, int n, const float* __restrict__ prev,
         const double* __restrict__ step, double next_ratio, float* __restrict__ theta) {
     __shared__ int go_on;
     if (threadIdx.x == 0) {
         bool accepted = state[0] != 0.0;
         if (!accepted) {
+            if (inv_count_dev) inv_count = *inv_count_dev;
             double s0 = 0.0, s1 = 0.0, s2 = 0.0, mx = -INFINITY, b0 = 0.0;
             for (int r = 0; r < rows; ++r) {
                 s0 += sums[4 * r]; s1 += sums[4 * r + 1]; s2 += sums[4 * r + 2];
@@ -176,7 +178,20 @@
         (next_ratio > 0.0 && (n <= 0 || !prev || !step || !theta)))
         return set_error(RL_ERR_ARG, "rl_line_search_decide: bad argument");
     hipLaunchKernelGGL(line_search_decide_kernel, dim3(1), dim3(CG_THREADS), 0, (hipStream_t)stream, rows, sums, before,
-                       inv_count, max_constraint, candidate, state, gate, n, prev, step, next_ratio, theta);
+                       inv_count, (const double*)nullptr, max_constraint, candidate, state, gate, n, prev, step, next_ratio,
+                       theta);
+    return check_launch("line_search_decide_kernel");
+}
+
+extern "C" int rl_line_search_decide_dev(int rows, const double* sums, const double* before, const double* inv_count_dev,
+                                         double max_constraint, int candidate, double* state, int32_t* gate, int n,
+                                         const float* prev, const double* step, double next_ratio, float* theta,
+                                         void* stream) {
+    if (rows <= 0 || !sums || !before || !inv_count_dev || !state || !gate || candidate < 0 ||
+        (next_ratio > 0.0 && (n <= 0 || !prev || !step || !theta)))
+        return set_error(RL_ERR_ARG, "rl_line_search_decide_dev: bad argument");
+    hipLaunchKernelGGL(line_search_decide_kernel, dim3(1), dim3(CG_THREADS), 0, (hipStream_t)stream, rows, sums, before,
+                       0.0, inv_count_dev, max_constraint, candidate, state, gate, n, prev, step, next_ratio, theta);
     return check_launch("line_search_decide_kernel");
 }
 
diff --git a/rllab_amd/csrc/policy_csplit_kernels.hip b/rllab_amd/csrc/policy_csplit_kernels.hip
--- a/rllab_amd/csrc/policy_csplit_kernels.hip
+++ b/rllab_amd/csrc/policy_csplit_kernels.hip
@@ -850,6 +850,8 @@
 }
 int csplit_fvp_dispatch(const rl_policy_batch* g, const float* vec, void* ws, size_t ws_bytes, double* out, hipStream_t st) {
     if (!csplit_fvp_takes(g)) return RL_SPLIT_NOT_TAKEN;
+    if (g->inv_count_dev)
+        return set_error(RL_ERR_UNSUPPORTED, "rl_policy_batch.inv_count_dev: the cooperative split product takes 1 / W from the host");
     cs::CsShape s;
     cs::cs_shape(g, s);
     return s.L == 2 ? cs::launch_class<2>(s, g, vec, ws, ws_bytes, out, st)
diff --git a/rllab_amd/csrc/policy_kernels.hip b/rllab_amd/csrc/policy_kernels.hip
--- a/rllab_amd/csrc/policy_kernels.hip
+++ b/rllab_amd/csrc/policy_kernels.hip
@@ -43,6 +43,7 @@
     const float* old_log_std;
     const float* weight;
     float inv_count;
+    const float* inv_count_dev;
     float log_min_std;
     float kl_penalty;
     const float* cot;
@@ -81,6 +82,7 @@
     constexpr int ACT_ROWS = 2 * HT * 4;
 
     extern __shared__ __attribute__((aligned(16))) float smem[];
+    const float inv_count = launch_inv_count(a.inv_count_dev, a.inv_count);
     if (MODE == MODE_LOSS) {
         if (a.gate != nullptr && *a.gate != 0) return;
     }
@@ -314,7 +316,7 @@
                 if (w1 > 0.0f) max_kl = fmaxf(max_kl, kl);
             }
             if (MODE != MODE_LOSS) {
-                const float c = -wgt * advb * (MODE == MODE_GRAD ? lr : 1.0f) * a.inv_count;
+                const float c = -wgt * advb * (MODE == MODE_GRAD ? lr : 1.0f) * inv_count;
                 const float c1 = (lh == 0) ? c : 0.0f;
 #pragma unroll
                 for (int k = 0; k < DA; ++k) {
@@ -322,7 +324,7 @@
                     if (!floored[k]) gls[k] += c1 * (znew[k] * znew[k] - 1.0f);
                 }
                 if (a.kl_penalty != 0.0f) {
-                    const float p = a.kl_penalty * wgt * a.inv_count;
+                    const float p = a.kl_penalty * wgt * inv_count;
                     const float p1 = (lh == 0) ? p : 0.0f;
 #pragma unroll
                     for (int k = 0; k < DA; ++k) {
@@ -359,7 +361,7 @@
                 }
                 act_bwd_frag(dh1[t], acc, h1[t], c1);
             }
-            const float c = wgt * a.inv_count;
+            const float c = wgt * inv_count;
 #pragma unroll
             for (int k = 0; k < DA; ++k) {
                 float pd = 0.0f;
@@ -745,7 +747,7 @@
     a.kl_penalty = g->kl_penalty;
     a.B = g->n_samples; a.theta = g->theta; a.vec = vec; a.obs = g->obs; a.act = g->actions; a.adv = g->advantages;
     a.old_mean = g->old_means; a.old_log_std = g->old_log_std; a.weight = g->weights;
-    a.inv_count = g->inv_count; a.log_min_std = g->log_min_std;
+    a.inv_count = g->inv_count; a.inv_count_dev = g->inv_count_dev; a.log_min_std = g->log_min_std;
     a.gate = (MODE == MODE_LOSS) ? g->gate : nullptr;
     a.obs_absmax = nullptr;
     if (MODE == MODE_GRAD && CACHE && g->activations && g->obs_absmax) {
@@ -881,6 +883,9 @@
                              pl ? pl->out_mean : nullptr, pl ? pl->out_dmean : nullptr);
     }
     if (g->hidden2 < 0) return set_error(RL_ERR_ARG, "rl_policy_batch.hidden2 = %d", g->hidden2);
+    if (g->inv_count_dev && !net_has_narrow_kernel(d, k, h0, h1, g->hidden2))
+        return set_error(RL_ERR_UNSUPPORTED, "rl_policy_batch.inv_count_dev: obs_dim=%d act_dim=%d hidden=(%d,%d,%d) runs on "
+                         "the cooperative kernels, which take 1 / W from the host (inv_count)", d, k, h0, h1, g->hidden2);
     if (g->hidden2 > 0) {
         if (cg) return set_error(RL_ERR_UNSUPPORTED, "rl_policy_fvp_cg_step: two-layer 32 / 64-unit nets only");
         if (!all_tanh)
diff --git a/rllab_amd/csrc/policy_mfma.h b/rllab_amd/csrc/policy_mfma.h
--- a/rllab_amd/csrc/policy_mfma.h
+++ b/rllab_amd/csrc/policy_mfma.h
@@ -12,6 +12,11 @@
 __device__ __forceinline__ float ftanh(float x) {
     const float e = __builtin_amdgcn_exp2f(x * 2.8853900817779268f);
     return __builtin_fmaf(-2.0f, __builtin_amdgcn_rcpf(e + 1.0f), 1.0f);
+}
+
+__device__ __forceinline__ float launch_inv_count(const float* __restrict__ dev, float host) {
+    if (dev == nullptr) return host;
+    return __builtin_bit_cast(float, __builtin_amdgcn_readfirstlane(__builtin_bit_cast(int, *dev)));
 }
 
 __device__ __forceinline__ void act_frag(f32x16& h, const f32x16& z, int code) {
diff --git a/rllab_amd/csrc/policy_split16_kernels.hip b/rllab_amd/csrc/policy_split16_kernels.hip
--- a/rllab_amd/csrc/policy_split16_kernels.hip
+++ b/rllab_amd/csrc/policy_split16_kernels.hip
@@ -583,6 +583,8 @@
 }
 int split16_fvp_dispatch(const rl_policy_batch* g, const float* vec, void* ws, size_t ws_bytes, double* out, hipStream_t st) {
     if (!split16_fvp_takes(g)) return RL_SPLIT_NOT_TAKEN;
+    if (g->inv_count_dev)
+        return set_error(RL_ERR_UNSUPPORTED, "rl_policy_batch.inv_count_dev: the 16-sample-tile product takes 1 / W from the host");
     const bool three = !(g->opts && g->opts->fvp_split_wps == 4);
 #define SPLITCASE(DO, DA) if (g->obs_dim == DO && g->act_dim == DA) \
         return three ? split16::launch<DO, DA, 3>(g, vec, ws, ws_bytes, out, st) : split16::launch<DO, DA, 4>(g, vec, ws, ws_bytes, out, st);
diff --git a/rllab_amd/csrc/policy_split_kernels.hip b/rllab_amd/csrc/policy_split_kernels.hip
--- a/rllab_amd/csrc/policy_split_kernels.hip
+++ b/rllab_amd/csrc/policy_split_kernels.hip
@@ -30,6 +30,7 @@
     const float* obs;
     const float* weight;
     float inv_count;
+    const float* inv_count_dev;
     float log_min_std;
     float* partial;
 };
@@ -235,6 +236,7 @@
     static_assert(DO + 1 <= 32, "two k-blocks of inputs + the bias slot");
     static_assert(LDS_TOTAL >= WAVES * P * 4 && LDS_TOTAL <= 160 * 1024, "LDS budget; the fold rows alias the landing zones");
     extern __shared__ __attribute__((aligned(16))) char smem[];
+    const float inv_count = launch_inv_count(a.inv_count_dev, a.inv_count);
     const int wave = threadIdx.x / WV, lane = threadIdx.x % WV;
     const int lj = lane & 31, lh = lane >> 5;
     char* const land = smem + wave * WAVE_BYTES;
@@ -540,7 +542,7 @@
             for (int kb = 0; kb < 2; ++kb) acc = mm6(op(KB0 + 2 + kb), D0s[kb], acc);
         }
         stage();
-        const float c = wgt * a.inv_count;
+        const float c = wgt * inv_count;
         f32x16 dz1;
         float gmu[DA];
         f32x16 gz1;
@@ -798,6 +800,7 @@
     static_assert(DO + 1 <= 32 && DA <= 8, "two k-blocks of inputs + the bias slot; at most eight actions");
     static_assert(LDS_TOTAL >= WAVES * P * 4 && LDS_TOTAL <= 160 * 1024, "LDS budget; the fold rows alias everything");
     extern __shared__ __attribute__((aligned(16))) char smem[];
+    const float inv_count = launch_inv_count(a.inv_count_dev, a.inv_count);
     const int wave = threadIdx.x / WV, lane = threadIdx.x % WV;
     const int lj = lane & 31, lh = lane >> 5;
     char* const land = smem + wave * WAVE_BYTES;
@@ -994,7 +997,7 @@
             chains(O_W1T, D0s, acc);
         }
         stage();
-        const float c = wgt * a.inv_count;
+        const float c = wgt * inv_count;
         f32x16 dz1[HT], gz1[HT];
         float gmu[DA];
 #pragma unroll
@@ -1210,7 +1213,7 @@
     constexpr int LDS_BYTES = WAVES * (2 * 64 * TS * 4 + TS * 8 * 4) + N_OPS * 3 * WV * 16 + 2 * (HT * 16 * DA * 2 + HT * 16) * 4;
     Args a;
     a.B = g->n_samples; a.theta = g->theta; a.vec = vec; a.acts = g->activations; a.obs = g->obs; a.weight = g->weights;
-    a.inv_count = g->inv_count; a.log_min_std = g->log_min_std;
+    a.inv_count = g->inv_count; a.inv_count_dev = g->inv_count_dev; a.log_min_std = g->log_min_std;
     const int n_tiles = a.B / TS;
     int grid = (n_tiles + WAVES - 1) / WAVES;
     if (grid > 256) grid = 256;
@@ -1241,7 +1244,7 @@
                               ((WPS == 2 || DA > 2) ? 2 * (16 * DA * 2 + 16) * 4 : 0);
     Args a;
     a.B = g->n_samples; a.theta = g->theta; a.vec = vec; a.acts = g->activations; a.obs = g->obs; a.weight = g->weights;
-    a.inv_count = g->inv_count; a.log_min_std = g->log_min_std;
+    a.inv_count = g->inv_count; a.inv_count_dev = g->inv_count_dev; a.log_min_std = g->log_min_std;
     const int n_tiles = a.B / TS;
     int grid = (n_tiles + WAVES - 1) / WAVES;
     if (grid > 256) grid = 256;
diff --git a/rllab_amd/csrc/policy_splith_kernels.hip b/rllab_amd/csrc/policy_splith_kernels.hip
--- a/rllab_amd/csrc/policy_splith_kernels.hip
+++ b/rllab_amd/csrc/policy_splith_kernels.hip
@@ -29,6 +29,7 @@
     const float* weight;
     const float* xmax;
     float inv_count;
+    const float* inv_count_dev;
     float log_min_std;
     float* partial;
 };
@@ -349,6 +350,7 @@
     static_assert(DO + 1 <= 32 && (DA <= 2 || WPS == 1), "two k-blocks of inputs + the bias slot; thin heads at two per SIMD");
     static_assert(LDS_TOTAL >= WAVES * P * 4 && LDS_TOTAL <= 160 * 1024, "LDS budget; the fold rows alias the landing zones");
     extern __shared__ __attribute__((aligned(16))) char smem[];
+    const float inv_count = launch_inv_count(a.inv_count_dev, a.inv_count);
     const int wave = threadIdx.x / WV, lane = threadIdx.x % WV;
     const int lj = lane & 31, lh = lane >> 5;
     char* const land = smem + wave * WAVE_BYTES;
@@ -406,7 +408,7 @@
         floored[k] = raw < a.log_min_std;
         const float ls = fmaxf(raw, a.log_min_std);
         var_[k] = __expf(2.0f * ls);
-        fkS[k] = 2.0f / (2.0f * var_[k] + 1e-8f) * a.inv_count;
+        fkS[k] = 2.0f / (2.0f * var_[k] + 1e-8f) * inv_count;
         fkmax = fmaxf(fkmax, fkS[k]);
     }
     float mx[5];
@@ -579,7 +581,7 @@
             gmu[k] = wgt * (dmu * fkS[k]);
         }
         if (lh == 0) {
-            wsum += wgt * a.inv_count;
+            wsum += wgt * inv_count;
 #pragma unroll
             for (int k = 0; k < DA; ++k) gb2[k] += gmu[k];
         }
@@ -733,6 +735,7 @@
     static_assert(DO + 1 <= 32 && DA <= 8, "two k-blocks of inputs + the bias slot; at most eight actions");
     static_assert(LDS_TOTAL >= WAVES * P * 4 && LDS_TOTAL <= 160 * 1024, "LDS budget; the fold rows alias everything");
     extern __shared__ __attribute__((aligned(16))) char smem[];
+    const float inv_count = launch_inv_count(a.inv_count_dev, a.inv_count);
     const int wave = threadIdx.x / WV, lane = threadIdx.x % WV;
     const int lj = lane & 31, lh = lane >> 5;
     char* const land = smem + wave * WAVE_BYTES;
@@ -782,7 +785,7 @@
         floored[k] = raw < a.log_min_std;
         const float ls = fmaxf(raw, a.log_min_std);
         var_[k] = __expf(2.0f * ls);
-        fkS[k] = 2.0f / (2.0f * var_[k] + 1e-8f) * a.inv_count;
+        fkS[k] = 2.0f / (2.0f * var_[k] + 1e-8f) * inv_count;
         fkmax = fmaxf(fkmax, fkS[k]);
     }
     float mx[5];
@@ -975,7 +978,7 @@
             gmu[k] = wgt * (dmu * fkS[k]);
         }
         if (lh == 0) {
-            wsum += wgt * a.inv_count;
+            wsum += wgt * inv_count;
 #pragma unroll
             for (int k = 0; k < DA; ++k) { gb2[k] += gmu[k]; gmub[lj * 8 + k] = gmu[k]; }
         }
@@ -1137,7 +1140,7 @@
 static Args make_args(const rl_policy_batch* g, const float* vec) {
     Args a;
     a.B = g->n_samples; a.theta = g->theta; a.vec = vec; a.acts = g->activations; a.obs = g->obs; a.weight = g->weights;
-    a.xmax = g->obs_absmax; a.inv_count = g->inv_count; a.log_min_std = g->log_min_std; a.partial = nullptr;
+    a.xmax = g->obs_absmax; a.inv_count = g->inv_count; a.inv_count_dev = g->inv_count_dev; a.log_min_std = g->log_min_std; a.partial = nullptr;
     return a;
 }
 
diff --git a/rllab_amd/csrc/process_kernels.hip b/rllab_amd/csrc/process_kernels.hip
--- a/rllab_amd/csrc/process_kernels.hip
+++ b/rllab_amd/csrc/process_kernels.hip
@@ -277,6 +277,41 @@
     if (b >= B) return;
     const double a = ((double)adv_in[b] - mean) / denom + shift;
     adv_out[b] = valid[b] ? (float)a : 0.0f;
+}
+
+__global__ void __launch_bounds__(64) batch_scalars_kernel(const double* __restrict__ s, int center_adv, int positive_adv,
+                                                           rl_batch_scalars_t* __restrict__ out) {
+#pragma clang fp contract(off)
+    if (threadIdx.x != 0 || blockIdx.x != 0) return;
+    const double cnt = s[ST_COUNT];
+    double mean = 0.0, denom = 1.0, shift = 0.0;
+    if (center_adv) {
+        mean = __ddiv_rn(s[ST_ADV], cnt);
+        const double d = __dsub_rn(__ddiv_rn(s[ST_ADV2], cnt), __dmul_rn(mean, mean));
+        const double var = (0.0 > d) ? 0.0 : d;
+        denom = __dadd_rn(__dsqrt_rn(var), 1e-8);
+    }
+    if (positive_adv) shift = __dadd_rn(-__ddiv_rn(__dsub_rn(s[ST_ADVMIN], mean), denom), 1e-8);
+    const double inv = __ddiv_rn(1.0, cnt);
+    out->mean = mean;
+    out->denom = denom;
+    out->shift = shift;
+    out->inv_count = inv;
+    out->inv_count_f32 = (float)inv;
+    out->reserved_pad = 0.0f;
+}
+
+__global__ void __launch_bounds__(256)
+adv_finish_dev_kernel(size_t B, const float* __restrict__ adv_in, const uint8_t* __restrict__ valid,
+                      const rl_batch_scalars_t* __restrict__ sc, float* __restrict__ adv_out,
+                      float* __restrict__ weight_out) {
+    const size_t b = (size_t)blockIdx.x * 256 + threadIdx.x;
+    if (b >= B) return;
+    const double mean = sc->mean, denom = sc->denom, shift = sc->shift;
+    const double a = ((double)adv_in[b] - mean) / denom + shift;
+    const bool v = valid[b] != 0;
+    adv_out[b] = v ? (float)a : 0.0f;
+    if (weight_out) weight_out[b] = v ? 1.0f : 0.0f;
 }
 
 constexpr int NE_TILE = 64;
@@ -533,6 +568,23 @@
     hipLaunchKernelGGL(adv_finish_kernel, dim3((unsigned)((n_samples + 255) / 256)), dim3(256), 0,
                        (hipStream_t)stream, n_samples, adv_in, valid, mean, denom, shift, adv_out);
     return check_launch("adv_finish_kernel");
+}
+
+extern "C" int rl_batch_scalars(const double* stats20, int center_adv, int positive_adv, rl_batch_scalars_t* out,
+                                void* stream) {
+    if (!stats20 || !out) return set_error(RL_ERR_ARG, "rl_batch_scalars: bad argument");
+    hipLaunchKernelGGL(batch_scalars_kernel, dim3(1), dim3(64), 0, (hipStream_t)stream, stats20, center_adv,
+                       positive_adv, out);
+    return check_launch("batch_scalars_kernel");
+}
+
+extern "C" int rl_adv_finish_dev(size_t n_samples, const float* adv_in, const uint8_t* valid,
+                                 const rl_batch_scalars_t* scalars, float* adv_out, float* weight_out, void* stream) {
+    if (n_samples == 0 || !adv_in || !valid || !scalars || !adv_out)
+        return set_error(RL_ERR_ARG, "rl_adv_finish_dev: bad argument");
+    hipLaunchKernelGGL(adv_finish_dev_kernel, dim3((unsigned)((n_samples + 255) / 256)), dim3(256), 0,
+                       (hipStream_t)stream, n_samples, adv_in, valid, scalars, adv_out, weight_out);
+    return check_launch("adv_finish_dev_kernel");
 }
 
 extern "C" int rl_lfb_normal_eq(size_t n_samples, int obs_dim, const float* obs, const int32_t* tin,
diff --git a/rllab_amd/policies/fused_ops.py b/rllab_amd/policies/fused_ops.py
--- a/rllab_amd/policies/fused_ops.py
+++ b/rllab_amd/policies/fused_ops.py
@@ -63,10 +63,12 @@
         obs, act, adv, old_mean, old_ls, w, theta = keep
         assert theta.data_ptr() == self.layout.theta().data_ptr()
         pol = self.policy
-        inv = float(inv_count)
+        inv_dev = getattr(inv_count, "dev_f32", None)
+        inv = inv_count if inv_dev is not None else float(inv_count)
         b = _lib.PolicyBatch(
             n_samples=obs.shape[-1], obs_dim=self.dims[0], act_dim=self.dims[1], hidden0=self.dims[2],
-            hidden1=self.dims[3], hidden2=self.dims[4], inv_count=inv,
+            hidden1=self.dims[3], hidden2=self.dims[4], inv_count=0.0 if inv_dev is not None else inv,
+            inv_count_dev=inv_dev,
             log_min_std=math.log(pol.min_std) if pol.min_std is not None else -1e30,
             theta=theta.data_ptr(), obs=obs.data_ptr(), actions=act.data_ptr(), advantages=adv.data_ptr(),
             old_means=old_mean.data_ptr(), old_log_std=old_ls.data_ptr(), weights=w.data_ptr(),
@@ -106,7 +108,7 @@
     def _resolve(c):
         if c["host"] is None:
             h = c["read"].get().reshape(-1, 4)
-            sums = h[:, :3].sum(axis=0) * c["inv"]
+            sums = h[:, :3].sum(axis=0) * float(c["inv"])
             c["host"] = (float(sums[0]), float(sums[1]), float(sums[2]), float(h[:, 3].max()))
         return c["host"]
 
@@ -209,6 +211,7 @@
         ws = self._workspace(dev)
         grad = torch.empty(self.n_kernel, dtype=torch.float64, device=dev)
         out4 = torch.empty(4, dtype=torch.float64, device=dev)
+        inv = float(inv)
         self._acts_tag = None
         b.activations = None
         b.kl_penalty = float(penalty)
@@ -368,10 +371,16 @@
                                                       st), "rl_policy_loss_kl")
                 rows = D.all_gather_rows(outs[k])
                 nxt = float(ratios[k + 1]) if k + 1 < K else 0.0
-                _lib.check(_lib.lib.rl_line_search_decide(
-                    rows.shape[0], _lib.ptr(rows), _lib.ptr(brows), inv, float(max_constraint), k, _lib.ptr(state),
-                    _lib.ptr(gate), n, _lib.ptr(prev32), _lib.ptr(step), nxt, _lib.ptr(theta), st),
-                    "rl_line_search_decide")
+                if hasattr(inv, "dev_f64"):
+                    _lib.check(_lib.lib.rl_line_search_decide_dev(
+                        rows.shape[0], _lib.ptr(rows), _lib.ptr(brows), inv.dev_f64, float(max_constraint), k,
+                        _lib.ptr(state), _lib.ptr(gate), n, _lib.ptr(prev32), _lib.ptr(step), nxt, _lib.ptr(theta), st),
+                        "rl_line_search_decide_dev")
+                else:
+                    _lib.check(_lib.lib.rl_line_search_decide(
+                        rows.shape[0], _lib.ptr(rows), _lib.ptr(brows), inv, float(max_constraint), k, _lib.ptr(state),
+                        _lib.ptr(gate), n, _lib.ptr(prev32), _lib.ptr(step), nxt, _lib.ptr(theta), st),
+                        "rl_line_search_decide")
                 self._epoch += 1
         finally:
             b.gate = None
@@ -379,7 +388,7 @@
 
     def line_search_resolve(self, rec, inputs):
         h = rec["read"].get()
-        K, inv = rec["K"], rec["inv"]
+        K, inv = rec["K"], float(rec["inv"])
         accepted = int(h[1]) if h[0] != 0.0 else None
         n_eval = K if accepted is None else accepted + 1
         sums = h[2:2 + 4 * K].reshape(K, 4)
diff --git a/rllab_amd/sampler/base.py b/rllab_amd/sampler/base.py
--- a/rllab_amd/sampler/base.py
+++ b/rllab_amd/sampler/base.py
@@ -64,8 +64,8 @@
 _WS = {}
 
 
-def _workspace(device, obs_dim):
-    key = (device, obs_dim)
+def _workspace(device, obs_dim, tag=None):
+    key = (device, obs_dim, tag)
     if key not in _WS:
         n = _lib.lib.rl_process_workspace_bytes(int(obs_dim))
         _WS[key] = torch.empty(n, dtype=torch.uint8, device=device)
@@ -114,6 +114,52 @@
 
 
 _SHIFT = dict(ret=0.0, und=0.0)
+
+
+class DeviceBatchScalars(object):
+
+    def __init__(self, record, stats_read):
+        self.record = record
+        self._read = stats_read
+        self._inv = None
+
+    @property
+    def dev_f32(self):
+        return self.record.data_ptr() + 32
+
+    @property
+    def dev_f64(self):
+        return self.record.data_ptr() + 24
+
+    def __float__(self):
+        if self._inv is None:
+            self._inv = 1.0 / float(fold_stats(self._read.get())[_COUNT])
+        return self._inv
+
+    def to(self, dtype):
+        return torch.tensor(float(self), dtype=dtype)
+
+
+def _device_scalars_path(algo, traj, baseline, dense_lfb, categorical):
+    import os
+    if os.environ.get("RLLAB_PROCESS_HOST_STATS", "0")[:1] == "1" or D.is_distributed() or categorical:
+        return False
+    if not (dense_lfb and hasattr(baseline, "defer_fit_dense") and traj.obs.is_cuda):
+        return False
+    if getattr(algo.policy, "recurrent", False) or traj.log_std is None or traj.log_std_planes is not None:
+        return False
+    if not hasattr(algo, "prefetch_update"):
+        return False
+    from rllab_amd.optimizers.conjugate_gradient_optimizer import ConjugateGradientOptimizer
+    from rllab_amd.policies.fused_ops import FusedGaussianMLPOps
+    opt = getattr(algo, "optimizer", None)
+    fused = getattr(opt, "_fused", None)
+    if not isinstance(opt, ConjugateGradientOptimizer) or type(fused) is not FusedGaussianMLPOps or fused.wide_kernels:
+        return False
+    if opt._subsample_factor < 1 or opt._hvp_given or traj.log_std.numel() != fused.dims[1]:
+        return False
+    _lib.launch_opts()
+    return _lib._OPTS.fvp_split not in (2, 3)
 
 
 def process_dense(algo, itr, traj, log=True):
@@ -164,7 +210,27 @@
                                   "continuous envs' observations; use LinearFeatureBaseline or ZeroBaseline")
     if dense_fit and log:
         logger.log("fitting baseline...")
-    if dense_fit and D.is_distributed() and hasattr(baseline, "normal_eq_dense"):
+    fast = _device_scalars_path(algo, traj, baseline, dense_lfb, categorical)
+    if fast:
+        stats_read = read_async(st.reshape(1, -1))
+        record = torch.empty(5, dtype=torch.float64, device=dev)
+        _lib.check(_lib.lib.rl_batch_scalars(_lib.ptr(st), int(bool(algo.center_adv)), int(bool(algo.positive_adv)),
+                                             _lib.ptr(record), _lib.stream_ptr()), "rl_batch_scalars")
+        adv_out = torch.empty((T, N), dtype=torch.float32, device=dev)
+        weights = torch.empty(B, dtype=torch.float32, device=dev)
+        _lib.check(_lib.lib.rl_adv_finish_dev(B, _lib.ptr(adv), _lib.ptr(valid_u8), _lib.ptr(record), _lib.ptr(adv_out),
+                                              _lib.ptr(weights), _lib.stream_ptr()), "rl_adv_finish_dev")
+        traj.advantages = adv_out
+        traj.weights = weights
+        traj.batch_scalars = DeviceBatchScalars(record, stats_read)
+        ls_read = read_async(traj.log_std)
+        baseline.defer_fit_dense(traj)
+        paths = PathList(traj)
+        samples_data = SamplesData(_traj=traj, paths=paths)
+        if traj.obs.is_cuda and getattr(algo, "_update_follows", False):
+            algo.prefetch_update(samples_data)
+        s = fold_stats(stats_read.get())
+    elif dense_fit and D.is_distributed() and hasattr(baseline, "normal_eq_dense"):
         packed = baseline.normal_eq_dense(traj)
         rows = D.all_gather_rows(torch.cat([st, packed]))
         stats_read = read_async(rows[:, :st.numel()].contiguous())
@@ -177,10 +243,13 @@
     else:
         stats_read = read_async(D.all_gather_rows(st))
         dense_fit_done = False
-    ls_read = read_async(traj.log_std) if (traj.log_std is not None and traj.log_std_planes is None) else None
-    if dense_fit and not dense_fit_done:
+    if not fast:
+        ls_read = read_async(traj.log_std) if (traj.log_std is not None and traj.log_std_planes is None) else None
+    if not fast and dense_fit and not dense_fit_done:
         baseline.fit_dense(traj, all_reduce=D.all_reduce_sum_ if D.is_distributed() else None)
-    if categorical:
+    if fast:
+        pass
+    elif categorical:
         host = stats_read.get().reshape(-1)
         s, ent_sum_host = fold_stats(host[:20]), float(host[20])
     else:
@@ -200,20 +269,21 @@
     else:
         ev = 1 - var_res / (var_y + 1e-8)
 
-    mean_a, denom, shift = 0.0, 1.0, 0.0
-    if algo.center_adv:
-        mean_a, var_a = moments(_ADV, _ADV2, cnt)
-        denom = float(np.sqrt(var_a)) + 1e-8
-    if algo.positive_adv:
-        shift = -((s[_ADVMIN] - mean_a) / denom) + 1e-8
-    adv_out = torch.empty((T, N), dtype=torch.float32, device=dev)
-    _lib.check(_lib.lib.rl_adv_finish(B, _lib.ptr(adv), _lib.ptr(valid_u8), float(mean_a), float(denom),
-                                      float(shift), _lib.ptr(adv_out), _lib.stream_ptr()), "rl_adv_finish")
-    traj.advantages = adv_out
-    paths = PathList(traj)
-    samples_data = SamplesData(_traj=traj, paths=paths)
-    if hasattr(algo, "prefetch_update") and traj.obs.is_cuda and getattr(algo, "_update_follows", False):
-        algo.prefetch_update(samples_data)
+    if not fast:
+        mean_a, denom, shift = 0.0, 1.0, 0.0
+        if algo.center_adv:
+            mean_a, var_a = moments(_ADV, _ADV2, cnt)
+            denom = float(np.sqrt(var_a)) + 1e-8
+        if algo.positive_adv:
+            shift = -((s[_ADVMIN] - mean_a) / denom) + 1e-8
+        adv_out = torch.empty((T, N), dtype=torch.float32, device=dev)
+        _lib.check(_lib.lib.rl_adv_finish(B, _lib.ptr(adv), _lib.ptr(valid_u8), float(mean_a), float(denom),
+                                          float(shift), _lib.ptr(adv_out), _lib.stream_ptr()), "rl_adv_finish")
+        traj.advantages = adv_out
+        paths = PathList(traj)
+        samples_data = SamplesData(_traj=traj, paths=paths)
+        if hasattr(algo, "prefetch_update") and traj.obs.is_cuda and getattr(algo, "_update_follows", False):
+            algo.prefetch_update(samples_data)
 
     if prog is not None and n_paths > 0:
         m_prog, var_prog = moments(_PROG, _PROG2, n_paths)
diff --git a/rllab_amd/sampler/trajectories.py b/rllab_amd/sampler/trajectories.py
--- a/rllab_amd/sampler/trajectories.py
+++ b/rllab_amd/sampler/trajectories.py
@@ -22,6 +22,8 @@
         self.progress_stats = None
         self.count = None
         self.log_std_host = None
+        self.weights = None
+        self.batch_scalars = None
 
     @property
     def device(self):
diff --git a/rllab_amd/sampler/vectorized_sampler.py b/rllab_amd/sampler/vectorized_sampler.py
--- a/rllab_amd/sampler/vectorized_sampler.py
+++ b/rllab_amd/sampler/vectorized_sampler.py
@@ -79,6 +79,9 @@
         return name, why
 
     def shutdown_worker(self):
+        baseline = getattr(self.algo, "baseline", None)
+        if hasattr(baseline, "launch_deferred_fit"):
+            baseline.launch_deferred_fit()
         if self.vec_env is not None:
             self.vec_env.terminate()
 
@@ -111,7 +114,7 @@
         if getattr(self.vec_env, "stateful_rollouts", False):
             return
         counter = self.vec_env.step_counter
-        first = self._rollout_chunk(policy, self.algo.max_path_length, True)
+        first = self._with_deferred_fit(lambda: self._rollout_chunk(policy, self.algo.max_path_length, True))
         self._prefetched = (itr, policy.param_version(), first, counter)
 
     def _drop_prefetched(self):
@@ -133,11 +136,24 @@
                 self._drop_prefetched()
         t_start = time.time()
         if first is None:
-            first = self._launch(policy, algo.max_path_length, True)
+            first = self._with_deferred_fit(lambda: self._launch(policy, algo.max_path_length, True))
         traj = self._meet_batch_size(policy, first)
         self.last_num_samples = traj.B
         self.last_sample_time = time.time() - t_start
         return PathList(traj)
+
+    def _with_deferred_fit(self, launch):
+        baseline = getattr(self.algo, "baseline", None)
+        if not (hasattr(baseline, "has_deferred_fit") and baseline.has_deferred_fit()):
+            return launch()
+        if os.environ.get("RLLAB_FIT_SIDE_STREAM", "1")[:1] == "0":
+            baseline.launch_deferred_fit()
+            return launch()
+        ready = torch.cuda.Event()
+        ready.record()
+        out = launch()
+        baseline.launch_deferred_fit(after=ready)
+        return out
 
     def _rollout_chunk(self, policy, steps, first):
         graphable = getattr(self.vec_env, "graphable", True)
```
